# Jsewill/chiaSWARM

Hardware: AMD Instinct MI355X
Metric: images/sec (whole node) SD2.1 512×512 50-step txt2img at 1/2/4/8 MI355X; p50 job latency (higher is better)
Workload: dtype bf16; 1 GPU; bench_config=sd21, global_batch=4, seq_len=4096, parallelism=dp1, resolution=512x512, denoise_steps=50, scheduler=DPMSolverMultistepScheduler (karras), impl=hip, hip_graphs=True

## Files before the change

chiaswarm_amd/models/layers.py:

```python
from __future__ import annotations

import math

import torch
import torch.nn as nn
import torch.nn.functional as F

from .. import ops


class Prepared(nn.Module):

    def prepare(self):
        pass


def prepare_model(model: nn.Module) -> nn.Module:
    for m in model.modules():
        if isinstance(m, Prepared):
            m.prepare()
    if hasattr(model, "prepare_self"):
        model.prepare_self()
    return model


class Linear(nn.Linear, Prepared):

    def forward(self, x, residual=None, act=None, row_stats=False):
        return ops.gemm(x, self.weight, self.bias, residual=residual, act=act, row_stats=row_stats)


class Conv2d(nn.Conv2d, Prepared):

    def prepare(self):
        self.wp = ops.pack_conv_weight(self.weight.detach())

    def _wp(self):
        wp = getattr(self, "wp", None)
        if wp is None or wp.device != self.weight.device or wp.dtype != self.weight.dtype:
            self.prepare()
        return self.wp

    def forward(self, x, residual=None, up2x=False, bias2d=None, padding=None, act=None, out_scale=1.0,
                out=None, gn_stats=False, row_stats=False, residual2=None, res_scale=1.0,
                norm=None, norm_optional=False):
        kh, kw = self.kernel_size
        if (kh == 1 and kw == 1 and self.stride == (1, 1) and not up2x and act is None and out_scale == 1.0
                and out is None and x.is_contiguous() and residual2 is None and res_scale == 1.0 and norm is None):
            w2 = self.weight.view(self.out_channels, self.in_channels)
            gr = x.shape[1] * x.shape[2] if (gn_stats and bias2d is None and x.dim() == 4) else 0
            y = ops.gemm(x, w2, self.bias, residual=residual, gn_rows=gr, row_stats=row_stats and bias2d is None)
            if bias2d is not None:
                y = y + bias2d[:, None, None, :].to(y.dtype)
            return y
        if padding is None:
            ph, pw = self.padding
            pad = ph if ph == pw else (ph, pw, ph, pw)
        else:
            pad = padding
        return ops.conv2d(x, self._wp(), self.bias, self.stride[0], pad, residual=residual,
                          up2x=up2x, bias2d=bias2d, act=act, out_scale=out_scale, out=out,
                          dilation=max(self.dilation), gn_stats=gn_stats, residual2=residual2, res_scale=res_scale,
                          norm=norm, norm_optional=norm_optional)


class Conv1d(nn.Conv1d, Prepared):

    def prepare(self):
        self.wp = self.weight.detach().permute(0, 2, 1).unsqueeze(1).contiguous()

    def _wp(self):
        wp = getattr(self, "wp", None)
        if wp is None or wp.device != self.weight.device or wp.dtype != self.weight.dtype:
            self.prepare()
        return self.wp

    def forward(self, x, act=None, residual=None, out_scale=1.0, out=None, padding=None):
        assert self.stride == (1,), "Conv1d: stride 1 only"
        p = self.padding[0] if padding is None else padding
        return ops.conv1d(x, self._wp(), self.bias, padding=p, dilation=self.dilation[0], act=act,
                          residual=residual, out_scale=out_scale, out=out)


class ConvTranspose1d(nn.ConvTranspose1d, Prepared):

    def prepare(self):
        self.phases = ops.pack_conv_transpose1d(self.weight.detach(), self.stride[0], self.padding[0])

    def forward(self, x, act=None):
        ph = getattr(self, "phases", None)
        if ph is None or (ph[0][0] is not None and (ph[0][0].device != self.weight.device
                                                    or ph[0][0].dtype != self.weight.dtype)):
            self.prepare()
        return ops.conv_transpose1d(x, self.weight, self.bias, self.stride[0], self.padding[0], self.phases, act)


class GroupNorm(nn.GroupNorm):
    def forward(self, x, silu=False):
        pre = getattr(x, "_csk_prenorm", None)
        if pre is not None and pre[0] == self._key(silu):
            return pre[1]
        return ops.group_norm(x, self.weight, self.bias, self.num_groups, self.eps, silu=silu)

    def _key(self, silu):
        w, b = self.weight, self.bias
        return (w.data_ptr(), w._version, b.data_ptr(), b._version, self.num_groups, self.eps, bool(silu))

    def attach(self, raw, normed, silu=False):
        if normed is not None:
            raw._csk_prenorm = (self._key(silu), normed)
        return raw

    def after_conv(self, silu=False, keep_raw=False):
        return (self.weight, self.bias, self.num_groups, self.eps, silu, keep_raw)


class LayerNorm(nn.LayerNorm):
    def forward(self, x):
        return ops.layer_norm(x, self.weight, self.bias, self.eps)


class Attention(Prepared):
    def __init__(self, query_dim, heads, dim_head, cross_dim=None, bias=False, out_bias=True,
                 norm_groups=None, norm_eps=1e-6, residual=False):
        super().__init__()
        inner = heads * dim_head
        self.heads, self.dim_head = heads, dim_head
        self.is_cross = cross_dim is not None
        kv_dim = cross_dim if cross_dim is not None else query_dim
        self.to_q = Linear(query_dim, inner, bias=bias)
        self.to_k = Linear(kv_dim, inner, bias=bias)
        self.to_v = Linear(kv_dim, inner, bias=bias)
        self.to_out = nn.ModuleList([Linear(inner, query_dim, bias=out_bias)])
        self.group_norm = GroupNorm(norm_groups, query_dim, eps=norm_eps) if norm_groups else None
        self.residual = residual
        self.scale = 1.0 / math.sqrt(dim_head)

    def prepare(self):
        q, k, v = self.to_q, self.to_k, self.to_v
        if self.is_cross:
            self.w_kv = torch.cat([k.weight, v.weight], 0).detach()
            self.b_kv = torch.cat([k.bias, v.bias], 0).detach() if k.bias is not None else None
        else:
            self.w_qkv = torch.cat([q.weight, k.weight, v.weight], 0).detach()
            self.b_qkv = (torch.cat([q.bias, k.bias, v.bias], 0).detach()
                          if q.bias is not None else None)

    def _ensure(self):
        attr = "w_kv" if self.is_cross else "w_qkv"
        w = getattr(self, attr, None)
        if w is None or w.device != self.to_q.weight.device or w.dtype != self.to_q.weight.dtype:
            self.prepare()

    def context_kv(self, ctx):
        self._ensure()
        b, s, _ = ctx.shape
        kv = ops.gemm(ctx, self.w_kv, self.b_kv)
        return kv.view(b, s, 2, self.heads, self.dim_head)

    def forward(self, x, ctx=None, kv=None, residual=None, causal=False):
        self._ensure()
        if self.is_cross:
            return self.attend_q(self.to_q(x), kv, ctx if ctx is not None else x, residual)
        return self.attend_qkv(ops.gemm(x, self.w_qkv, self.b_qkv), residual, causal=causal)

    def attend_qkv(self, qkv, residual=None, causal=False, row_stats=False):
        b, s, _ = qkv.shape
        h, d = self.heads, self.dim_head
        qkv = qkv.view(b, s, 3, h, d)
        store = self.__dict__.get("_store_probs")
        if store is not None:
            q, k = qkv[:, :, 0].float().transpose(1, 2), qkv[:, :, 1].float().transpose(1, 2)
            store.append(torch.softmax(q @ k.transpose(-1, -2) * self.scale, dim=-1))
        o = ops.attention(qkv[:, :, 0], qkv[:, :, 1], qkv[:, :, 2], self.scale, causal=causal)
        return self.to_out[0](o.reshape(b, s, h * d), residual=residual, row_stats=row_stats)

    def attend_q(self, q, kv, ctx, residual=None, row_stats=False):
        b, s, _ = q.shape
        h, d = self.heads, self.dim_head
        if kv is None:
            kv = self.context_kv(ctx)
        store = self.__dict__.get("_store_probs")
        if store is not None:
            qf, kf = q.view(b, s, h, d).float().transpose(1, 2), kv[:, :, 0].float().transpose(1, 2)
            store.append(torch.softmax(qf @ kf.transpose(-1, -2) * self.scale, dim=-1))
        o = ops.attention(q.view(b, s, h, d), kv[:, :, 0], kv[:, :, 1], self.scale)
        return self.to_out[0](o.reshape(b, s, h * d), residual=residual, row_stats=row_stats)


class SpatialSelfAttention(Attention):

    def __init__(self, channels, norm_groups=32, eps=1e-6):
        super().__init__(channels, 1, channels, bias=True, norm_groups=norm_groups, norm_eps=eps)

    def forward(self, x):
        b, hh, ww, c = x.shape
        hN = self.group_norm(x).view(b, hh * ww, c)
        out = super().forward(hN, residual=x.view(b, hh * ww, c))
        return out.view(b, hh, ww, c)


class GEGLU(Prepared):
    def __init__(self, dim_in, dim_out):
        super().__init__()
        self.proj = Linear(dim_in, dim_out * 2)

    def prepare(self):
        self.wp, self.bp = ops.pack_geglu(self.proj.weight.detach(),
                                          self.proj.bias.detach() if self.proj.bias is not None else None)

    def ensure(self):
        wp = getattr(self, "wp", None)
        if wp is None or wp.device != self.proj.weight.device or wp.dtype != self.proj.weight.dtype:
            self.prepare()

    def forward(self, x):
        self.ensure()
        return ops.gemm(x, self.wp, self.bp, act="geglu")


class FeedForward(Prepared):

    def __init__(self, dim, mult=4):
        super().__init__()
        inner = dim * mult
        self.inner = inner
        self.net = nn.ModuleList([GEGLU(dim, inner), nn.Identity(), Linear(inner, dim)])

    def prepare(self):
        p, d = self.net[0].proj, self.net[2]
        if p.weight.shape[1] != 320:
            self.ff_w1p = self.ff_b1p = self.ff_w2p = None
            return
        self.ff_w1p, self.ff_b1p, self.ff_w2p = ops.pack_ff_fused(
            p.weight.detach(), None if p.bias is None else p.bias.detach(), d.weight.detach())

    def fused_weights(self):
        w = getattr(self, "ff_w1p", None)
        p = self.net[0].proj.weight
        if (w is None and p.shape[1] == 320) or (w is not None and (w.device != p.device or w.dtype != p.dtype)):
            self.prepare()
        return getattr(self, "ff_w1p", None), getattr(self, "ff_b1p", None), getattr(self, "ff_w2p", None)

    def forward(self, x, residual=None):
        return self.net[2](self.net[0](x), residual=residual)


class BasicTransformerBlock(nn.Module):
    def __init__(self, dim, heads, dim_head, cross_dim):
        super().__init__()
        self.norm1 = LayerNorm(dim)
        self.attn1 = Attention(dim, heads, dim_head)
        self.norm2 = LayerNorm(dim)
        self.attn2 = Attention(dim, heads, dim_head, cross_dim=cross_dim)
        self.norm3 = LayerNorm(dim)
        self.ff = FeedForward(dim)

    def _fold(self, name, w, b, norm):
        key = (w.data_ptr(), w._version, norm.weight.data_ptr(), norm.weight._version, w.dtype, w.device)
        folds = self.__dict__.setdefault("_ln_folds", {})
        f = folds.get(name)
        if f is None or f[0] != key:
            f = (key, ops.fold_layer_norm(w.detach(), None if b is None else b.detach(), norm.weight.detach(),
                                          None if norm.bias is None else norm.bias.detach()))
            folds[name] = f
        return f[1]

    def forward(self, x, ctx=None, kv=None, row_stats=None, dup=False, qkv=None):
        hip = ops.row_stats_wanted(x)
        if row_stats is None:
            row_stats = hip
        a1, a2, ff = self.attn1, self.attn2, self.ff
        a1._ensure()
        if qkv is None:
            fus = ops.ln_fusable(x)
            qkv = ops.layer_norm_gemm(x, self.norm1, a1.w_qkv, a1.b_qkv,
                                      self._fold("qkv", a1.w_qkv, a1.b_qkv, self.norm1) if fus else None)
        x = a1.attend_qkv(qkv, residual=x, row_stats=hip)
        if hip and not dup and kv is not None and x.dim() == 3 and ops.xattn_fusable(x, kv, x.shape[1]):
            w2, colsum, b2 = self._fold("q", a2.to_q.weight, a2.to_q.bias, self.norm2)
            x = ops.xattn_block(x, w2, colsum, b2, kv, a2.to_out[0].weight, a2.to_out[0].bias, self.norm2.eps,
                                a2.scale, x.shape[1], row_stats=hip)
        elif hip and not dup and kv is not None and x.dim() == 3 and ops.qattn_fusable(x, kv, x.shape[1]):
            fus = ops.ln_fusable(x)
            o = ops.layer_norm_gemm_attn(x, self.norm2, a2.to_q.weight, a2.to_q.bias,
                                         self._fold("q", a2.to_q.weight, a2.to_q.bias, self.norm2) if fus else None,
                                         kv, a2.scale, x.shape[1])
            x = a2.to_out[0](o, residual=x, row_stats=hip)
        else:
            fus = ops.ln_fusable(x)
            q = ops.layer_norm_gemm(x, self.norm2, a2.to_q.weight, a2.to_q.bias,
                                    self._fold("q", a2.to_q.weight, a2.to_q.bias, self.norm2) if fus else None)
            if dup:
                q, x = ops.dup2(q), ops.dup2(x)
            x = a2.attend_q(q, kv, ctx if ctx is not None else x, residual=x, row_stats=hip)
        if hip and not row_stats and ops.ff_fusable(x, ff.inner):
            w1p, b1p, w2p = ff.fused_weights()
            if w1p is not None:
                return ops.ff_fused(x, self.norm3.weight, self.norm3.bias, w1p, b1p, w2p, ff.net[2].bias,
                                    self.norm3.eps)
        g = ff.net[0]
        g.ensure()
        fus = ops.ln_fusable(x)
        hdn = ops.layer_norm_gemm(x, self.norm3, g.wp, g.bp, self._fold("ff", g.wp, g.bp, self.norm3) if fus else None,
                                  act="geglu")
        return ff.net[2](hdn, residual=x, row_stats=row_stats)


class Transformer2D(nn.Module):

    def __init__(self, channels, heads, cross_dim, layers=1, linear_proj=True, groups=32):
        super().__init__()
        dim_head = channels // heads
        self.norm = GroupNorm(groups, channels, eps=1e-6)
        self.linear_proj = linear_proj
        if linear_proj:
            self.proj_in = Linear(channels, channels)
            self.proj_out = Linear(channels, channels)
        else:
            self.proj_in = Conv2d(channels, channels, 1)
            self.proj_out = Conv2d(channels, channels, 1)
        self.transformer_blocks = nn.ModuleList(
            [BasicTransformerBlock(channels, heads, dim_head, cross_dim) for _ in range(layers)])

    def cross_modules(self):
        return [blk.attn2 for blk in self.transformer_blocks]

    def _xin_weights(self):
        blk = self.transformer_blocks[0]
        a1 = blk.attn1
        a1._ensure()
        wi = self.proj_in.weight
        key = (wi.data_ptr(), wi._version, a1.w_qkv.data_ptr(), a1.w_qkv._version, blk.norm1.weight._version,
               wi.device, wi.dtype)
        hit = self.__dict__.get("_xin")
        if hit is None or hit[0] != key:
            w2, colsum, b2 = blk._fold("qkv", a1.w_qkv, a1.b_qkv, blk.norm1)
            c = wi.shape[0]
            hit = (key, ops.pack_xin_qkv(wi.detach().reshape(c, c), None if self.proj_in.bias is None
                                         else self.proj_in.bias.detach(), w2, colsum, b2))
            self.__dict__["_xin"] = hit
        return hit[1]

    def _xin_ok(self, x) -> bool:
        if not ops.row_stats_wanted(x) or not self.transformer_blocks:
            return False
        c = x.shape[-1]
        a1 = self.transformer_blocks[0].attn1
        w = self.proj_in.weight
        return (w.shape[0] == c and w.numel() == c * c and a1.to_q.weight.shape[0] == c and not a1.is_cross
                and ops.xin_fusable(x, self.norm.num_groups))

    def forward(self, x, ctx=None, kvs=None, dup=False):
        b, hh, ww, c = x.shape
        hip = ops.row_stats_wanted(x)
        qkv0 = None
        got = None
        if self._xin_ok(x):
            got = ops.xin_qkv(x, self.norm.weight, self.norm.bias, self.norm.num_groups, self.norm.eps,
                              self._xin_weights(), self.transformer_blocks[0].norm1.eps)
        if got is not None:
            h, qkv0 = got[0].view(b, hh * ww, c), got[1].view(b, hh * ww, 3 * c)
        else:
            h = self.norm(x)
            h = self.proj_in(h, row_stats=hip)
            rows = getattr(h, "_csk_rows", None)
            h = h.view(b, hh * ww, c)
            if rows is not None:
                h._csk_rows = rows
        nb = len(self.transformer_blocks)
        for i, blk in enumerate(self.transformer_blocks):
            if dup and i == 0:
                h = blk(h, ctx=ctx, kv=None if kvs is None else kvs[i], row_stats=hip and i + 1 < nb, dup=True,
                        qkv=qkv0)
                x, b = ops.dup2(x), 2 * b
                continue
            h = blk(h, ctx=ctx, kv=None if kvs is None else kvs[i], row_stats=hip and i + 1 < nb,
                    qkv=qkv0 if i == 0 else None)
        if isinstance(self.proj_out, Linear):
            return ops.gemm(h.view(b, hh, ww, c), self.proj_out.weight, self.proj_out.bias, residual=x,
                            gn_rows=hh * ww)
        return self.proj_out(h.view(b, hh, ww, c), residual=x, gn_stats=True)


class ResnetBlock2D(Prepared):

    def __init__(self, cin, cout, temb_channels=None, groups=32, eps=1e-5, groups_out=None):
        super().__init__()
        self.norm1 = GroupNorm(groups, cin, eps=eps)
        self.conv1 = Conv2d(cin, cout, 3, padding=1)
        self.time_emb_proj = Linear(temb_channels, cout) if temb_channels else None
        self.norm2 = GroupNorm(groups_out or groups, cout, eps=eps)
        self.conv2 = Conv2d(cout, cout, 3, padding=1)
        self.conv_shortcut = Conv2d(cin, cout, 1, padding=0) if cin != cout else None
        self.out_channels = cout

    def prepare(self):
        self.__dict__["_scf"] = None

    def _sc_static(self) -> bool:
        sc, c2 = self.conv_shortcut, self.conv2
        return (sc is not None and sc.kernel_size == (1, 1) and sc.stride == (1, 1) and sc.padding == (0, 0)
                and c2.kernel_size == (3, 3) and c2.stride == (1, 1) and c2.padding == (1, 1)
                and c2.dilation == (1, 1) and sc.in_channels % 64 == 0 and c2.in_channels % 64 == 0
                and c2.out_channels % 64 == 0 and self.norm1.weight.dim() == 1 and self.norm2.weight.dim() == 1)

    def _sc_pack(self):
        sc, c2 = self.conv_shortcut, self.conv2
        w2, ws, b2, bs = c2.weight, sc.weight, c2.bias, sc.bias
        key = (w2.data_ptr(), w2._version, ws.data_ptr(), ws._version, None if b2 is None else b2._version,
               None if bs is None else bs._version, w2.device, w2.dtype)
        hit = self.__dict__.get("_scf")
        if hit is None or hit[0] != key:
            _, wv, (wsc,) = ops.pack_conv_extra(ops.pack_conv_weight(w2.detach()),
                                                [ws.detach().reshape(sc.out_channels, sc.in_channels)])
            bias = None
            if b2 is not None or bs is not None:
                bias = sum(b.detach().float() for b in (b2, bs) if b is not None).to(w2.dtype)
            hit = (key, (wv, wsc, bias))
            self.__dict__["_scf"] = hit
        if c2.__dict__.get("wp") is not None:
            c2.wp = None
        return hit[1]

    def _sc_fuse(self, srcs):
        if not ops.SC_FUSE or not self._sc_static():
            return None
        cs = [int(t.shape[-1]) for t in srcs]
        if sum(cs) != self.conv_shortcut.in_channels or any(c % 64 for c in cs) or any(t.dim() != 4 for t in srcs):
            return None
        wv, wsc, bias = self._sc_pack()
        extra, off = [], 0
        for t, c in zip(srcs, cs):
            extra.append((t, wsc[:, off:off + c]))
            off += c
        return wv, tuple(extra), bias

    def _shortcut(self, srcs):
        sc_conv = self.conv_shortcut
        if len(srcs) == 1:
            return sc_conv(srcs[0])
        a, b = srcs
        w = sc_conv.weight.view(sc_conv.out_channels, sc_conv.in_channels)
        ca = a.shape[-1]
        return ops.gemm(b, w[:, ca:], sc_conv.bias, residual=ops.gemm(a, w[:, :ca]))

    def _conv2(self, h, sc, next_norm, fuse=None):
        conv2 = lambda residual, **kw: self.conv2(h, residual=residual, **kw)
        if fuse is not None:
            wv, extra, bias = fuse
            if ops.conv_extra_fusable(h, wv, extra):
                conv2 = lambda residual, **kw: ops.conv2d(h, wv, bias, 1, 1, extra=extra, **kw)
                sc = None
            else:
                sc = self._shortcut(sc)
        if next_norm is None or next_norm.weight.dim() != 1:
            return conv2(sc, gn_stats=True)
        yn, out = conv2(sc, norm=next_norm.after_conv(keep_raw=True), norm_optional=True)
        return next_norm.attach(out, yn)

    def forward(self, x, temb_proj=None, next_norm=None):
        fuse = self._sc_fuse((x,))
        if fuse is not None:
            h = self.norm1(x, silu=True)
            h = self.conv1(h, bias2d=temb_proj, norm=self.norm2.after_conv(silu=True))
            return self._conv2(h, (x,), next_norm, fuse)
        sc = x
        with ops.side_branch(x) as br:
            if self.conv_shortcut is not None:
                sc = self.conv_shortcut(x)
        h = self.norm1(x, silu=True)
        h = self.conv1(h, bias2d=temb_proj, norm=self.norm2.after_conv(silu=True))
        br.join()
        return self._conv2(h, sc, next_norm)

    def forward_cat(self, a, b, temb_proj=None, next_norm=None):
        sc_conv = self.conv_shortcut
        hn = None
        if ops.use_hip(a) and sc_conv is not None and sc_conv.kernel_size == (1, 1) and self.norm1.weight.dim() == 1:
            hn = ops.group_norm_cat(a, b, self.norm1.weight, self.norm1.bias, self.norm1.num_groups,
                                    self.norm1.eps, silu=True)
        if hn is None:
            return self.forward(ops.cat_channels(a, b), temb_proj, next_norm)
        fuse = self._sc_fuse((a, b))
        if fuse is not None:
            h = self.conv1(hn, bias2d=temb_proj, norm=self.norm2.after_conv(silu=True))
            return self._conv2(h, (a, b), next_norm, fuse)
        w = sc_conv.weight.view(sc_conv.out_channels, sc_conv.in_channels)
        ca = a.shape[-1]
        with ops.side_branch(a) as br:
            sc = ops.gemm(a, w[:, :ca])
            sc = ops.gemm(b, w[:, ca:], sc_conv.bias, residual=sc)
        h = self.conv1(hn, bias2d=temb_proj, norm=self.norm2.after_conv(silu=True))
        br.join()
        return self._conv2(h, sc, next_norm)


class Downsample2D(nn.Module):
    def __init__(self, channels, padding=1):
        super().__init__()
        self.conv = Conv2d(channels, channels, 3, stride=2, padding=padding)
        self.pad_asym = padding == 0

    def forward(self, x):
        if self.pad_asym:
            return self.conv(x, padding=(0, 0, 1, 1), gn_stats=True)
        return self.conv(x, gn_stats=True)


class Upsample2D(nn.Module):
    def __init__(self, channels):
        super().__init__()
        self.conv = Conv2d(channels, channels, 3, padding=1)

    def forward(self, x, size=None):
        b, h, w, c = x.shape
        if size is None or (int(size[0]), int(size[1])) == (2 * h, 2 * w):
            return self.conv(x, up2x=True, gn_stats=True)
        xi = F.interpolate(x.permute(0, 3, 1, 2), size=(int(size[0]), int(size[1])), mode="nearest")
        return self.conv(xi.permute(0, 2, 3, 1).contiguous(), gn_stats=True)


def timestep_embedding(t: torch.Tensor, dim: int, flip_sin_to_cos=True, shift=0.0,
                       max_period=10000.0) -> torch.Tensor:
    half = dim // 2
    exponent = -math.log(max_period) * torch.arange(half, dtype=torch.float32, device=t.device)
    exponent = exponent / (half - shift)
    emb = t.float()[:, None] * torch.exp(exponent)[None, :]
    emb = torch.cat([torch.sin(emb), torch.cos(emb)], dim=-1)
    if flip_sin_to_cos:
        emb = torch.cat([emb[:, half:], emb[:, :half]], dim=-1)
    return emb


class TimestepEmbedding(nn.Module):
    def __init__(self, cin, dim):
        super().__init__()
        self.linear_1 = Linear(cin, dim)
        self.linear_2 = Linear(dim, dim)

    def forward(self, x):
        return self.linear_2(self.linear_1(x, act="silu"))


def init_random_(model: nn.Module, seed: int = 0, std_scale: float = 1.0):
    g = torch.Generator(device="cpu").manual_seed(seed)
    with torch.no_grad():
        for name, p in model.named_parameters():
            if p.dim() >= 2:
                fan_in = p[0].numel()
                std = std_scale / math.sqrt(fan_in)
                if name.endswith("embedding.weight") or "embedding" in name and p.dim() == 2 and "linear" not in name:
                    std = 0.02
                t = torch.randn(p.shape, generator=g, dtype=torch.float32) * std
                p.copy_(t.to(p.dtype))
            elif name.endswith("bias"):
                p.zero_()
            else:
                p.fill_(1.0)
    return model


def init_random_fast_(model: nn.Module, seed: int = 0, std_scale: float = 1.0):
    dev = next(model.parameters()).device
    g = torch.Generator(device=dev).manual_seed(seed)
    with torch.no_grad():
        for name, p in model.named_parameters():
            if p.dim() >= 2:
                fan_in = p[0].numel()
                std = std_scale / math.sqrt(fan_in)
                if "embedding" in name and "linear" not in name:
                    std = 0.02
                p.copy_((torch.randn(p.shape, generator=g, device=dev, dtype=torch.float32) * std).to(p.dtype))
            elif name.endswith("bias"):
                p.zero_()
            else:
                p.fill_(1.0)
    return model
```

chiaswarm_amd/ops/__init__.py:

```python
from __future__ import annotations

import math

import os

import torch
import torch.nn.functional as F

from . import _lib
from .mode import get_mode, ops_mode, set_mode, use_hip

GEGLU_BLOCK = 16


def pack_geglu(w: torch.Tensor, b: torch.Tensor | None):
    two_f, k = w.shape
    f = two_f // 2
    assert f % GEGLU_BLOCK == 0
    wp = w.view(2, f // GEGLU_BLOCK, GEGLU_BLOCK, k).transpose(0, 1).reshape(two_f, k)
    bp = None
    if b is not None:
        bp = b.view(2, f // GEGLU_BLOCK, GEGLU_BLOCK).transpose(0, 1).reshape(two_f)
    return wp.contiguous(), (bp.contiguous() if bp is not None else None)


def _gelu_f(x):
    return F.gelu(x)


_ACT_REF = {
    None: lambda y: y, "none": lambda y: y, "gelu": F.gelu, "silu": F.silu,
    "quick_gelu": lambda y: y * torch.sigmoid(1.702 * y), "lrelu": lambda y: F.leaky_relu(y, 0.2),
    "lrelu0.1": lambda y: F.leaky_relu(y, 0.1), "lrelu0.01": lambda y: F.leaky_relu(y, 0.01),
    "tanh": torch.tanh, "relu": F.relu, "elu": F.elu, "gelu_tanh": lambda y: F.gelu(y, approximate="tanh"),
}


def apply_act(y, act):
    return _ACT_REF[act](y)


def _cdt(t):
    return torch.float32 if not t.is_cuda else t.dtype


def _ref_gemm(a2, w, bias, residual, act):
    dt = _cdt(a2)
    if bias is not None:
        y = torch.addmm(bias.to(dt), a2.to(dt), w.to(dt).t())
    else:
        y = a2.to(dt) @ w.to(dt).t()
    if act == "geglu":
        m, n = y.shape
        y = y.view(m, n // (2 * GEGLU_BLOCK), 2, GEGLU_BLOCK)
        y = (y[:, :, 0, :] * _gelu_f(y[:, :, 1, :])).reshape(m, n // 2)
    else:
        y = apply_act(y, act)
    if residual is not None:
        y = y + residual.reshape(y.shape).to(dt)
    return y.to(a2.dtype)


def gemm(a: torch.Tensor, w: torch.Tensor, bias=None, residual=None, act=None, gn_rows=0, row_stats=False):
    lead = a.shape[:-1]
    k = a.shape[-1]
    a2 = a.reshape(-1, k)
    if use_hip(a):
        from . import hip_ops

        y = hip_ops.gemm(a2, w, bias, residual, act, gn_rows=gn_rows, row_stats=row_stats)
    else:
        y = _ref_gemm(a2, w, bias, residual, act)
    out = y.view(*lead, y.shape[-1])
    for attr in ("_csk_gn", "_csk_rows"):
        st = getattr(y, attr, None)
        if st is not None:
            setattr(out, attr, st)
    return out


def fold_layer_norm(w: torch.Tensor, bias, gamma: torch.Tensor, beta):
    wf = w.float()
    w2 = (wf * gamma.float()[None, :]).to(w.dtype)
    colsum = w2.float().sum(1).contiguous()
    b2 = wf @ beta.float() if beta is not None else torch.zeros(w.shape[0], device=w.device)
    if bias is not None:
        b2 = b2 + bias.float()
    return w2.contiguous(), colsum, b2.to(w.dtype)


LN_FUSE = os.environ.get("CSK_LN_FUSE", "1") == "1"


SIDE_STREAM = os.environ.get("CSK_SIDE_STREAM", "0") == "1"
_SIDE: dict = {}


class side_branch:

    def __init__(self, x: torch.Tensor):
        self.on = SIDE_STREAM and use_hip(x)
        self.dev = x.device

    def __enter__(self):
        if self.on:
            self.main = torch.cuda.current_stream(self.dev)
            self.side = _SIDE.get(self.dev)
            if self.side is None:
                self.side = _SIDE[self.dev] = torch.cuda.Stream(self.dev)
            self.side.wait_stream(self.main)
            self._ctx = torch.cuda.stream(self.side)
            self._ctx.__enter__()
        return self

    def __exit__(self, *exc):
        if self.on:
            self._ctx.__exit__(*exc)
        return False

    def join(self):
        if self.on:
            self.main.wait_stream(self.side)


def row_stats_wanted(x: torch.Tensor) -> bool:
    return LN_FUSE and use_hip(x)


def ln_fusable(x: torch.Tensor) -> bool:
    rows = getattr(x, "_csk_rows", None)
    return LN_FUSE and use_hip(x) and rows is not None and x.shape[-1] % 8 == 0


def layer_norm_gemm(x, norm, w, bias, folded, act=None, residual=None, row_stats=False):
    if ln_fusable(x):
        from . import hip_ops

        w2, colsum, b2 = folded
        lead = x.shape[:-1]
        y = hip_ops.gemm(x.reshape(-1, x.shape[-1]), w2, b2, residual, act,
                         ln=(x._csk_rows, colsum, float(norm.eps)), row_stats=row_stats)
        out = y.view(*lead, y.shape[-1])
        if getattr(y, "_csk_rows", None) is not None:
            out._csk_rows = y._csk_rows
        return out
    return gemm(layer_norm(x, norm.weight, norm.bias, norm.eps), w, bias, residual=residual, act=act,
                row_stats=row_stats)


def qattn_fusable(x: torch.Tensor, kv, rows_per_b: int) -> bool:
    if not use_hip(x):
        return False
    from . import hip_ops

    return hip_ops.qattn_ok(x, kv, rows_per_b)


def layer_norm_gemm_attn(x, norm, w, bias, folded, kv, scale, rows_per_b):
    lead = x.shape[:-1]
    if use_hip(x):
        from . import hip_ops

        if ln_fusable(x):
            w2, colsum, b2 = folded
            o = hip_ops.gemm_attn(x.reshape(-1, x.shape[-1]), w2, b2, kv, scale, rows_per_b,
                                  ln=(x._csk_rows, colsum, float(norm.eps)))
        else:
            xn = layer_norm(x, norm.weight, norm.bias, norm.eps)
            o = hip_ops.gemm_attn(xn.reshape(-1, x.shape[-1]), w, bias, kv, scale, rows_per_b)
        return o.view(*lead, o.shape[-1])
    return _ref_gemm_attn(layer_norm(x, norm.weight, norm.bias, norm.eps), w, bias, kv, scale)


def _ref_gemm_attn(xn, w, bias, kv, scale):
    b, s, c = xn.shape
    q = xn.float() @ w.float().t()
    if bias is not None:
        q = q + bias.float()
    heads, d = kv.shape[3], kv.shape[4]
    k, v = kv[:b, :, 0].float(), kv[:b, :, 1].float()
    qh = q.view(b, s, heads, d).transpose(1, 2)
    att = torch.softmax((qh @ k.permute(0, 2, 3, 1)) * scale, -1)
    return (att @ v.transpose(1, 2)).transpose(1, 2).reshape(b, s, c).to(xn.dtype)


_FF_PERM = (0, 1, 2, 3, 8, 9, 10, 11, 4, 5, 6, 7, 12, 13, 14, 15)


def _ff_keys(device):
    r = torch.arange(32, device=device)
    k1 = (r & 7) ^ ((r >> 3) & 1)
    k2 = (r >> 2) & 3
    p8, p4 = torch.arange(8, device=device), torch.arange(4, device=device)
    return p8[None, :] ^ k1[:, None], p4[None, :] ^ k2[:, None]


def pack_ff_fused(w1, b1, w2):
    two_i, c = w1.shape
    inner = two_i // 2
    t = inner // 16
    k8, k4 = _ff_keys(w1.device)
    w1t = torch.stack((w1[:inner].reshape(t, 16, c), w1[inner:].reshape(t, 16, c)), 1).reshape(t, 32, c // 64, 8, 8)
    w1p = torch.gather(w1t, 3, k8[None, :, None, :, None].expand(t, 32, c // 64, 8, 8))
    w1p = w1p.permute(0, 2, 1, 3, 4).reshape(t, c // 64, 32, 64)
    b1p = None
    if b1 is not None:
        b1p = torch.stack((b1[:inner].reshape(t, 16), b1[inner:].reshape(t, 16)), 1).reshape(t, 32).float()
    perm = torch.tensor(_FF_PERM, device=w2.device)
    w2q = w2.reshape(c, t, 16).index_select(2, perm).reshape(c // 32, 32, inner // 32, 4, 8)
    w2p = torch.gather(w2q, 3, k4[None, :, None, :, None].expand(c // 32, 32, inner // 32, 4, 8))
    w2p = w2p.permute(2, 0, 1, 3, 4).reshape(inner // 32, c // 32, 32, 32)
    return w1p.contiguous(), (None if b1p is None else b1p.contiguous()), w2p.contiguous()


def unpack_ff_fused(w1p, b1p, w2p):
    t, si = w1p.shape[0], w1p.shape[1]
    c, inner = 64 * si, 16 * t
    k8, k4 = _ff_keys(w1p.device)
    inv8, inv4 = torch.argsort(k8, 1), torch.argsort(k4, 1)
    x = w1p.reshape(t, si, 32, 8, 8).permute(0, 2, 1, 3, 4)
    x = torch.gather(x, 3, inv8[None, :, None, :, None].expand(t, 32, si, 8, 8)).reshape(t, 32, c)
    w1 = torch.cat((x[:, :16].reshape(inner, c), x[:, 16:].reshape(inner, c)), 0)
    b1 = None if b1p is None else torch.cat((b1p[:, :16].reshape(inner), b1p[:, 16:].reshape(inner)), 0)
    nc, no = w2p.shape[0], w2p.shape[1]
    y = w2p.reshape(nc, no, 32, 4, 8).permute(1, 2, 0, 3, 4)
    y = torch.gather(y, 3, inv4[None, :, None, :, None].expand(no, 32, nc, 4, 8)).reshape(c, inner // 16, 16)
    w2 = y[:, :, torch.argsort(torch.tensor(_FF_PERM, device=w2p.device))].reshape(c, inner)
    return w1, b1, w2


def ff_fusable(x: torch.Tensor, inner: int) -> bool:
    if not use_hip(x) or x.dim() != 3:
        return False
    from . import hip_ops

    return hip_ops.ff_fused_ok(x, inner)


def ff_fused(x, gamma, beta, w1p, b1p, w2p, b2, eps):
    if use_hip(x):
        from . import hip_ops

        return hip_ops.ff_geglu(x, gamma, beta, w1p, b1p, w2p, b2, eps)
    return _ref_ff_fused(x, gamma, beta, w1p, b1p, w2p, b2, eps)


def _ref_ff_fused(x, gamma, beta, w1p, b1p, w2p, b2, eps):
    w1, b1, w2 = unpack_ff_fused(w1p, b1p, w2p)
    c, inner = w2.shape
    xf = x.float()
    h = torch.nn.functional.layer_norm(xf, (c,), gamma.float(), None if beta is None else beta.float(), eps)
    vg = torch.nn.functional.linear(h, w1.float(), None if b1 is None else b1.float())
    hid = vg[..., :inner] * torch.nn.functional.gelu(vg[..., inner:])
    y = torch.nn.functional.linear(hid, w2.float(), None if b2 is None else b2.float())
    return (xf + y).to(x.dtype)


def _a_tiles(w):
    n, c = w.shape
    t = n // 32
    k8, _ = _ff_keys(w.device)
    x = w.reshape(t, 32, c // 64, 8, 8)
    x = torch.gather(x, 3, k8[None, :, None, :, None].expand(t, 32, c // 64, 8, 8))
    return x.permute(0, 2, 1, 3, 4).reshape(t, c // 64, 32, 64)


def _a_untiles(p):
    t, si = p.shape[0], p.shape[1]
    k8, _ = _ff_keys(p.device)
    inv8 = torch.argsort(k8, 1)
    x = p.reshape(t, si, 32, 8, 8).permute(0, 2, 1, 3, 4)
    return torch.gather(x, 3, inv8[None, :, None, :, None].expand(t, 32, si, 8, 8)).reshape(32 * t, 64 * si)


def pack_xin_qkv(wi, bi, wq, colsum, bq):
    c = wi.shape[0]
    perm = torch.tensor(_FF_PERM, device=wq.device)
    wqp = wq.reshape(wq.shape[0], c // 16, 16).index_select(2, perm).reshape(wq.shape[0], c)
    w = torch.cat([_a_tiles(wi.reshape(c, c)), _a_tiles(wqp)], 0).contiguous()
    f32 = lambda t, n: (torch.zeros(n, device=wi.device) if t is None else t.float()).contiguous()
    return w, f32(bi, c), f32(colsum, wq.shape[0]), f32(bq, wq.shape[0])


def unpack_xin_qkv(w):
    c = 64 * w.shape[1]
    full = _a_untiles(w)
    wi, wqp = full[:c], full[c:]
    inv = torch.argsort(torch.tensor(_FF_PERM, device=w.device))
    return wi, wqp.reshape(wqp.shape[0], c // 16, 16).index_select(2, inv).reshape(wqp.shape[0], c)


def xin_fusable(x: torch.Tensor, groups: int) -> bool:
    if not use_hip(x):
        return False
    from . import hip_ops

    return hip_ops.xin_ok(x, groups)


def xin_qkv(x, gn_gamma, gn_beta, groups, gn_eps, packed, ln_eps):
    w, bi, colsum, bq = packed
    if use_hip(x):
        from . import hip_ops

        stat = hip_ops.gn_stats(x, groups, gn_eps)
        if stat is None:
            return None
        return hip_ops.xin_qkv(x, stat, gn_gamma, gn_beta, w, bi, colsum, bq, ln_eps)
    return _ref_xin_qkv(x, gn_gamma, gn_beta, groups, gn_eps, packed, ln_eps)


def _ref_xin_qkv(x, gn_gamma, gn_beta, groups, gn_eps, packed, ln_eps):
    w, bi, colsum, bq = packed
    wi, wq = unpack_xin_qkv(w)
    B, C = x.shape[0], x.shape[-1]
    xf = x.float().reshape(B, -1, C)
    g = xf.reshape(B, -1, groups, C // groups)
    mean = g.mean(dim=(1, 3), keepdim=True)
    var = g.var(dim=(1, 3), keepdim=True, unbiased=False)
    xg = ((g - mean) * torch.rsqrt(var + gn_eps)).reshape(B, -1, C)
    xg = xg * gn_gamma.float() + (0 if gn_beta is None else gn_beta.float())
    h = xg @ wi.float().t() + bi
    n = torch.nn.functional.layer_norm(h, (C,), eps=ln_eps)
    qkv = n @ wq.float().t() + bq
    return h.reshape(-1, C).to(x.dtype), qkv.reshape(-1, 3 * C).to(x.dtype)


def xattn_fusable(x: torch.Tensor, kv, rows_per_b: int) -> bool:
    if not use_hip(x):
        return False
    from . import hip_ops

    return hip_ops.xattn_ok(x, kv, rows_per_b)


def xattn_block(x, wq, colsum, bq, kv, wo, bo, eps, scale, rows_per_b, row_stats=True):
    if use_hip(x):
        from . import hip_ops

        return hip_ops.xattn_block(x, wq, colsum, bq, kv, wo, bo, eps, scale, rows_per_b, row_stats=row_stats)
    return _ref_xattn_block(x, wq, colsum, bq, kv, wo, bo, eps, scale)


def _ref_xattn_block(x, wq, colsum, bq, kv, wo, bo, eps, scale):
    xf = x.float()
    mean = xf.mean(-1, keepdim=True)
    rstd = torch.rsqrt(xf.var(-1, unbiased=False, keepdim=True) + eps)
    q = rstd * (xf @ wq.float().t() - mean * colsum.float()) + bq.float()
    b, s, c = x.shape
    heads, d = kv.shape[3], kv.shape[4]
    k, v = kv[:b, :, 0].float(), kv[:b, :, 1].float()
    qh = q.view(b, s, heads, d).transpose(1, 2)
    att = torch.softmax((qh @ k.permute(0, 2, 3, 1)) * scale, -1)
    o = (att @ v.transpose(1, 2)).transpose(1, 2).reshape(b, s, c)
    y = o @ wo.float().t() + xf
    if bo is not None:
        y = y + bo.float()
    return y.to(x.dtype)


def cat_channels(a: torch.Tensor, b: torch.Tensor) -> torch.Tensor:
    y = torch.cat([a, b], dim=-1)
    sa, sb = getattr(a, "_csk_gn", None), getattr(b, "_csk_gn", None)
    if sa is not None and sb is not None and sa[1] == sb[1]:
        ca, cb = a.shape[-1], b.shape[-1]
        nseg = sa[0].numel() // (2 * ca)
        if nseg * 2 * cb == sb[0].numel():
            y._csk_gn = (torch.cat([sa[0].view(nseg, ca, 2), sb[0].view(nseg, cb, 2)], 1).view(-1), sa[1])
    return y


def pack_conv_weight(w: torch.Tensor) -> torch.Tensor:
    return w.permute(0, 2, 3, 1).contiguous()


def norm_padding(padding):
    if isinstance(padding, int):
        return (padding,) * 4
    assert len(padding) == 4
    return tuple(int(p) for p in padding)


def conv_out_size(h, w, kh, kw, stride, padding, up2x=False, dilation=1):
    pt, pl, pb, pr = norm_padding(padding)
    if up2x:
        h, w = 2 * h, 2 * w
    return ((h + pt + pb - dilation * (kh - 1) - 1) // stride + 1,
            (w + pl + pr - dilation * (kw - 1) - 1) // stride + 1)


def _ref_conv2d(x, wp, bias, stride, padding, residual, up2x, bias2d, act=None, out_scale=1.0, dilation=1,
                residual2=None, res_scale=1.0, extra=None):
    dt = _cdt(x)
    xn = x.to(dt).permute(0, 3, 1, 2)
    if up2x:
        xn = F.interpolate(xn, scale_factor=2.0, mode="nearest")
    pt, pl, pb, pr = norm_padding(padding)
    w = wp.to(dt).permute(0, 3, 1, 2)
    b = bias.to(dt) if bias is not None else None
    if pt == pb and pl == pr and min(pt, pl) >= 0:
        y = F.conv2d(xn, w, b, stride=stride, padding=(pt, pl), dilation=dilation)
    else:
        y = F.conv2d(F.pad(xn, (pl, pr, pt, pb)), w, b, stride=stride, dilation=dilation)
    y = y.permute(0, 2, 3, 1)
    for a, wa in extra or ():
        y = y + a.to(dt) @ wa.to(dt).t()
    if bias2d is not None:
        y = y + bias2d.to(dt)[:, None, None, :]
    y = apply_act(y, act)
    if out_scale != 1.0:
        y = y * out_scale
    if residual is not None:
        y = y + (residual.to(dt) if res_scale == 1.0 else res_scale * residual.to(dt))
    if residual2 is not None:
        y = y + residual2.to(dt)
    return y.to(x.dtype).contiguous()


SC_FUSE = os.environ.get("CSK_SC_FUSE", "1") == "1"


def pack_conv_extra(wp: torch.Tensor, ws) -> tuple:
    cout, kh, kw, cin = wp.shape
    wf = torch.cat([wp.reshape(cout, -1)] + [w.reshape(cout, -1).to(wp.dtype) for w in ws], dim=1).contiguous()
    k0, views = kh * kw * cin, []
    off = k0
    for w in ws:
        c = w.reshape(cout, -1).shape[1]
        views.append(wf[:, off:off + c])
        off += c
    return wf, wf[:, :k0].unflatten(1, (kh, kw, cin)), tuple(views)


def conv_extra_fusable(x, wp, extra, stride=1, padding=1, up2x=False, dilation=1) -> bool:
    if not use_hip(x):
        return True
    from . import hip_ops

    return hip_ops.conv_extra_ok(x, wp, extra, stride, padding, up2x, dilation)


def conv2d(x, wp, bias=None, stride=1, padding=1, residual=None, up2x=False, bias2d=None, act=None,
           out_scale=1.0, out=None, dilation=1, gn_stats=False, residual2=None, res_scale=1.0, out_u8=False,
           norm=None, norm_optional=False, extra=None):
    if use_hip(x):
        from . import hip_ops

        return hip_ops.conv2d(x, wp, bias, stride, padding, residual, up2x, bias2d, act, out_scale, out, dilation,
                              gn_stats, residual2=residual2, res_scale=res_scale, out_u8=out_u8, norm=norm,
                              norm_optional=norm_optional, extra=extra)
    if norm is not None and (out_u8 or residual2 is not None or res_scale != 1.0):
        raise ValueError("conv2d: norm with out_u8 / residual2 / res_scale")
    if norm is not None and out is not None and not norm[5]:
        raise ValueError("conv2d: out= with norm is the raw output: it needs keep_raw")
    y = _ref_conv2d(x, wp, bias, stride, padding, residual, up2x, bias2d, act, out_scale, dilation,
                    residual2, res_scale, extra)
    if out_u8:
        y = (y.float().clamp(0, 1) * 255).round().to(torch.uint8)
    if out is not None:
        out.copy_(y)
        y = out
    if norm is not None:
        gamma, beta, groups, eps, silu, keep_raw = norm
        if norm_optional and keep_raw:
            return None, y
        yn = _ref_group_norm(y, gamma, beta, groups, eps, silu)
        return (yn, y) if keep_raw else yn
    return y


DW_KMAX = 7
DW_PAD_MODES = ("zeros", "reflect")


def pack_depthwise_weight(w: torch.Tensor) -> torch.Tensor:
    if w.dim() == 4:
        if w.shape[1] != 1:
            raise ValueError(f"pack_depthwise_weight: expected [C, 1, kh, kw], got {tuple(w.shape)}")
        w = w[:, 0]
    if w.dim() != 3:
        raise ValueError(f"pack_depthwise_weight: expected [C, 1, kh, kw] or [C, kh, kw], got {tuple(w.shape)}")
    return w.detach().permute(1, 2, 0).float().contiguous()


def _dw_check(name, x, wp, bias, padding, pad_mode):
    if x.dim() != 4:
        raise ValueError(f"{name}: x must be NHWC [B, H, W, C], got {tuple(x.shape)}")
    B, H, W, C = x.shape
    if C % 8 != 0:
        raise ValueError(f"{name}: C = {C} is not a multiple of 8")
    if wp.dim() != 3 or wp.shape[2] != C or wp.dtype != torch.float32:
        raise ValueError(f"{name}: wp must be pack_depthwise_weight's fp32 [kh, kw, {C}], got "
                         f"{wp.dtype} {tuple(wp.shape)}")
    kh, kw = wp.shape[0], wp.shape[1]
    if not (1 <= kh <= DW_KMAX and 1 <= kw <= DW_KMAX):
        raise ValueError(f"{name}: kernel {kh}x{kw} outside 1..{DW_KMAX}")
    if pad_mode not in DW_PAD_MODES:
        raise ValueError(f"{name}: pad_mode {pad_mode!r} not in {DW_PAD_MODES}")
    pad = norm_padding(padding)
    if min(pad) < 0:
        raise ValueError(f"{name}: negative padding {pad}")
    pt, pl, pb, pr = pad
    if pad_mode == "reflect" and (max(pt, pb) >= H or max(pl, pr) >= W):
        raise ValueError(f"{name}: reflect padding {pad} must be smaller than the input {H}x{W}")
    if bias is not None and tuple(bias.shape) != (C,):
        raise ValueError(f"{name}: bias shape {tuple(bias.shape)} != ({C},)")
    return pad


def _dw_view_check(name, t, shape, what):
    if t is not None and tuple(t.shape) != tuple(shape):
        raise ValueError(f"{name}: {what} shape {tuple(t.shape)} != {tuple(shape)}")


def _dw_padded(x, pad, pad_mode):
    pt, pl, pb, pr = pad
    xn = x.to(_cdt(x)).permute(0, 3, 1, 2)
    if max(pad) == 0:
        return xn
    return F.pad(xn, (pl, pr, pt, pb), mode="reflect" if pad_mode == "reflect" else "constant")


def _ref_depthwise_conv2d(x, wp, bias, stride, pad, pad_mode, residual):
    dt = _cdt(x)
    c = x.shape[-1]
    w = wp.permute(2, 0, 1).unsqueeze(1).to(dt).contiguous()
    y = F.conv2d(_dw_padded(x, pad, pad_mode), w, bias.to(dt) if bias is not None else None, stride=stride, groups=c)
    y = y.permute(0, 2, 3, 1)
    if residual is not None:
        y = y + residual.to(dt)
    return y.to(x.dtype).contiguous()


def depthwise_conv2d(x, wp, bias=None, stride=1, padding=0, pad_mode="zeros", residual=None, out=None):
    name = "depthwise_conv2d"
    pad = _dw_check(name, x, wp, bias, padding, pad_mode)
    if stride not in (1, 2):
        raise ValueError(f"{name}: stride {stride} not in (1, 2)")
    B, H, W, C = x.shape
    ho, wo = conv_out_size(H, W, wp.shape[0], wp.shape[1], stride, pad)
    if ho < 1 or wo < 1:
        raise ValueError(f"{name}: kernel {wp.shape[0]}x{wp.shape[1]} larger than the padded input")
    _dw_view_check(name, residual, (B, ho, wo, C), "residual")
    _dw_view_check(name, out, (B, ho, wo, C), "out")
    if use_hip(x):
        from . import hip_ops

        return hip_ops.depthwise_conv2d(x, wp, bias, stride, pad, pad_mode, residual, out, (ho, wo))
    y = _ref_depthwise_conv2d(x, wp, bias, stride, pad, pad_mode, residual)
    if out is not None:
        out.copy_(y)
        y = out
    return y


def _ref_depthwise_conv_transpose2d(x, wp, bias, pad, pad_mode, crop):
    dt = _cdt(x)
    c = x.shape[-1]
    w = wp.permute(2, 0, 1).unsqueeze(1).to(dt).contiguous()
    y = F.conv_transpose2d(_dw_padded(x, pad, pad_mode), w, bias.to(dt) if bias is not None else None, stride=2,
                           padding=crop, groups=c)
    return y.permute(0, 2, 3, 1).to(x.dtype).contiguous()


def depthwise_conv_transpose2d(x, wp, bias=None, in_padding=0, pad_mode="zeros", crop=0, out=None):
    name = "depthwise_conv_transpose2d"
    pad = _dw_check(name, x, wp, bias, in_padding, pad_mode)
    if not isinstance(crop, int) or crop < 0:
        raise ValueError(f"{name}: crop {crop!r} must be a non-negative int")
    B, H, W, C = x.shape
    pt, pl, pb, pr = pad
    ho = (H + pt + pb - 1) * 2 - 2 * crop + wp.shape[0]
    wo = (W + pl + pr - 1) * 2 - 2 * crop + wp.shape[1]
    if ho < 1 or wo < 1:
        raise ValueError(f"{name}: crop {crop} leaves no output")
    _dw_view_check(name, out, (B, ho, wo, C), "out")
    if use_hip(x):
        from . import hip_ops

        return hip_ops.depthwise_conv_transpose2d(x, wp, bias, pad, pad_mode, crop, out, (ho, wo))
    y = _ref_depthwise_conv_transpose2d(x, wp, bias, pad, pad_mode, crop)
    if out is not None:
        out.copy_(y)
        y = out
    return y


def conv1d(x, wp, bias=None, padding=0, dilation=1, act=None, residual=None, out_scale=1.0, out=None):
    pl, pr = (padding, padding) if isinstance(padding, int) else padding
    x4 = x.unsqueeze(1)
    r4 = residual.unsqueeze(1) if residual is not None else None
    o4 = out.unsqueeze(1) if out is not None else None
    y = conv2d(x4, wp, bias, 1, (0, pl, 0, pr), residual=r4, act=act, out_scale=out_scale, out=o4,
               dilation=dilation)
    return y.squeeze(1)


def pack_conv_transpose1d(w: torch.Tensor, stride: int, padding: int):
    cin, cout, k = w.shape
    s, p = int(stride), int(padding)
    phases = []
    for r in range(s):
        j0, q = (r + p) % s, (r + p) // s
        nt = max(0, -(-(k - j0) // s))
        if nt == 0:
            phases.append((None, 0))
            continue
        taps = [j0 + (nt - 1 - u) * s for u in range(nt)]
        wr = w[:, :, taps]
        phases.append((wr.permute(1, 2, 0).unsqueeze(1).contiguous(), nt - 1 - q))
    return phases


def conv_transpose1d(x, w, bias, stride, padding, phases=None, act=None):
    b, L, _ = x.shape
    cout, k = w.shape[1], w.shape[2]
    s = int(stride)
    lout = (L - 1) * s - 2 * padding + k
    if not use_hip(x):
        dt = _cdt(x)
        y = F.conv_transpose1d(x.to(dt).transpose(1, 2), w.to(dt), bias.to(dt) if bias is not None else None,
                               stride=s, padding=padding)
        return apply_act(y.transpose(1, 2), act).to(x.dtype).contiguous()
    if phases is None:
        phases = pack_conv_transpose1d(w, s, padding)
    return _conv_transpose1d_polyphase(x, phases, bias, s, lout, cout, act)


def _conv_transpose1d_polyphase(x, phases, bias, s, lout, cout, act=None):
    b, L, _ = x.shape
    tmax = -(-lout // s)
    buf = torch.empty(b, tmax * s, cout, dtype=x.dtype, device=x.device)
    view = buf.view(b, tmax, s, cout)
    for r, (wp, pl) in enumerate(phases):
        tr = -(-(lout - r) // s)
        if tr <= 0:
            continue
        o = view[:, :tr, r, :]
        if wp is None:
            o.copy_((bias if bias is not None else torch.zeros(cout, device=x.device)).to(x.dtype).expand_as(o))
            if act is not None:
                o.copy_(apply_act(o.float(), act).to(o.dtype))
            continue
        nt = wp.shape[2]
        pr = tr - L - pl + nt - 1
        if b > 1 and tr != tmax:
            for i in range(b):
                conv1d(x[i:i + 1], wp, bias, padding=(pl, pr), act=act, out=o[i:i + 1])
        else:
            conv1d(x, wp, bias, padding=(pl, pr), act=act, out=o)
    return buf[:, :lout] if tmax * s != lout else buf


def axpby_nhwc(x, z, a, b, out=None, act=None):
    if out is None:
        out = torch.empty(x.shape, dtype=x.dtype, device=x.device)
    if use_hip(x):
        from . import hip_ops

        if x.dim() == 3:
            hip_ops.axpby_nhwc(x.unsqueeze(1), z.unsqueeze(1) if z is not None else None, a, b, out.unsqueeze(1), act)
            return out
        return hip_ops.axpby_nhwc(x, z, a, b, out, act)
    y = a * x.to(_cdt(x))
    if z is not None:
        y = y + b * z.to(_cdt(x))
    out.copy_(apply_act(y, act).to(out.dtype))
    return out


def act(x, kind, out=None):
    return axpby_nhwc(x, None, 1.0, 0.0, out, kind)


def axpby(x, y, a, b):
    if use_hip(x):
        from . import hip_ops

        return hip_ops.axpby(x, y, a, b)
    return (a * x.to(_cdt(x)) + b * y.to(_cdt(x))).to(x.dtype)


def _ref_group_norm(x, gamma, beta, groups, eps, silu):
    dt = _cdt(x)
    c = x.shape[-1]
    xn = x.to(dt).movedim(-1, 1)
    if gamma.dim() == 2:
        y = F.group_norm(xn, groups, None, None, eps)
        shp = (gamma.shape[0], c) + (1,) * (xn.dim() - 2)
        y = y * gamma.to(dt).view(shp) + beta.to(dt).view(shp)
    else:
        y = F.group_norm(xn, groups, gamma.to(dt), beta.to(dt), eps)
    if silu == "gelu":
        y = F.gelu(y)
    elif silu:
        y = F.silu(y)
    return y.movedim(1, -1).to(x.dtype).contiguous()


def group_norm(x, gamma, beta, groups=32, eps=1e-5, silu=False):
    if use_hip(x):
        from . import hip_ops

        return hip_ops.group_norm(x, gamma, beta, groups, eps, silu)
    return _ref_group_norm(x, gamma, beta, groups, eps, silu)


def group_norm_cat(a, b, gamma, beta, groups=32, eps=1e-5, silu=False):
    if use_hip(a):
        from . import hip_ops

        return hip_ops.group_norm_cat(a, b, gamma, beta, groups, eps, silu)
    return None


def _ref_layer_norm(x, gamma, beta, eps):
    dt = _cdt(x)
    return F.layer_norm(x.to(dt), (x.shape[-1],), gamma.to(dt), beta.to(dt) if beta is not None else None,
                        eps).to(x.dtype)


def layer_norm(x, gamma, beta, eps=1e-5):
    if use_hip(x):
        from . import hip_ops

        return hip_ops.layer_norm(x, gamma, beta, eps)
    return _ref_layer_norm(x, gamma, beta, eps)


def _ref_attention(q, k, v, scale, causal):
    if q.is_cuda:
        o = F.scaled_dot_product_attention(q.transpose(1, 2), k.transpose(1, 2), v.transpose(1, 2),
                                           is_causal=causal, scale=scale)
        return o.transpose(1, 2).contiguous()
    qt, kt, vt = (t.permute(0, 2, 1, 3).float() for t in (q, k, v))
    s = (qt @ kt.transpose(-1, -2)) * scale
    if causal:
        sq, sk = s.shape[-2], s.shape[-1]
        mask = torch.ones(sq, sk, dtype=torch.bool, device=s.device).triu(1 + sk - sq)
        s = s.masked_fill(mask, float("-inf"))
    p = torch.softmax(s, dim=-1)
    o = p @ vt
    return o.permute(0, 2, 1, 3).to(q.dtype).contiguous()


def _ref_attention_bias(q, k, v, scale, causal=False, bias=None, kv_lens=None):
    B, Sq, H, _ = q.shape
    Skv = k.shape[1]
    qt, kt, vt = (t.permute(0, 2, 1, 3).float() for t in (q, k, v))
    s = (qt @ kt.transpose(-1, -2)) * scale
    if bias is not None:
        s = s + bias.float().expand(B, H, Sq, Skv)
    if kv_lens is not None:
        hidden = torch.arange(Skv, device=s.device)[None, :] >= kv_lens.reshape(B, 1).to(torch.long)
        s = s.masked_fill(hidden[:, None, None, :], float("-inf"))
    if causal:
        mask = torch.ones(Sq, Skv, dtype=torch.bool, device=s.device).triu(1 + Skv - Sq)
        s = s.masked_fill(mask, float("-inf"))
    m = s.amax(-1, keepdim=True)
    p = torch.exp(s - torch.where(torch.isinf(m), torch.zeros_like(m), m))
    l = p.sum(-1, keepdim=True)
    o = (p @ vt) / torch.where(l > 0, l, torch.ones_like(l))
    return o.permute(0, 2, 1, 3).to(q.dtype).contiguous()


def attention(q, k, v, scale=None, causal=False, kv_len=None, *, bias=None, kv_lens=None):
    if scale is None:
        scale = 1.0 / math.sqrt(q.shape[-1])
    if bias is not None or kv_lens is not None:
        if kv_len is not None:
            raise ValueError("attention: kv_len (KV-cache fill level) and kv_lens (per-sample key padding) "
                             "cannot be combined")
        if use_hip(q):
            from . import hip_ops

            return hip_ops.attention_bias(q, k, v, scale, causal, bias, kv_lens)
        return _ref_attention_bias(q, k, v, scale, causal, bias, kv_lens)
    if use_hip(q):
        from . import hip_ops

        return hip_ops.attention(q, k, v, scale, causal, kv_len)
    if kv_len is not None:
        n = int(kv_len.reshape(-1)[0].item())
        k, v = k[:, :n], v[:, :n]
    return _ref_attention(q, k, v, scale, causal)


def _ref_rms_norm(x, gamma, eps):
    xf = x.float()
    return xf * torch.rsqrt(xf.pow(2).mean(-1, keepdim=True) + eps) * gamma.float()


def _ref_decode_norm(x2, ln, rms, what):
    if ln is not None and rms is not None:
        raise ValueError(f"{what}: ln= and rms= exclude each other")
    if ln is not None:
        return _ref_layer_norm(x2, ln[0], ln[1], ln[2])
    if rms is not None:
        return _ref_rms_norm(x2, rms[0], rms[1]).to(_cdt(x2))
    return x2


def gemv(x, w, bias=None, *, act=None, residual=None, ln=None, rms=None, out=None):
    if ln is not None and rms is not None:
        raise ValueError("gemv: ln= and rms= exclude each other")
    lead = x.shape[:-1]
    k = x.shape[-1]
    x2 = x.reshape(-1, k)
    if use_hip(x):
        from . import hip_ops

        y = hip_ops.gemv(x2, w, bias, act, residual, ln, out, rms)
    else:
        y = _ref_gemm(_ref_decode_norm(x2, ln, rms, "gemv"), w, bias, residual, act).to(x.dtype)
        if out is not None:
            out.copy_(y)
            y = out
    return y.view(*lead, y.shape[-1]) if out is None else y


def gemv_glu(x, w_gate, w_up, *, act="silu", rms=None, ln=None, out=None):
    if ln is not None and rms is not None:
        raise ValueError("gemv_glu: ln= and rms= exclude each other")
    if act == "geglu":
        raise ValueError("gemv_glu: act is the gate's pointwise activation, not 'geglu'")
    lead = x.shape[:-1]
    x2 = x.reshape(-1, x.shape[-1])
    if use_hip(x):
        from . import hip_ops

        y = hip_ops.gemv_glu(x2, w_gate, w_up, act, rms, ln, out)
    else:
        xn = _ref_decode_norm(x2, ln, rms, "gemv_glu")
        y = (_ref_gemm(xn, w_gate, None, None, act) * _ref_gemm(xn, w_up, None, None, None)).to(x.dtype)
        if out is not None:
            out.copy_(y)
            y = out
    return y.view(*lead, y.shape[-1]) if out is None else y


def _ref_rope(x, cos, sin):
    h = x.shape[-1] // 2
    xf = x.float()
    a, b = xf[..., :h], xf[..., h:]
    return torch.cat((a * cos - b * sin, b * cos + a * sin), -1)


def decode_attention(q, k_cache, v_cache, scale, kv_len, *, k_new=None, v_new=None, pos=None, rope=None):
    if scale is None:
        scale = 1.0 / math.sqrt(q.shape[-1])
    if not isinstance(kv_len, torch.Tensor) or kv_len.dtype != torch.int32 or kv_len.device != q.device:
        raise TypeError("decode_attention: kv_len must be an int32 tensor on the device of q")
    if q.dim() != 4 or q.shape[1] != 1:
        raise ValueError(f"decode_attention: q must be [B, 1, H, D], got {tuple(q.shape)}")
    B, _, H, D = q.shape
    if (k_cache.dim() != 4 or k_cache.shape != v_cache.shape or k_cache.shape[0] != B or k_cache.shape[3] != D
            or k_cache.shape[2] < 1 or H % k_cache.shape[2] != 0):
        raise ValueError(f"decode_attention: caches {tuple(k_cache.shape)} / {tuple(v_cache.shape)} do not match "
                         f"q {tuple(q.shape)}")
    Hkv = k_cache.shape[2]
    if (k_new is None) != (v_new is None):
        raise ValueError("decode_attention: k_new and v_new come together")
    if k_new is not None and (k_new.shape != (B, 1, Hkv, D) or v_new.shape != (B, 1, Hkv, D)):
        raise ValueError(f"decode_attention: k_new / v_new {tuple(k_new.shape)} / {tuple(v_new.shape)} must be "
                         f"{(B, 1, Hkv, D)}")
    if rope is not None and (D % 2 or len(rope) != 2):
        raise ValueError("decode_attention: rope = (cos, sin) needs an even head dim")
    if use_hip(q):
        from . import hip_ops

        return hip_ops.decode_attention(q, k_cache, v_cache, scale, kv_len, k_new, v_new, pos, rope)
    n = min(max(int(kv_len.reshape(-1)[0].item()), 0), k_cache.shape[1])
    if n == 0:
        return torch.zeros_like(q)
    if rope is not None:
        cos, sin = rope[0][n - 1].float(), rope[1][n - 1].float()
        q = _ref_rope(q, cos, sin).to(q.dtype)
        if k_new is not None:
            k_new = _ref_rope(k_new, cos, sin)
    if k_new is not None:
        k_cache[:, n - 1] = k_new[:, 0].to(k_cache.dtype)
        v_cache[:, n - 1] = v_new[:, 0].to(v_cache.dtype)
    k, v = k_cache[:, :n], v_cache[:, :n]
    if Hkv != H:
        k, v = (t[:, :, :, None].expand(B, n, Hkv, H // Hkv, D).reshape(B, n, H, D) for t in (k, v))
    return _ref_attention(q, k, v, scale, False)


def canny(gray: torch.Tensor, low: float = 100.0, high: float = 200.0) -> torch.Tensor:
    if use_hip(gray):
        from . import hip_ops

        return hip_ops.canny(gray, low, high)
    from ..controlnet.preprocess import canny_np

    return torch.from_numpy(canny_np(gray.cpu().numpy(), float(low), float(high))).to(gray.device)


def dup2(x):
    if use_hip(x):
        from . import hip_ops

        y = hip_ops.dup2(x)
        st = getattr(x, "_csk_gn", None)
        if st is not None:
            y._csk_gn = (torch.cat([st[0], st[0]]), st[1])
        return y
    return torch.cat([x, x], 0)


def silu(x):
    if use_hip(x):
        from . import hip_ops

        return hip_ops.silu(x)
    return F.silu(x.to(_cdt(x))).to(x.dtype)


def add(x, y):
    if use_hip(x):
        from . import hip_ops

        return hip_ops.add(x, y)
    return (x.to(_cdt(x)) + y.to(_cdt(x))).to(x.dtype)


def _ref_sched_step(e, x, prev_x0, c, guidance, noise):
    ef = e.float()
    if guidance is not None:
        e_u, e_c = ef.chunk(2)
        ef = e_u + guidance * (e_c - e_u)
    x0 = c.p * x + c.q * ef
    out = c.A * x + c.B * x0
    if c.C != 0.0 and prev_x0 is not None:
        out = out + c.C * prev_x0
    if c.D != 0.0 and noise is not None:
        out = out + c.D * noise
    return out, x0


def sched_step(e, x, sched, coeffs, guidance=None, noise=None):
    prev = sched.prev_x0
    if use_hip(x):
        from . import hip_ops

        out, x0 = hip_ops.sched_step(e, x, prev, coeffs, guidance, noise)
    else:
        out, x0 = _ref_sched_step(e, x, prev, coeffs, guidance, noise)
    sched.prev_x0 = x0
    sched.step_index += 1
    return out


def vae_postprocess(img):
    if use_hip(img):
        from . import hip_ops

        return hip_ops.vae_postprocess(img)
    return ((img.float() / 2 + 0.5).clamp(0, 1) * 255).round().to(torch.uint8)
```

chiaswarm_amd/ops/hip_ops.py:

```python
from __future__ import annotations

import ctypes
import os

import torch

from . import _lib, tuning
from ._lib import c_float, c_int, c_int64, c_void_p, sig

ACT = {None: 0, "none": 0, "gelu": 1, "silu": 2, "geglu": 3, "quick_gelu": 4}

sig("csk_gemm", c_void_p, c_void_p, c_void_p, c_void_p, c_void_p, c_void_p,
    c_int, c_int, c_int, c_int, c_int, c_int, c_int, c_int, c_int, c_float, c_void_p, c_int, c_int, c_void_p, c_void_p)
sig("csk_conv2d", c_void_p, c_void_p, c_void_p, c_void_p, c_void_p, c_void_p,
    c_int, c_int, c_int, c_int, c_int, c_int, c_int, c_int, c_int, c_int, c_int, c_int, c_int,
    c_int, c_int, c_int, c_int, c_float, c_int, c_void_p, c_int, c_int, c_void_p, c_void_p)
sig("csk_gemm_ln", c_void_p, c_void_p, c_void_p, c_void_p, c_void_p, c_void_p,
    c_int, c_int, c_int, c_int, c_int, c_int, c_int, c_int, c_int, c_float, c_void_p,
    c_void_p, c_void_p, c_int, c_int, c_float, c_void_p, c_void_p, c_int, c_int, c_void_p, c_void_p)
sig("csk_conv2d_ex", c_void_p, c_void_p, c_void_p, c_void_p, c_void_p, c_int, c_void_p,
    c_int, c_int, c_int, c_int, c_int, c_int, c_int, c_int, c_int, c_int, c_int, c_int, c_int,
    c_int, c_int, c_int, c_int, c_float, c_int, c_void_p, c_int, c_int, c_void_p, c_void_p)
sig("csk_group_norm_part", c_void_p, c_void_p, c_void_p, c_int, c_void_p, c_int, c_void_p, c_void_p, c_void_p,
    c_int, c_int, c_int, c_int, c_int, c_int, c_float, c_int, c_int, c_void_p)
sig("csk_group_norm_part2", c_void_p, c_void_p, c_void_p, c_int, c_void_p, c_void_p, c_int, c_void_p, c_void_p,
    c_void_p, c_int, c_int, c_int, c_int, c_int, c_int, c_float, c_int, c_int, c_void_p)


GN_FINE = 0


def set_gn_fine(v: int):
    global GN_FINE
    GN_FINE = int(v)
    _lib.call("csk_set_gn_fine", GN_FINE)


GN_TARGET_WG = 512
SPLITK_GN_SEG = 64
SPLITK_GN = True


def _gn_seg(tile, split, rows_per_b, M, code, N=8):
    bm, bn = tuning.TILES.get(tile, (0, 0))
    if code == 3 or bm == 0 or rows_per_b <= 0:
        return 0
    if split > 1:
        if not SPLITK_GN:
            return 0
        s = SPLITK_GN_SEG
        return s if rows_per_b % s == 0 and M % s == 0 and N % 8 == 0 else 0
    if rows_per_b % bm or M % bm:
        return 0
    seg = bm * bn // 256 if GN_FINE else bm
    band = bm // tuning.EPI_WM.get(tile, 2) if (bm > 128 or bn == 160) else bm
    return min(seg, band)


def _ws(split, M, N, device):
    if split > 1:
        return torch.empty(split * M * N, dtype=torch.float32, device=device)
    if split < 0:
        return torch.empty(-split * (M + 255) * (N + 255), dtype=torch.float32, device=device)
    return None


def _gn_part(M, N, seg, device):
    return torch.empty((M // seg) * N * 2, dtype=torch.float32, device=device)
sig("csk_axpby", c_void_p, c_void_p, c_void_p, c_int64, c_float, c_float, c_void_p)
ACT.update({"lrelu": 5, "lrelu0.1": 6, "tanh": 7, "relu": 8, "lrelu0.01": 9, "elu": 10, "gelu_tanh": 11})
sig("csk_group_norm", c_void_p, c_void_p, c_void_p, c_int, c_void_p, c_void_p, c_void_p, c_int, c_int, c_int, c_int,
    c_int, c_int, c_float, c_int, c_int, c_void_p)
sig("csk_layer_norm", c_void_p, c_void_p, c_void_p, c_void_p, c_int, c_int, c_float, c_void_p)
ATTN_VARIANT = int(os.environ.get("CSK_ATTN", "0"))
sig("csk_attention", c_void_p, c_void_p, c_void_p, c_void_p, ctypes.POINTER(c_int64), c_int, c_int, c_int, c_int,
    c_int, c_float, c_int, c_int, c_void_p, c_void_p)
sig("csk_silu", c_void_p, c_void_p, c_int64, c_void_p)
sig("csk_canny", c_void_p, c_void_p, c_int, c_int, c_int, c_float, c_float, c_void_p, c_void_p)
sig("csk_add", c_void_p, c_void_p, c_void_p, c_int64, c_void_p)
sig("csk_sched_step", c_void_p, c_void_p, c_void_p, c_void_p, c_void_p, c_void_p, c_int64,
    c_float, c_float, c_float, c_float, c_float, c_float, c_float, c_int, c_void_p)
sig("csk_vae_post", c_void_p, c_void_p, c_int64, c_void_p)
sig("csk_loop_prologue", c_void_p, c_void_p, c_void_p, c_void_p, c_int, c_void_p)
sig("csk_sched_loop", c_void_p, c_void_p, c_void_p, c_void_p, c_void_p, c_void_p, c_void_p, c_int, c_int, c_int64,
    c_int, c_void_p)
LOOP_COEF_STRIDE = 12
sig("csk_pad_channels", c_void_p, c_void_p, c_int64, c_int, c_int, c_void_p)
sig("csk_set_gn_prologue_max", c_int)
sig("csk_debug_selftest", c_int, c_void_p)
sig("csk_set_gn_lds", c_int)
sig("csk_set_sw_odd", c_int)
sig("csk_set_epi_band", c_int)
sig("csk_set_epi_nt", c_int)
sig("csk_set_skr_unroll", c_int)
sig("csk_set_short_kv_variant", c_int)
sig("csk_set_short_kv_rows", c_int)
sig("csk_set_attn32", c_int)
sig("csk_xattn_block", c_void_p, c_void_p, c_void_p, c_void_p, c_void_p, c_void_p, c_void_p, c_void_p, c_void_p,
    c_int, c_int, c_int, c_int, c_int, c_float, c_float, c_void_p)
sig("csk_attention_fa", c_void_p, c_void_p, c_void_p, c_void_p, ctypes.POINTER(c_int64), c_int, c_int, c_int, c_int,
    c_int, c_float, c_int, c_void_p)
sig("csk_set_attn_fa", c_int)
sig("csk_attn_fa_ok", c_int, c_int, c_int, c_int, c_int, c_int, c_int)
sig("csk_attention_split", c_void_p, c_void_p, c_void_p, c_void_p, ctypes.POINTER(c_int64), c_int, c_int, c_int, c_int,
    c_int, c_float, c_int, c_void_p, c_void_p, c_void_p)
sig("csk_dup2", c_void_p, c_void_p, c_int64, c_void_p)
sig("csk_row_bcast", c_void_p, c_void_p, c_void_p, c_int, c_int, c_int, c_void_p)
sig("csk_set_ln_in_kernel", c_int)
sig("csk_set_gn_finalize_wg", c_int)
sig("csk_set_gn_cb", c_int)
sig("csk_set_gn_cb_mult", c_int)
sig("csk_set_gn_cb_small", c_int)
sig("csk_set_gn_fine", c_int)
sig("csk_timestep_embedding", c_void_p, c_void_p, c_int, c_int, c_int, c_int, c_float, c_float, c_void_p)


def timestep_embedding(t, batch, dim, flip_sin_to_cos=True, shift=0.0, max_period=10000.0):
    t = t.reshape(-1)
    if t.dtype != torch.float32 or not t.is_contiguous():
        t = t.float().contiguous()
    if t.numel() not in (1, batch):
        raise ValueError(f"timestep_embedding: {t.numel()} timesteps for batch {batch}")
    y = torch.empty((batch, dim), dtype=torch.bfloat16, device=t.device)
    _lib.call("csk_timestep_embedding", _p(y), _p(t), 0 if t.numel() == 1 else 1, batch, dim,
              int(bool(flip_sin_to_cos)), float(shift), float(max_period), _s())
    return y


def _bf16(t, name):
    if t.dtype != torch.bfloat16:
        raise TypeError(f"{name}: HIP kernels take bfloat16, got {t.dtype}")


def _p(t):
    return None if t is None else t.data_ptr()


def _s():
    return _lib.stream_ptr()


def _round8(n):
    return (n + 7) // 8 * 8


def pad_last(x: torch.Tensor, n: int) -> torch.Tensor:
    c = x.shape[-1]
    if c == n:
        return x
    x = x.contiguous()
    y = torch.empty(x.shape[:-1] + (n,), dtype=x.dtype, device=x.device)
    rows = x.numel() // c
    _lib.call("csk_pad_channels", _p(y), _p(x), rows, c, n, _s())
    return y


def gemm(a2, w, bias=None, residual=None, act=None, out=None, gn_rows=0, ln=None, row_stats=False):
    _bf16(a2, "gemm.a")
    _bf16(w, "gemm.w")
    M, K = a2.shape
    N = w.shape[0]
    if w.shape[1] != K:
        raise ValueError(f"gemm: K mismatch {a2.shape} x {w.shape}")
    if a2.stride(1) != 1 or a2.stride(0) % 8 != 0 or (a2.data_ptr() % 16):
        a2 = a2.contiguous()
    if w.stride(1) != 1 or w.stride(0) % 8 != 0:
        w = w.contiguous()
    if K % 8 != 0:
        kp = _round8(K)
        a2 = pad_last(a2, kp)
        w = pad_last(w, kp)
        K = kp
    code = ACT[act]
    n_out = N // 2 if code == 3 else N
    if out is None:
        out = torch.empty((M, n_out), dtype=torch.bfloat16, device=a2.device)
    if residual is not None:
        residual = residual.reshape(M, n_out)
        _bf16(residual, "gemm.residual")
        if not residual.is_contiguous():
            residual = residual.contiguous()
    if bias is not None:
        _bf16(bias, "gemm.bias")
    lda, ldb = a2.stride(0), w.stride(0)

    def run(tile, split, part=None):
        ws = _ws(split, M, N, a2.device)
        _lib.call("csk_gemm", _p(out), _p(a2), _p(w), _p(bias), None, _p(residual),
                  M, N, K, lda, ldb, n_out, n_out, 1, code, 1.0, _p(part), tile, split, _p(ws), _s())

    tile, split = tuning.choose(f"g:{M}:{N}:{K}:{code}", M, N, K, run)
    if split < 0 and tile not in tuning.GLDS:
        split = 1
    if ln is not None or row_stats:
        if split > 1:
            tile, split = (19 if N <= 1280 else 20), 1
        if tile in (25, 26, 31, 32, 33, 34):
            tile = 11
        elif tile == 36:
            tile = 13
        if ln is None and code == 3:
            row_stats = False
    seg = _gn_seg(tile, split, gn_rows, M, code, N) if gn_rows and out.is_contiguous() else 0
    part = _gn_part(M, N, seg, a2.device) if seg else None
    if ln is None and not row_stats:
        run(tile, split, part)
    else:
        bn = tuning.TILES[tile][1]
        rp = torch.empty(-(-N // bn) * M * 2, dtype=torch.float32, device=a2.device) if row_stats else None
        lp = lc = rowbuf = None
        nparts = pcols = 0
        eps = 0.0
        if ln is not None:
            (lp, nparts, pcols), lc, eps = ln
            if K % 8 or nparts * pcols < K or lp.numel() < nparts * M * 2:
                raise ValueError("gemm: fused LayerNorm statistics do not match the input")
            rowbuf = torch.empty(M * 2, dtype=torch.float32, device=a2.device)
        _lib.call("csk_gemm_ln", _p(out), _p(a2), _p(w), _p(bias), None, _p(residual),
                  M, N, K, lda, ldb, n_out, n_out, 1, code, 1.0, _p(part), _p(lp), _p(lc), nparts, pcols,
                  float(eps), _p(rowbuf), _p(rp), tile, 1, None, _s())
        if rp is not None:
            out._csk_rows = (rp, -(-N // bn), bn)
    if part is not None:
        out._csk_gn = (part, seg)
    return out


sig("csk_gemm_ln_attn", c_void_p, c_void_p, c_void_p, c_void_p, c_int, c_int, c_int, c_int, c_int, c_int, c_int,
    c_void_p, c_void_p, c_int, c_int, c_float, c_void_p, c_void_p, c_int, c_int, c_float, c_int, c_void_p)
QATTN = os.environ.get("CSK_QATTN", "1") == "1"
QATTN_MIN_TILES = int(os.environ.get("CSK_QATTN_MIN_TILES", "256"))
QATTN_STATS = [0]


def qattn_ok(x, kv, rows_per_b) -> bool:
    C = x.shape[-1]
    M = x.numel() // C
    return (QATTN and kv is not None and kv.dim() == 5 and kv.shape[2] == 2 and kv.shape[4] == 64
            and kv.shape[3] * 64 == C and 1 <= kv.shape[1] <= 80 and C % 64 == 0 and rows_per_b % 128 == 0
            and M % rows_per_b == 0 and kv.shape[0] >= M // rows_per_b
            and (M // 128) * (C // 64) >= QATTN_MIN_TILES)


def gemm_attn(a2, w, bias, kv, scale, rows_per_b, ln=None, tile=None):
    _bf16(a2, "gemm_attn.a")
    _bf16(w, "gemm_attn.w")
    _bf16(kv, "gemm_attn.kv")
    M, K = a2.shape
    N = w.shape[0]
    if w.shape[1] != K or K % 8:
        raise ValueError(f"gemm_attn: K mismatch {a2.shape} x {w.shape}")
    if a2.stride(1) != 1 or a2.stride(0) % 8 != 0 or (a2.data_ptr() % 16):
        a2 = a2.contiguous()
    w = w.contiguous()
    kv = kv.contiguous()
    if bias is not None:
        _bf16(bias, "gemm_attn.bias")
        bias = bias.contiguous()
    if tile is None:
        tile = 12 if K >= 1280 else 19
    elif tile not in (12, 19):
        raise ValueError("gemm_attn: tile 12 or 19")
    out = torch.empty((M, N), dtype=torch.bfloat16, device=a2.device)
    lp = lc = rowbuf = None
    nparts = pcols = 0
    eps = 0.0
    if ln is not None:
        (lp, nparts, pcols), lc, eps = ln
        if nparts * pcols < K or lp.numel() < nparts * M * 2:
            raise ValueError("gemm_attn: fused LayerNorm statistics do not match the input")
        rowbuf = torch.empty(M * 2, dtype=torch.float32, device=a2.device)
    QATTN_STATS[0] += 1
    _lib.call("csk_gemm_ln_attn", _p(out), _p(a2), _p(w), _p(bias), M, N, K, a2.stride(0), w.stride(0), N,
              int(rows_per_b), _p(lp), _p(lc), nparts, pcols, float(eps), _p(rowbuf), _p(kv), int(kv.shape[0]),
              int(kv.shape[1]), float(scale), tile, _s())
    return out


def _pix_stride(t):
    B, H, W, C = t.shape
    s = t.stride()
    if s[3] != 1:
        return None
    ps = s[2]
    if (W > 1 and s[2] != ps) or (H > 1 and s[1] != W * ps) or (B > 1 and s[0] != H * W * ps):
        return None
    return ps


sig("csk_conv_tile_ok2", c_int, c_int, c_int, c_int, c_int, c_int, c_int, c_int)
sig("csk_conv_tile2", c_void_p, c_void_p, c_void_p, c_void_p, c_void_p, c_void_p, c_int, c_int, c_int, c_int, c_int,
    c_int, c_int, c_int, c_int, c_int, c_float, c_float, c_int, c_int, c_void_p)
CONV_TILE = os.environ.get("CSK_CONV_TILE", "1") == "1"
CONV_TILE64 = os.environ.get("CSK_CONV_TILE64", "1") == "1"
CONV_TILE_NARROW_MIN_PX = int(os.environ.get("CSK_CONV_TILE_NARROW_MIN_PX", str(1 << 18)))
CONV_TILE_STATS = [0]

sig("csk_set_skgn_fused", c_int)
sig("csk_set_skgn_min_wg", c_int)
sig("csk_get_skgn_min_wg")
sig("csk_get_skr_unroll")
sig("csk_splitk_gn_fused_ok", c_int, c_int, c_int, c_int)
sig("csk_conv2d_gn", c_void_p, c_void_p, c_void_p, c_void_p, c_void_p, c_int, c_void_p, c_int, c_int, c_int, c_int,
    c_int, c_int, c_int, c_int, c_int, c_int, c_int, c_int, c_int, c_int, c_int, c_int, c_float, c_int, c_int, c_int,
    c_void_p, c_void_p, c_void_p, c_void_p, c_int, c_float, c_int, c_int, c_void_p)
sig("csk_conv2d_ex2", c_void_p, c_void_p, c_void_p, c_void_p, c_void_p, c_int, c_void_p, c_int, c_int, c_int, c_int,
    c_int, c_int, c_int, c_int, c_int, c_int, c_int, c_int, c_int, c_int, c_int, c_int, c_int, c_float, c_int,
    c_void_p, c_int, c_int, c_void_p, c_void_p, c_int, c_int, c_void_p, c_int, c_int, c_void_p)
sig("csk_conv2d_gn2", c_void_p, c_void_p, c_void_p, c_void_p, c_void_p, c_int, c_void_p, c_int, c_int, c_int, c_int,
    c_int, c_int, c_int, c_int, c_int, c_int, c_int, c_int, c_int, c_int, c_int, c_int, c_float, c_int, c_int, c_int,
    c_void_p, c_void_p, c_void_p, c_void_p, c_int, c_float, c_int, c_int, c_void_p, c_int, c_int, c_void_p, c_int,
    c_int, c_void_p)
SC_FUSE_STATS = [0]
XS_TILES = tuning.GLDS | {33, 34}
SC_FUSE_OFF = set()


def conv_extra_ok(x, wp, extra, stride=1, padding=1, up2x=False, dilation=1) -> bool:
    from . import conv_out_size

    if not extra or len(extra) > 2 or x.dim() != 4 or x.dtype != torch.bfloat16:
        return False
    B, H, W, Cin = x.shape
    Cout, kh, kw, _ = wp.shape
    if stride != 1 or up2x or dilation != 1 or Cin % 64 or conv_out_size(H, W, kh, kw, 1, padding) != (H, W):
        return False
    xs = _pix_stride(x)
    if xs is None or xs % 8 or x.data_ptr() % 16:
        return False
    for a, wa in extra:
        if a.dtype != torch.bfloat16 or a.dim() != 4 or tuple(a.shape[:3]) != (B, H, W) or a.shape[3] % 64:
            return False
        ps = _pix_stride(a)
        if ps is None or ps % 8 or a.data_ptr() % 16 or tuple(wa.shape) != (Cout, a.shape[3]):
            return False
    if (B, H, W, Cin, Cout, tuple(a.shape[3] for a, _ in extra)) in SC_FUSE_OFF:
        return False
    return fused_weight(wp, extra) is not None


def fused_weight(wp, extra):
    Cout, kh, kw, Cin = wp.shape
    k0 = kh * kw * Cin
    K = k0 + sum(w.shape[1] for _, w in extra)
    if wp.dtype != torch.bfloat16 or wp.stride() != (K, kw * Cin, Cin, 1) or wp.data_ptr() % 16:
        return None
    off = k0
    for _, w in extra:
        if w.dtype != wp.dtype or w.stride() != (K, 1) or w.data_ptr() != wp.data_ptr() + 2 * off:
            return None
        off += w.shape[1]
    return torch.as_strided(wp, (Cout, K), (K, 1))


SKGN_FUSED = os.environ.get("CSK_SKGN_FUSED", "1") == "1"
SKGN_STATS = [0, 0, 0]
SKGN_SITES = None


def set_skgn_fused(on: bool):
    global SKGN_FUSED
    SKGN_FUSED = bool(on)
    _lib.call("csk_set_skgn_fused", int(SKGN_FUSED))


def set_skgn_min_wg(n: int) -> int:
    old = _lib.call_int("csk_get_skgn_min_wg")
    _lib.call("csk_set_skgn_min_wg", int(n))
    return old


def _eff_split(split, K):
    if split <= 1:
        return split
    kchunk = -(-(-(-K // 64)) // split) * 64
    return -(-K // kchunk)


def _skgn_ok(split, K, M, Cout, rows_per_b, ys, code, gamma, beta, groups, silu, bias, bias2d, b2s, residual, rs,
             out, keep_raw):
    if not SKGN_FUSED or _eff_split(split, K) <= 1 or code != 0 or gamma.dim() != 1 or silu not in (True, False):
        return False
    if gamma.dtype != torch.bfloat16 or beta.dtype != torch.bfloat16 or gamma.numel() != Cout or beta.numel() != Cout:
        return False
    if not (gamma.is_contiguous() and beta.is_contiguous()):
        return False
    for t in (gamma, beta, bias, bias2d, residual, out if keep_raw else None):
        if t is not None and t.data_ptr() % 8:
            return False
    if (keep_raw and ys % 4) or (residual is not None and rs % 4) or (bias2d is not None and b2s % 4):
        return False
    return _lib.call_int("csk_splitk_gn_fused_ok", M, Cout, rows_per_b, int(groups)) > 0


def conv2d(x, wp, bias, stride, padding, residual, up2x, bias2d, act=None, out_scale=1.0, out=None, dilation=1,
           gn_stats=False, residual2=None, res_scale=1.0, out_u8=False, norm=None, norm_optional=False, extra=None):
    from . import conv_out_size, norm_padding

    if extra is not None:
        if out_u8 or residual2 is not None or res_scale != 1.0:
            raise ValueError("conv2d: extra with out_u8 / residual2 / res_scale")
        if not conv_extra_ok(x, wp, extra, stride, padding, up2x, dilation):
            raise ValueError("conv2d: extra K segments need conv_extra_ok() (64-channel multiples, same-size "
                             "stride-1 conv, aligned NHWC sources, one packed weight)")
    if norm is not None:
        if out_u8 or residual2 is not None or res_scale != 1.0:
            raise ValueError("conv2d: norm with out_u8 / residual2 / res_scale")
        if out is not None and not norm[5]:
            raise ValueError("conv2d: out= with norm is the raw output: it needs keep_raw")
        gn_stats = True

    _bf16(x, "conv.x")
    _bf16(wp, "conv.w")
    B, H, W, Cin = x.shape
    xs = _pix_stride(x)
    if xs is None or xs % 8 != 0 or Cin % 8 != 0 or x.data_ptr() % 16:
        x = x.contiguous()
        xs = Cin
    Cout, kh, kw, Cw = wp.shape
    if Cw != Cin:
        raise ValueError(f"conv2d: Cin mismatch {tuple(x.shape)} vs {tuple(wp.shape)}")
    if Cin % 8 != 0:
        cp = _round8(Cin)
        x = pad_last(x, cp)
        wp = pad_last(wp.contiguous(), cp)
        Cin = xs = cp
    wf, xseg = None, ()
    if extra is not None:
        wf = fused_weight(wp, extra)
        xseg = tuple((a, _pix_stride(a), a.shape[3]) for a, _ in extra)
    else:
        wp = wp.contiguous()
    pt, pl, pb, pr = norm_padding(padding)
    Ho, Wo = conv_out_size(H, W, kh, kw, stride, padding, up2x, dilation)
    if out_u8:
        return _conv2d_u8(x, wp, bias, stride, padding, residual, up2x, bias2d, act, out_scale, out, dilation,
                          residual2, res_scale, Ho, Wo)
    oshape = (B, Ho, Wo, Cout)
    if out is None and (norm is None or norm[5]):
        out = torch.empty(oshape, dtype=torch.bfloat16, device=x.device)
    ys = Cout if out is None else _pix_stride(out)
    if out is not None and (out.shape != oshape or ys is None):
        raise ValueError(f"conv2d out {tuple(out.shape)} / strides unsupported")
    rs = 0
    if residual is not None:
        if tuple(residual.shape) != oshape:
            raise ValueError(f"conv2d residual {tuple(residual.shape)} != {oshape}")
        rs = _pix_stride(residual)
        if rs is None:
            residual = residual.contiguous()
            rs = Cout
    b2s = 0
    if bias2d is not None:
        if bias2d.shape != (B, Cout):
            raise ValueError("conv2d bias2d shape")
        _bf16(bias2d, "conv.bias2d")
        if bias2d.stride(1) != 1 or bias2d.data_ptr() % 16 or bias2d.stride(0) % 8:
            bias2d = bias2d.contiguous()
        b2s = bias2d.stride(0) if B > 1 else Cout
    M, K = B * Ho * Wo, kh * kw * Cin + sum(s[2] for s in xseg)
    code = ACT[act]
    sargs = ()
    if xseg:
        sb = xseg[1] if len(xseg) > 1 else (None, 0, 0)
        sargs = (_p(xseg[0][0]), xseg[0][1], xseg[0][2], _p(sb[0]), sb[1], sb[2])

    def run(tile, split, part=None):
        nonlocal out
        if out is None:
            out = torch.empty(oshape, dtype=torch.bfloat16, device=x.device)
        ws = _ws(split, M, Cout, x.device)
        if xseg:
            _lib.call("csk_conv2d_ex2", _p(out), _p(x), _p(wf), _p(bias), _p(bias2d), b2s, _p(residual),
                      B, H, W, Cin, Cout, kh, kw, stride, pt, pl, Ho, Wo, 0, xs, ys, rs, code,
                      float(out_scale), int(dilation), _p(part), tile, split, _p(ws), *sargs, _s())
            return
        _lib.call("csk_conv2d_ex", _p(out), _p(x), _p(wp), _p(bias), _p(bias2d), b2s, _p(residual),
                  B, H, W, Cin, Cout, kh, kw, stride, pt, pl, Ho, Wo, int(bool(up2x)), xs, ys, rs, code,
                  float(out_scale), int(dilation), _p(part), tile, split, _p(ws), _s())

    rs2 = 0
    if residual2 is not None:
        if tuple(residual2.shape) != oshape:
            raise ValueError(f"conv2d residual2 {tuple(residual2.shape)} != {oshape}")
        rs2 = _pix_stride(residual2)
        if rs2 is None:
            residual2 = residual2.contiguous()
            rs2 = Cout
    key = f"c:{B}:{H}:{W}:{Cin}:{Cout}:{kh}:{stride}:{int(bool(up2x))}"
    if kh != kw or dilation != 1:
        key += f":{kw}:{dilation}"
    narrow = Cout < 16
    if xseg:
        fkey = key + ":x" + ":".join(str(s[2]) for s in xseg)
        tile, split = tuning.choose_extra(fkey, key, M, Cout, K, run, XS_TILES)
        SC_FUSE_STATS[0] += 1
    elif (CONV_TILE and kh == 3 and kw == 3 and stride == 1 and (pt, pl, pb, pr) == (1, 1, 1, 1) and dilation == 1
            and bias2d is None and not gn_stats
            and code in (0, 2, 5, 6, 8, 9)
            and (Cout == 32 or (Cout == 64 and CONV_TILE64) or (Cout <= 16 and M >= CONV_TILE_NARROW_MIN_PX))
            and (residual is None or (not narrow and rs % 4 == 0 and residual.data_ptr() % 8 == 0))
            and (residual2 is None or (not narrow and rs2 % 4 == 0 and residual2.data_ptr() % 8 == 0))
            and _lib.call_int("csk_conv_tile_ok2", B, Ho, Wo, Cin, Cout, xs, ys, int(bool(up2x))) > 0
            and x.data_ptr() % 16 == 0 and (narrow or out.data_ptr() % 8 == 0) and wp.data_ptr() % 16 == 0):
        _lib.call("csk_conv_tile2", _p(out), _p(x), _p(wp), _p(bias), _p(residual), _p(residual2), B, Ho, Wo, Cin,
                  Cout, xs, ys, rs, rs2, code, float(out_scale), float(res_scale), int(bool(up2x)), 0, _s())
        CONV_TILE_STATS[0] += 1
        return out
    elif residual2 is not None or res_scale != 1.0:
        y = conv2d(x, wp, bias, stride, padding, None, up2x, bias2d, act, out_scale, None, dilation)
        if residual is not None:
            y = torch.add(y, residual, alpha=res_scale) if res_scale != 1.0 else y + residual
        if residual2 is not None:
            y = y + residual2
        out.copy_(y)
        return out
    else:
        tile, split = tuning.choose(key, M, Cout, K, run)
    if norm is not None:
        gamma, beta, groups, eps, silu, keep_raw = norm
        if ys == Cout and _skgn_ok(split, K, M, Cout, Ho * Wo, ys, code, gamma, beta, groups, silu, bias, bias2d, b2s,
                                   residual, rs, out, keep_raw):
            yn = torch.empty((B, Ho, Wo, Cout), dtype=torch.bfloat16, device=x.device)
            ws = _ws(split, M, Cout, x.device)
            _lib.call("csk_conv2d_gn2" if xseg else "csk_conv2d_gn", _p(out) if keep_raw else None, _p(x),
                      _p(wf if xseg else wp), _p(bias), _p(bias2d), b2s,
                      _p(residual), B, H, W, Cin, Cout, kh, kw, stride, pt, pl, Ho, Wo, int(bool(up2x)), xs, ys, rs,
                      float(out_scale), int(dilation), tile, split, _p(ws), _p(yn), _p(gamma), _p(beta), int(groups),
                      float(eps), int(bool(silu)), int(bool(keep_raw)), *sargs, _s())
            SKGN_STATS[0] += 1
            if SKGN_SITES is not None:
                SKGN_SITES.append((B, Ho, Wo, Cin, Cout, split, bool(keep_raw)))
            return (yn, out) if keep_raw else yn
    seg = _gn_seg(tile, split, Ho * Wo, M, code, Cout) if gn_stats and ys == Cout else 0
    part = _gn_part(M, Cout, seg, x.device) if seg else None
    run(tile, split, part)
    if part is not None:
        out._csk_gn = (part, seg)
    return _norm_after(out, norm, norm_optional)


def _norm_after(out, norm, optional=False):
    if norm is None:
        return out
    gamma, beta, groups, eps, silu, keep_raw = norm
    if optional and keep_raw:
        SKGN_STATS[2] += 1
        return None, out
    SKGN_STATS[1] += 1
    yn = group_norm(out, gamma, beta, groups, eps, silu)
    return (yn, out) if keep_raw else yn


def _conv2d_u8(x, wp, bias, stride, padding, residual, up2x, bias2d, act, out_scale, out, dilation, residual2,
               res_scale, Ho, Wo):
    from . import norm_padding

    B, H, W, Cin = x.shape
    Cout = wp.shape[0]
    if out is None:
        out = torch.empty((B, Ho, Wo, Cout), dtype=torch.uint8, device=x.device)
    if out.dtype != torch.uint8 or out.shape != (B, Ho, Wo, Cout) or not out.is_contiguous():
        raise ValueError("conv2d out_u8: out must be a contiguous uint8 [B, Ho, Wo, Cout]")
    xs = _pix_stride(x)
    if (CONV_TILE and Cout < 16 and residual is None and residual2 is None and bias2d is None and stride == 1
            and wp.shape[1:3] == (3, 3) and norm_padding(padding) == (1, 1, 1, 1) and dilation == 1
            and code_ok(act) and B * Ho * Wo >= CONV_TILE_NARROW_MIN_PX and xs is not None
            and x.data_ptr() % 16 == 0 and wp.is_contiguous() and wp.data_ptr() % 16 == 0
            and _lib.call_int("csk_conv_tile_ok2", B, Ho, Wo, Cin, Cout, xs, Cout, int(bool(up2x))) > 0):
        _lib.call("csk_conv_tile2", _p(out), _p(x), _p(wp), _p(bias), None, None, B, Ho, Wo, Cin, Cout, xs, Cout,
                  0, 0, ACT[act], float(out_scale), 1.0, int(bool(up2x)), 1, _s())
        CONV_TILE_STATS[0] += 1
        return out
    y = conv2d(x, wp, bias, stride, padding, residual, up2x, bias2d, act, out_scale, None, dilation,
               residual2=residual2, res_scale=res_scale)
    out.copy_((y.float().clamp(0, 1) * 255).round().to(torch.uint8))
    return out


def code_ok(act):
    return ACT[act] in (0, 2, 5, 6, 8, 9)


sig("csk_dwconv_tile", c_int)
sig("csk_dwconv", c_void_p, c_void_p, c_void_p, c_int, c_void_p, c_void_p, c_int, c_int, c_int, c_int, c_int, c_int,
    c_int, c_int, c_int, c_int, c_int, c_int, c_int, c_int, c_int, c_int, c_void_p)
sig("csk_dwconv_t", c_void_p, c_void_p, c_void_p, c_int, c_void_p, c_int, c_int, c_int, c_int, c_int, c_int, c_int,
    c_int, c_int, c_int, c_int, c_int, c_int, c_int, c_int, c_int, c_void_p)
DWCONV_TH, DWCONV_TW, DWCONV_CB = 8, 16, 64
DWCONV_VARIANTS = ("direct", "halo")
DWCONV_STATS = [0]


def _dw_variant(kh, kw, stride):
    return "halo" if stride == 1 and kh * kw > 1 else "direct"


def _dw_operand(name, what, t, C):
    if t.dtype != torch.bfloat16:
        raise ValueError(f"{name}: {what} must be bfloat16 on the HIP path, got {t.dtype}")
    ps = _pix_stride(t)
    if ps is None or ps % 8 or ps < C or t.data_ptr() % 16:
        raise ValueError(f"{name}: {what} must be an NHWC tensor or channel slice (last dim contiguous, pixel "
                         f"stride and channel offset multiples of 8), got strides {t.stride()}")
    return ps


def _dw_common(name, x, wp, bias, out, ho, wo):
    B, H, W, C = x.shape
    xs = _dw_operand(name, "x", x, C)
    if not wp.is_cuda or wp.device != x.device or not wp.is_contiguous():
        raise ValueError(f"{name}: wp must be a contiguous tensor on {x.device}")
    if B > 65535:
        raise ValueError(f"{name}: batch {B} > 65535")
    bias_f32 = 0
    if bias is not None:
        if bias.dtype not in (torch.bfloat16, torch.float32) or not bias.is_contiguous() or bias.device != x.device:
            raise ValueError(f"{name}: bias must be contiguous bf16 or fp32 on {x.device}")
        if bias.data_ptr() % 16:
            raise ValueError(f"{name}: bias must be 16-byte aligned")
        bias_f32 = int(bias.dtype == torch.float32)
    if out is None:
        out = torch.empty((B, ho, wo, C), dtype=torch.bfloat16, device=x.device)
    os_ = _dw_operand(name, "out", out, C)
    return xs, os_, bias_f32, out


def depthwise_conv2d(x, wp, bias, stride, pad, pad_mode, residual, out, out_hw, variant=None):
    name = "depthwise_conv2d"
    B, H, W, C = x.shape
    ho, wo = out_hw
    kh, kw = wp.shape[0], wp.shape[1]
    xs, os_, bias_f32, out = _dw_common(name, x, wp, bias, out, ho, wo)
    rs = 0
    if residual is not None:
        rs = _dw_operand(name, "residual", residual, C)
    variant = variant or _dw_variant(kh, kw, stride)
    if variant not in DWCONV_VARIANTS:
        raise ValueError(f"{name}: variant {variant!r} not in {DWCONV_VARIANTS}")
    _lib.call("csk_dwconv", _p(x), _p(wp), _p(bias), bias_f32, _p(residual), _p(out), B, H, W, C, xs, rs, os_, ho, wo,
              kh, kw, int(stride), pad[0], pad[1], int(pad_mode == "reflect"), DWCONV_VARIANTS.index(variant), _s())
    DWCONV_STATS[0] += 1
    return out


def depthwise_conv_transpose2d(x, wp, bias, pad, pad_mode, crop, out, out_hw):
    name = "depthwise_conv_transpose2d"
    B, H, W, C = x.shape
    ho, wo = out_hw
    xs, os_, bias_f32, out = _dw_common(name, x, wp, bias, out, ho, wo)
    pt, pl, pb, pr = pad
    _lib.call("csk_dwconv_t", _p(x), _p(wp), _p(bias), bias_f32, _p(out), B, H, W, C, xs, os_, ho, wo, wp.shape[0],
              wp.shape[1], pt, pl, H + pt + pb, W + pl + pr, int(crop), int(pad_mode == "reflect"), _s())
    DWCONV_STATS[0] += 1
    return out


sig("csk_axpby_nhwc", c_void_p, c_int, c_void_p, c_int, c_void_p, c_int, c_int64, c_int, c_float, c_float, c_int,
    c_void_p)


def axpby_nhwc(x, z, a, b, out, act=None):
    xs, ys = _pix_stride(x), _pix_stride(out)
    zs = _pix_stride(z) if z is not None else 0
    if None in (xs, zs, ys) or (z is not None and x.shape != z.shape) or x.shape != out.shape:
        raise ValueError("axpby_nhwc: operands must be same-shape NHWC views")
    C = x.shape[-1]
    P = x.numel() // C
    if C % 8 or xs % 8 or ys % 8 or zs % 8:
        raise ValueError("axpby_nhwc: channels / pixel strides must be multiples of 8")
    _lib.call("csk_axpby_nhwc", _p(out), ys, _p(x), xs, _p(z), zs, P, C, float(a), float(b), ACT[act], _s())
    return out


def axpby(x, y, a, b, out=None):
    x, y = x.contiguous(), y.contiguous()
    out = torch.empty_like(x) if out is None else out
    _lib.call("csk_axpby", _p(out), _p(x), _p(y), x.numel(), float(a), float(b), _s())
    return out


def group_norm(x, gamma, beta, groups, eps, silu):
    _bf16(x, "group_norm.x")
    x = x.contiguous()
    B, C = x.shape[0], x.shape[-1]
    P = x.numel() // (B * C)
    rows = max(1, 256 // max(1, -(-(C // 8) // (2 if C > 2048 else 1))))
    chunk = max(4 * rows, -(-P * B // GN_TARGET_WG))
    nchunk = -(-P // chunk)
    chunk = -(-P // nchunk)
    bstride = 0
    if gamma.dim() == 2:
        if gamma.shape != (B, C) or beta.shape != (B, C):
            raise ValueError("group_norm: per-sample affine must be [B, C]")
        if gamma.stride(1) != 1 or beta.stride(1) != 1 or gamma.stride(0) != beta.stride(0):
            gamma, beta = gamma.contiguous(), beta.contiguous()
        bstride = gamma.stride(0)
    act = 2 if silu == "gelu" else int(bool(silu))
    y = torch.empty_like(x)
    fused = getattr(x, "_csk_gn", None)
    if fused is not None:
        fpart, seg = fused
        if P % seg == 0 and fpart.numel() == (B * P // seg) * C * 2:
            stat = torch.empty(B * groups * 2, dtype=torch.float32, device=x.device)
            _lib.call("csk_group_norm_part", _p(y), _p(x), None, 0, _p(fpart), seg, _p(stat), _p(gamma), _p(beta),
                      B, P, C, groups, chunk, nchunk, float(eps), act, bstride, _s())
            return y
    part = torch.empty(B * nchunk * groups * 3 + B * groups * 2, dtype=torch.float32, device=x.device)
    _lib.call("csk_group_norm", _p(y), _p(x), None, 0, _p(part), _p(gamma), _p(beta), B, P, C, groups, chunk, nchunk,
              float(eps), act, bstride, _s())
    return y


def group_norm_cat(a, b, gamma, beta, groups, eps, silu):
    sa, sb = getattr(a, "_csk_gn", None), getattr(b, "_csk_gn", None)
    GN_CAT_STATS[1] += 1
    if a.shape[:-1] != b.shape[:-1] or not (a.is_contiguous() and b.is_contiguous()):
        return None
    B, Ca, Cb = a.shape[0], a.shape[-1], b.shape[-1]
    C = Ca + Cb
    P = a.numel() // (B * Ca)
    if Ca % 8 or Cb % 8 or gamma.dim() != 1 or C % groups or C > 4096:
        return None
    rows = max(1, 256 // max(1, -(-(C // 8) // (2 if C > 2048 else 1))))
    chunk = max(4 * rows, -(-P * B // GN_TARGET_WG))
    nchunk = -(-P // chunk)
    chunk = -(-P // nchunk)
    y = torch.empty(a.shape[:-1] + (C,), dtype=torch.bfloat16, device=a.device)
    fused = sa is not None and sb is not None and sa[1] == sb[1] and P % sa[1] == 0
    if fused:
        seg = sa[1]
        nseg = sa[0].numel() // (2 * Ca)
        fused = nseg * 2 * Cb == sb[0].numel()
    if fused:
        stat = torch.empty(B * groups * 2, dtype=torch.float32, device=a.device)
        _lib.call("csk_group_norm_part2", _p(y), _p(a), _p(b), Ca, _p(sa[0]), _p(sb[0]), seg, _p(stat), _p(gamma),
                  _p(beta), B, P, C, groups, chunk, nchunk, float(eps), int(bool(silu)), 0, _s())
    else:
        part = torch.empty(B * nchunk * groups * 3 + B * groups * 2, dtype=torch.float32, device=a.device)
        _lib.call("csk_group_norm", _p(y), _p(a), _p(b), Ca, _p(part), _p(gamma), _p(beta), B, P, C, groups, chunk,
                  nchunk, float(eps), int(bool(silu)), 0, _s())
    GN_CAT_STATS[0] += 1
    return y


GN_CAT_STATS = [0, 0]


def layer_norm(x, gamma, beta, eps):
    _bf16(x, "layer_norm.x")
    x = x.contiguous()
    C = x.shape[-1]
    y = torch.empty_like(x)
    _lib.call("csk_layer_norm", _p(y), _p(x), _p(gamma), _p(beta), x.numel() // C, C, float(eps), _s())
    return y


def attention(q, k, v, scale, causal=False, kv_len=None):
    for t, n in ((q, "q"), (k, "k"), (v, "v")):
        _bf16(t, "attention." + n)
        if t.stride(-1) != 1:
            raise ValueError("attention: last dim must be contiguous")
    B, Sq, H, D = q.shape
    Skv = k.shape[1]
    if D > 512 or (D > 256 and (causal or kv_len is not None or D % 16)):
        raise ValueError(f"attention: head dim {D} unsupported (<= 256, or <= 512 non-causal, multiple of 16)")
    o = torch.empty((B, Sq, H, D), dtype=torch.bfloat16, device=q.device)
    st = (c_int64 * 12)(*q.stride()[:3], *k.stride()[:3], *v.stride()[:3], *o.stride()[:3])
    if kv_len is not None and (kv_len.dtype != torch.int32 or not kv_len.is_cuda):
        raise TypeError("attention: kv_len must be an int32 device tensor")
    plain = not causal and kv_len is None and ATTN_VARIANT == 0
    if plain and attn_fa_ok(B, H, Sq, Skv, D):
        _lib.call("csk_attention_fa", _p(o), _p(q), _p(k), _p(v), st, B, H, Sq, Skv, D, float(scale), ATTN_FA_WORKERS,
                  _s())
        return o
    split = attn_kv_split(B, H, Sq, Skv, D) if plain else 1
    if split > 1:
        return attention_split(q, k, v, scale, split, o)
    _lib.call("csk_attention", _p(o), _p(q), _p(k), _p(v), st, B, H, Sq, Skv, D, float(scale), int(bool(causal)),
              ATTN_VARIANT, _p(kv_len), _s())
    return o


sig("csk_attention_bias", c_void_p, c_void_p, c_void_p, c_void_p, ctypes.POINTER(c_int64), c_int, c_int, c_int, c_int,
    c_int, c_float, c_int, c_void_p, ctypes.POINTER(c_int64), c_void_p, c_void_p)
sig("csk_set_attn_bias_waves", c_int)


def set_attn_bias_waves(n: int):
    _lib.call("csk_set_attn_bias_waves", int(n))


def attention_bias(q, k, v, scale, causal=False, bias=None, kv_lens=None):
    for t, n in ((q, "q"), (k, "k"), (v, "v")):
        _bf16(t, "attention_bias." + n)
        if t.dim() != 4:
            raise ValueError(f"attention_bias.{n}: expected [B, S, H, D], got {tuple(t.shape)}")
        if not t.is_cuda:
            raise TypeError(f"attention_bias.{n}: must be a device tensor")
        if t.stride(-1) != 1:
            raise ValueError("attention_bias: last dim must be contiguous")
    B, Sq, H, D = q.shape
    Skv = k.shape[1]
    if k.shape != (B, Skv, H, D) or v.shape != (B, Skv, H, D):
        raise ValueError(f"attention_bias: k / v {tuple(k.shape)} / {tuple(v.shape)} do not match q {tuple(q.shape)}")
    if bias is not None:
        if bias.dtype != torch.float32 or not bias.is_cuda:
            raise TypeError("attention_bias: bias must be a float32 device tensor")
        if bias.dim() == 0:
            bias = bias.reshape(1)
        full = (B, H, Sq, Skv)
        if bias.dim() > 4 or any(n not in (1, m) for n, m in zip(bias.shape[::-1], full[::-1])):
            raise ValueError(f"attention_bias: bias {tuple(bias.shape)} does not broadcast to {full}")
        if Skv > 1 and (bias.shape[-1] != Skv or bias.stride(-1) != 1):
            bias = bias.expand(*bias.shape[:-1], Skv).contiguous()
        bias = bias.expand(B, H, Sq, Skv)
    if kv_lens is not None:
        if kv_lens.dtype != torch.int32 or not kv_lens.is_cuda:
            raise TypeError("attention_bias: kv_lens must be an int32 device tensor")
        if tuple(kv_lens.shape) != (B,) or kv_lens.stride(0) != 1:
            raise ValueError(f"attention_bias: kv_lens must be a contiguous [B = {B}] tensor, got {tuple(kv_lens.shape)}")
    if D > 128 or D % 8 or D < 8:
        from . import _ref_attention_bias

        return _ref_attention_bias(q, k, v, scale, causal, bias, kv_lens)
    o = torch.empty((B, Sq, H, D), dtype=torch.bfloat16, device=q.device)
    if o.numel() == 0:
        return o
    if Skv == 0:
        return o.zero_()
    st = (c_int64 * 12)(*q.stride()[:3], *k.stride()[:3], *v.stride()[:3], *o.stride()[:3])
    bst = (c_int64 * 3)(*bias.stride()[:3]) if bias is not None else None
    _lib.call("csk_attention_bias", _p(o), _p(q), _p(k), _p(v), st, B, H, Sq, Skv, D, float(scale),
              int(bool(causal)), _p(bias), bst, _p(kv_lens), _s())
    return o


def attention_split(q, k, v, scale, split, o=None):
    B, Sq, H, D = q.shape
    Skv = k.shape[1]
    if D != 64 or not 2 <= split <= 16:
        raise ValueError("attention_split: head dim 64, 2..16 splits")
    if o is None:
        o = torch.empty((B, Sq, H, D), dtype=torch.bfloat16, device=q.device)
    st = (c_int64 * 12)(*q.stride()[:3], *k.stride()[:3], *v.stride()[:3], *o.stride()[:3])
    rows = B * H * Sq
    part_o = torch.empty((split, rows, 64), dtype=torch.float32, device=q.device)
    part_ml = torch.empty((split, rows, 2), dtype=torch.float32, device=q.device)
    _lib.call("csk_attention_split", _p(o), _p(q), _p(k), _p(v), st, B, H, Sq, Skv, D, float(scale), split,
              _p(part_o), _p(part_ml), _s())
    return o


ATTN_FA = os.environ.get("CSK_ATTN_FA", "1") == "1"
ATTN_FA_WORKERS = 0


def attn_fa_ok(B, H, Sq, Skv, D) -> bool:
    return ATTN_FA and _lib.call_int("csk_attn_fa_ok", B, H, Sq, Skv, D, 0, 0) == 1


def set_attn_fa(on: bool):
    global ATTN_FA
    ATTN_FA = bool(on)
    _lib.call("csk_set_attn_fa", int(ATTN_FA))


def attn_fa_errors() -> int:
    out = ctypes.c_uint(0)
    fn = _lib.load().csk_attn_fa_errors
    fn.restype = ctypes.c_int
    err = fn(ctypes.byref(out))
    if err:
        raise RuntimeError(f"csk_attn_fa_errors: hipError {err}")
    return int(out.value)


sig("csk_attn_fa_reset")


def attn_fa_health() -> bool:
    if attn_fa_errors() == 0:
        return True
    set_attn_fa(False)
    _lib.call("csk_attn_fa_reset")
    return False


ATTN32 = True


def set_attn32(on: bool):
    global ATTN32
    ATTN32 = bool(on)
    _lib.call("csk_set_attn32", int(ATTN32))


ATTN_SPLIT_WG = int(os.environ.get("CSK_ATTN_SPLIT_WG", "1024"))


def attn_kv_split(B, H, Sq, Skv, D) -> int:
    if D != 64 or Skv <= 128 or ATTN_SPLIT_WG <= 0 or not ATTN32:
        return 1
    wg = B * H * -(-Sq // 128)
    split = 1
    while wg * split < ATTN_SPLIT_WG and split < 4 and -(-Skv // 64) >= 32 * split:
        split *= 2
    return split


def silu(x):
    _bf16(x, "silu")
    x = x.contiguous()
    y = torch.empty_like(x)
    _lib.call("csk_silu", _p(y), _p(x), x.numel(), _s())
    return y


def row_bcast(dst, tab, cur):
    _bf16(dst, "row_bcast.dst")
    _bf16(tab, "row_bcast.tab")
    if dst.dim() != 2 or tab.dim() != 2 or dst.shape[1] != tab.shape[1] or not dst.is_contiguous() \
            or not tab.is_contiguous() or cur.dtype != torch.int32:
        raise ValueError("row_bcast: contiguous bf16 [rows, W] / [n, W], int32 cur")
    _lib.call("csk_row_bcast", _p(dst), _p(tab), _p(cur), dst.shape[0], dst.shape[1], tab.shape[0], _s())


def dup2(x):
    x = x.contiguous()
    y = torch.empty((2 * x.shape[0],) + tuple(x.shape[1:]), dtype=x.dtype, device=x.device)
    if x.dtype != torch.bfloat16 or x.numel() % 8 or x.data_ptr() % 16:
        y[: x.shape[0]].copy_(x)
        y[x.shape[0]:].copy_(x)
        return y
    _lib.call("csk_dup2", _p(y), _p(x), x.numel(), _s())
    return y


def add(x, y):
    _bf16(x, "add")
    if x.shape != y.shape:
        raise ValueError(f"hip add: shapes {tuple(x.shape)} and {tuple(y.shape)} differ (no broadcasting)")
    x, y = x.contiguous(), y.contiguous().to(x.dtype)
    out = torch.empty_like(x)
    _lib.call("csk_add", _p(out), _p(x), _p(y), x.numel(), _s())
    return out


def sched_step(e, x, prev_x0, c, guidance, noise):
    _bf16(e, "sched_step.e")
    x = x.contiguous()
    n = x.numel()
    cfg = guidance is not None
    if e.numel() != n * (2 if cfg else 1):
        raise ValueError("sched_step: model output / latent size mismatch")
    xn = torch.empty_like(x)
    x0 = torch.empty_like(x)
    _lib.call("csk_sched_step", _p(xn), _p(x0), _p(e.contiguous()), _p(x),
              _p(prev_x0) if (prev_x0 is not None and c.C != 0.0) else None,
              _p(noise) if (noise is not None and c.D != 0.0) else None, n,
              float(c.p), float(c.q), float(c.A), float(c.B), float(c.C), float(c.D),
              float(guidance or 0.0), int(cfg), _s())
    return xn, x0


def loop_prologue(counter, cur, t_tab, t_out):
    if counter.dtype != torch.int32 or cur.dtype != torch.int32 or t_tab.dtype != torch.float32 \
            or t_out.dtype != torch.float32 or t_tab.numel() < 1:
        raise TypeError("loop_prologue: int32 counter/cur, fp32 t_tab/t_out")
    _lib.call("csk_loop_prologue", _p(counter), _p(cur), _p(t_tab), _p(t_out), t_tab.numel(), _s())


def sched_loop(e, x, x0prev, noise_tab, cur, coef, x_in, mode, reps=None):
    _bf16(e, "sched_loop.e")
    _bf16(x_in, "sched_loop.x_in")
    nrep = mode + 1
    reps = nrep if reps is None else int(reps)
    B, H, W, C = x.shape
    if C != 4 or x.dtype != torch.float32 or not x.is_contiguous() or not x0prev.is_contiguous() \
            or x0prev.shape != x.shape or x0prev.dtype != torch.float32:
        raise ValueError("sched_loop: x / x0prev must be contiguous fp32 [B, H, W, 4]")
    if e.numel() != nrep * x.numel() or not e.is_contiguous():
        raise ValueError(f"sched_loop: model output {tuple(e.shape)} vs {nrep} x {tuple(x.shape)}")
    if x_in.dim() != 4 or x_in.shape[0] != reps * B or x_in.shape[1:3] != (H, W) or x_in.shape[3] < 4 \
            or not x_in.is_contiguous():
        raise ValueError(f"sched_loop: x_in {tuple(x_in.shape)} for {reps} x {tuple(x.shape)}")
    if coef.dtype != torch.float32 or coef.dim() != 2 or coef.shape[1] != LOOP_COEF_STRIDE \
            or cur.dtype != torch.int32:
        raise ValueError("sched_loop: coef must be fp32 [n, LOOP_COEF_STRIDE], cur int32")
    if noise_tab is not None and (noise_tab.dtype != torch.float32 or
                                  noise_tab.numel() != coef.shape[0] * x.numel()):
        raise ValueError("sched_loop: noise table must be fp32 [n, B, H, W, 4]")
    _lib.call("csk_sched_loop", _p(e), _p(x), _p(x0prev), _p(noise_tab), _p(cur), _p(coef), _p(x_in),
              x_in.shape[3], reps, B * H * W, mode, _s())


def vae_postprocess(img):
    _bf16(img, "vae_post")
    img = img.contiguous()
    y = torch.empty(img.shape, dtype=torch.uint8, device=img.device)
    _lib.call("csk_vae_post", _p(y), _p(img), img.numel(), _s())
    return y


def canny(img, low, high):
    if img.dtype != torch.uint8 or img.dim() not in (2, 3):
        raise TypeError("canny: uint8 [H, W] or [H, W, C] expected")
    img = img.contiguous()
    H, W = img.shape[:2]
    C = 1 if img.dim() == 2 else img.shape[2]
    out = torch.empty((H, W), dtype=torch.uint8, device=img.device)
    a4, a1 = -(-(H * W * 4) // 256) * 256, -(-(H * W) // 256) * 256
    ws = torch.empty(256 + a4 + 2 * a1, dtype=torch.uint8, device=img.device)
    _lib.call("csk_canny", _p(out), _p(img), H, W, C, float(low), float(high), _p(ws), _s())
    return out


XATTN_FUSED = os.environ.get("CSK_XATTN", "1") == "1"
XATTN_CHANNELS = (320,)
XATTN_WAVES = int(os.environ.get("CSK_XATTN_WAVES", "8"))
_xattn_waves_applied = [None]


XATTN_MIN_WG = int(os.environ.get("CSK_XATTN_MIN_WG", "256"))


def xattn_ok(x, kv, rows_per_b) -> bool:
    C = x.shape[-1]
    if x.numel() // max(C, 1) // 128 < XATTN_MIN_WG:
        return False
    return (XATTN_FUSED and C in XATTN_CHANNELS and kv is not None and kv.dim() == 5 and kv.shape[2] == 2
            and kv.shape[3] * kv.shape[4] == C and kv.shape[4] == 64 and 1 <= kv.shape[1] <= 80
            and rows_per_b % 128 == 0 and x.numel() // C % rows_per_b == 0
            and kv.shape[0] >= x.numel() // C // rows_per_b)


def xattn_block(x, wq, colsum, bq, kv, wo, bo, eps, scale, rows_per_b, row_stats=True):
    for t, n in ((x, "x"), (wq, "wq"), (bq, "bq"), (kv, "kv"), (wo, "wo")):
        _bf16(t, "xattn_block." + n)
    if bo is not None:
        _bf16(bo, "xattn_block.bo")
    C = x.shape[-1]
    M = x.numel() // C
    x2 = x.reshape(M, C)
    if not x2.is_contiguous():
        x2 = x2.contiguous()
    kv = kv.contiguous()
    if colsum.dtype != torch.float32 or colsum.numel() != C:
        raise ValueError("xattn_block: colsum must be fp32 [C]")
    y = torch.empty((M, C), dtype=torch.bfloat16, device=x.device)
    rp = torch.empty(M * 2, dtype=torch.float32, device=x.device) if row_stats else None
    if _xattn_waves_applied[0] != XATTN_WAVES:
        _lib.call("csk_set_xattn_waves", int(XATTN_WAVES))
        _xattn_waves_applied[0] = XATTN_WAVES
    _lib.call("csk_xattn_block", _p(y), _p(x2), _p(wq.contiguous()), _p(colsum.contiguous()), _p(bq.contiguous()),
              _p(kv), _p(wo.contiguous()), _p(None if bo is None else bo.contiguous()), _p(rp), M, C, int(rows_per_b),
              int(kv.shape[0]), int(kv.shape[1]), float(eps), float(scale), _s())
    out = y.view(x.shape)
    if rp is not None:
        out._csk_rows = (rp, 1, C)
    return out


sig("csk_ff_geglu_ok", c_int, c_int, c_int)
sig("csk_ff_geglu", c_void_p, c_void_p, c_void_p, c_void_p, c_void_p, c_void_p, c_void_p, c_void_p, c_int, c_int,
    c_int, c_float, c_void_p)
sig("csk_set_ff_probe", c_int)
FF_MIN_ROWS = int(os.environ.get("CSK_FF_MIN_ROWS", "16384"))
FF_FUSED = os.environ.get("CSK_FF_FUSED", "1") == "1"


def ff_fused_ok(x, inner: int) -> bool:
    C = x.shape[-1]
    M = x.numel() // C
    return (FF_FUSED and x.dtype == torch.bfloat16 and M >= FF_MIN_ROWS
            and _lib.call_int("csk_ff_geglu_ok", M, C, inner) == 1)


def ff_geglu(x, gamma, beta, w1p, b1p, w2p, b2, eps):
    for t, n in ((x, "x"), (gamma, "gamma"), (w1p, "w1p"), (w2p, "w2p")):
        _bf16(t, "ff_geglu." + n)
    C = x.shape[-1]
    M = x.numel() // C
    inner = 32 * w2p.shape[0]
    x2 = x.reshape(M, C)
    if not x2.is_contiguous():
        x2 = x2.contiguous()
    y = torch.empty((M, C), dtype=torch.bfloat16, device=x.device)
    if beta is not None:
        _bf16(beta, "ff_geglu.beta")
    if b2 is not None:
        _bf16(b2, "ff_geglu.b2")
    if b1p is not None and b1p.dtype != torch.float32:
        raise ValueError("ff_geglu: b1p must be fp32")
    _lib.call("csk_ff_geglu", _p(y), _p(x2), _p(gamma.contiguous()), _p(None if beta is None else beta.contiguous()),
              _p(w1p.contiguous()), _p(None if b1p is None else b1p.contiguous()), _p(w2p.contiguous()),
              _p(None if b2 is None else b2.contiguous()), M, C, inner, float(eps), _s())
    return y.view(x.shape)


sig("csk_set_xattn_probe", c_int)
sig("csk_set_xattn_waves", c_int)


sig("csk_xin_qkv_ok", c_int, c_int, c_int, c_int)
sig("csk_xin_qkv", c_void_p, c_void_p, c_void_p, c_void_p, c_void_p, c_void_p, c_int, c_void_p, c_void_p, c_void_p,
    c_void_p, c_int, c_int, c_float, c_void_p)
sig("csk_set_xin_probe", c_int)
sig("csk_set_conv_tile_no_rw", c_int)
sig("csk_gn_finalize", c_void_p, c_void_p, c_void_p, c_int, c_int, c_int, c_int, c_int, c_int, c_float, c_void_p)
XIN_FUSED = os.environ.get("CSK_XIN_FUSED", "1") == "1"
XIN_MIN_ROWS = int(os.environ.get("CSK_XIN_MIN_ROWS", "16384"))


def gn_stats(x, groups, eps):
    fused = getattr(x, "_csk_gn", None)
    if fused is None:
        return None
    B, C = x.shape[0], x.shape[-1]
    P = x.numel() // (B * C)
    part, seg = fused
    if P % seg or part.numel() != (B * P // seg) * C * 2 or C % groups:
        return None
    stat = torch.empty((B, groups, 2), dtype=torch.float32, device=x.device)
    _lib.call("csk_gn_finalize", _p(stat), _p(part), None, 0, seg, B, P, C, groups, float(eps), _s())
    return stat


def xin_ok(x, groups) -> bool:
    if not XIN_FUSED or x.dtype != torch.bfloat16 or getattr(x, "_csk_gn", None) is None:
        return False
    B, C = x.shape[0], x.shape[-1]
    M = x.numel() // C
    return M >= XIN_MIN_ROWS and _lib.call_int("csk_xin_qkv_ok", M, C, M // B, groups) == 1


def xin_qkv(x, stat, gamma, beta, w, bi, colsum, bq, eps):
    _bf16(x, "xin.x")
    _bf16(w, "xin.w")
    _bf16(gamma, "xin.gamma")
    B, C = x.shape[0], x.shape[-1]
    M = x.numel() // C
    x2 = x.reshape(M, C)
    if not x2.is_contiguous():
        x2 = x2.contiguous()
    for t, n in ((bi, "bi"), (colsum, "colsum"), (bq, "bq"), (stat, "stat")):
        if t is not None and (t.dtype != torch.float32 or not t.is_contiguous()):
            raise ValueError(f"xin_qkv: {n} must be contiguous fp32")
    if beta is not None:
        _bf16(beta, "xin.beta")
    h = torch.empty((M, C), dtype=torch.bfloat16, device=x.device)
    qkv = torch.empty((M, 3 * C), dtype=torch.bfloat16, device=x.device)
    _lib.call("csk_xin_qkv", _p(h), _p(qkv), _p(x2), _p(stat), _p(gamma.contiguous()),
              _p(None if beta is None else beta.contiguous()), stat.shape[1], _p(w.contiguous()), _p(bi), _p(colsum),
              _p(bq), M, M // B, float(eps), _s())
    return h, qkv


sig("csk_gemv", c_void_p, c_void_p, c_void_p, c_void_p, c_void_p, c_void_p, c_void_p, c_int, c_int, c_int, c_int,
    c_int, c_int, c_int, c_int, c_float, c_void_p)
sig("csk_gemv_ex", c_void_p, c_void_p, c_void_p, c_void_p, c_void_p, c_void_p, c_void_p, c_void_p, c_int, c_int,
    c_int, c_int, c_int, c_int, c_int, c_int, c_int, c_int, c_float, c_void_p)
sig("csk_gemv_plan", c_int)
sig("csk_set_gemv_nt", c_int)
sig("csk_attention_decode", c_void_p, c_void_p, c_void_p, c_void_p, c_void_p, c_void_p, ctypes.POINTER(c_int64),
    c_int, c_int, c_int, c_int, c_float, c_void_p, c_void_p, c_void_p, c_void_p)
sig("csk_attention_decode_ex", c_void_p, c_void_p, c_void_p, c_void_p, c_void_p, c_void_p, ctypes.POINTER(c_int64),
    c_int, c_int, c_int, c_int, c_int, c_float, c_void_p, c_void_p, c_void_p, c_void_p, c_void_p, c_int, c_void_p)
sig("csk_attn_decode_split")
DECODE = os.environ.get("CSK_DECODE", "1") == "1"
DECODE_STATS = {"gemv": 0, "decode_attention": 0, "gemv_glu": 0}
GEMV_NORM_NONE, GEMV_NORM_LN, GEMV_NORM_RMS = 0, 1, 2
GEMV_MAX_M = 8
GEMV_LDS_FLOATS = 32768
DECODE_SPLIT = 64
DECODE_HEAD_DIMS = (32, 64, 128)
_DECODE_WS: dict = {}


def set_decode(on: bool):
    global DECODE
    DECODE = bool(on)


def set_gemv_nt(on: bool):
    _lib.call("csk_set_gemv_nt", int(bool(on)))


def _aligned_rows(t, single_row_ok=False):
    return (t.stride(1) == 1 and t.data_ptr() % 16 == 0
            and (t.stride(0) % 8 == 0 or (single_row_ok and t.shape[0] == 1)))


def rms_norm(x, gamma, eps):
    from . import _ref_rms_norm

    return _ref_rms_norm(x, gamma, eps).to(x.dtype)


def _gemv_kernel_takes(M, K):
    mt = 1 if M <= 1 else 2 if M <= 2 else 4 if M <= 4 else 8
    return DECODE and 1 <= M <= GEMV_MAX_M and K % 8 == 0 and K >= 8 and mt * K <= GEMV_LDS_FLOATS


def _gemv_norm(ln, rms, K):
    if ln is None and rms is None:
        return GEMV_NORM_NONE, None, None, 0.0
    if ln is not None:
        mode, (gamma, beta, eps), what = GEMV_NORM_LN, ln, "LayerNorm"
    else:
        mode, (gamma, eps), beta, what = GEMV_NORM_RMS, rms, None, "RMSNorm"
    _bf16(gamma, "gemv.gamma")
    if gamma.numel() != K or (beta is not None and beta.numel() != K):
        raise ValueError(f"gemv: {what} affine of {gamma.numel()} elements for K = {K}")
    gamma = gamma.contiguous()
    if gamma.data_ptr() % 16:
        gamma = gamma.clone()
    if beta is not None:
        _bf16(beta, "gemv.beta")
        beta = beta.contiguous()
        if beta.data_ptr() % 16:
            beta = beta.clone()
    return mode, gamma, beta, float(eps)


def gemv(x2, w, bias=None, act=None, residual=None, ln=None, out=None, rms=None):
    _bf16(x2, "gemv.x")
    _bf16(w, "gemv.w")
    M, K = x2.shape
    N = w.shape[0]
    if w.shape[1] != K:
        raise ValueError(f"gemv: K mismatch {tuple(x2.shape)} x {tuple(w.shape)}")
    code = ACT[act]
    if not _gemv_kernel_takes(M, K) or code == 3:
        if ln is not None:
            x2 = layer_norm(x2, ln[0], ln[1], ln[2])
        elif rms is not None:
            x2 = rms_norm(x2, rms[0], rms[1])
        y = gemm(x2, w, bias, residual, act, out=out if out is not None and out.is_contiguous() else None)
        if out is not None and y is not out:
            out.copy_(y)
            return out
        return y
    if not _aligned_rows(x2, single_row_ok=True):
        x2 = x2.contiguous()
    if not _aligned_rows(w):
        w = w.contiguous()
    if out is None:
        out = torch.empty((M, N), dtype=torch.bfloat16, device=x2.device)
    elif out.shape != (M, N) or out.dtype != torch.bfloat16 or out.stride(1) != 1 or out.device != x2.device:
        raise ValueError(f"gemv: out must be a bf16 [{M}, {N}] view with a contiguous last dim")
    ldr = 0
    if residual is not None:
        _bf16(residual, "gemv.residual")
        residual = residual.reshape(M, N)
        if residual.stride(1) != 1:
            residual = residual.contiguous()
        ldr = residual.stride(0)
    if bias is not None:
        _bf16(bias, "gemv.bias")
        bias = bias.contiguous()
    mode, gamma, beta, eps = _gemv_norm(ln, rms, K)
    _lib.call("csk_gemv_ex", _p(out), _p(x2), _p(w), None, _p(bias), _p(residual), _p(gamma), _p(beta), mode, M, N, K,
              x2.stride(0), w.stride(0), 0, ldr, out.stride(0), code, eps, _s())
    DECODE_STATS["gemv"] += 1
    return out


def gemv_glu(x2, wg, wu, act="silu", rms=None, ln=None, out=None):
    _bf16(x2, "gemv_glu.x")
    _bf16(wg, "gemv_glu.w_gate")
    _bf16(wu, "gemv_glu.w_up")
    M, K = x2.shape
    N = wg.shape[0]
    if wg.shape != wu.shape or wg.shape[1] != K:
        raise ValueError(f"gemv_glu: shapes {tuple(x2.shape)} x {tuple(wg.shape)} / {tuple(wu.shape)}")
    code = ACT[act]
    if code == 3:
        raise ValueError("gemv_glu: act is the gate's pointwise activation, not 'geglu'")
    if out is not None and (out.shape != (M, N) or out.dtype != torch.bfloat16 or out.stride(1) != 1
                            or out.device != x2.device):
        raise ValueError(f"gemv_glu: out must be a bf16 [{M}, {N}] view with a contiguous last dim")
    if not _gemv_kernel_takes(M, K):
        if ln is not None:
            x2 = layer_norm(x2, ln[0], ln[1], ln[2])
        elif rms is not None:
            x2 = rms_norm(x2, rms[0], rms[1])
        y = gemm(x2, wg, None, None, act) * gemm(x2, wu, None, None, None)
        if out is not None:
            out.copy_(y)
            return out
        return y
    if not _aligned_rows(x2, single_row_ok=True):
        x2 = x2.contiguous()
    if not _aligned_rows(wg):
        wg = wg.contiguous()
    if not _aligned_rows(wu):
        wu = wu.contiguous()
    if out is None:
        out = torch.empty((M, N), dtype=torch.bfloat16, device=x2.device)
    mode, gamma, beta, eps = _gemv_norm(ln, rms, K)
    _lib.call("csk_gemv_ex", _p(out), _p(x2), _p(wg), _p(wu), None, None, _p(gamma), _p(beta), mode, M, N, K,
              x2.stride(0), wg.stride(0), wu.stride(0), 0, out.stride(0), code, eps, _s())
    DECODE_STATS["gemv_glu"] += 1
    return out


def gemv_plan(N):
    v = _lib.call_int("csk_gemv_plan", int(N))
    return v // 16, v % 16


def _decode_ws(device, B, H, S, D):
    key = (device, B, H, S, D)
    ws = _DECODE_WS.get(key)
    if ws is None:
        nsplit = -(-S // DECODE_SPLIT)
        ws = (torch.zeros(B * H * nsplit * (D + 2), dtype=torch.float32, device=device),
              torch.zeros(B * H, dtype=torch.int32, device=device))
        _DECODE_WS[key] = ws
    return ws


def decode_attention(q, kc, vc, scale, kv_len, k_new=None, v_new=None, pos=None, rope=None):
    for t, n in ((q, "q"), (kc, "k_cache"), (vc, "v_cache"), (k_new, "k_new"), (v_new, "v_new")):
        if t is not None:
            _bf16(t, "decode_attention." + n)
            if t.stride(-1) != 1:
                raise ValueError("decode_attention: last dim must be contiguous")
    B, _, H, D = q.shape
    S, Hkv = kc.shape[1], kc.shape[2]
    cos = sin = None
    if rope is not None:
        cos, sin = rope
        for t in (cos, sin):
            if t.dtype != torch.float32 or t.device != q.device or t.dim() != 2 or t.shape[1] != D // 2 \
                    or t.shape[0] < S or not t.is_contiguous():
                raise ValueError(f"decode_attention: rope tables must be contiguous fp32 [P >= {S}, {D // 2}] on "
                                 f"the device of q, got {tuple(t.shape)} {t.dtype}")

    def vec_ok(t):
        return t is None or (t.data_ptr() % 16 == 0 and all(s % 8 == 0 for s in t.stride()[:3]))

    if (not DECODE or D not in DECODE_HEAD_DIMS or B * H > 65535 or not (vec_ok(kc) and vec_ok(vc))
            or (cos is not None and (cos.data_ptr() % 16 or sin.data_ptr() % 16))):
        if (k_new is not None or rope is not None) and pos is None:
            pos = (kv_len.to(torch.long) - 1).clamp_(0, S - 1)
        if rope is not None:
            from . import _ref_rope

            c, s = cos.index_select(0, pos), sin.index_select(0, pos)
            q = _ref_rope(q, c, s).to(q.dtype)
            if k_new is not None:
                k_new = _ref_rope(k_new, c, s).to(k_new.dtype)
        if k_new is not None:
            kc.index_copy_(1, pos, k_new)
            vc.index_copy_(1, pos, v_new)
        if Hkv != H:
            kc, vc = (t[:, :, :, None].expand(B, S, Hkv, H // Hkv, D).reshape(B, S, H, D) for t in (kc, vc))
        return attention(q, kc, vc, scale, kv_len=kv_len)
    if not vec_ok(q):
        q = q.contiguous()
    if not vec_ok(k_new):
        k_new = k_new.contiguous()
    if not vec_ok(v_new):
        v_new = v_new.contiguous()
    o = torch.empty((B, 1, H, D), dtype=torch.bfloat16, device=q.device)
    ws, cnt = _decode_ws(q.device, B, H, S, D)

    def bh(t):
        return (t.stride(0), t.stride(2)) if t is not None else (0, 0)

    st = (c_int64 * 14)(*bh(q), *kc.stride()[:3], *vc.stride()[:3], *bh(k_new), *bh(v_new), *bh(o))
    _lib.call("csk_attention_decode_ex", _p(o), _p(q), _p(kc), _p(vc), _p(k_new), _p(v_new), st, B, H, Hkv, S, D,
              float(scale), _p(kv_len), _p(ws), _p(cnt), _p(cos), _p(sin), 0 if cos is None else cos.shape[0], _s())
    DECODE_STATS["decode_attention"] += 1
    return o
```

csrc/kernels/ff.hip:

```cpp
#include "common.h"

#include "attn_tile.h"

typedef __attribute__((address_space(1))) const void* ff_gptr_t;
typedef __attribute__((address_space(3))) void* ff_lptr_t;

struct FfArgs {
  const bf16_t* x;
  const bf16_t* gamma;
  const bf16_t* beta;
  const bf16_t* w1;
  const float* b1;
  const bf16_t* w2;
  const bf16_t* b2;
  bf16_t* y;
  const bf16_t* x_end;
  const bf16_t* w1_end;
  const bf16_t* w2_end;
  int M, I;
  float eps;
};

#define FF_WAVES 4
#define FF_ROWS (32 * FF_WAVES)
#define FF_SLOT 10240
#define FF_NSLOT 7
#define FF_PIECES (FF_SLOT / 512)
#define FF_PPW (FF_PIECES / FF_WAVES)
#define FF_IMAX 1280

template <int N>
__device__ __forceinline__ void ff_vmcnt() {
  asm volatile("s_waitcnt vmcnt(%0)" ::"n"(N) : "memory");
}

__device__ __forceinline__ void ff_ld(v8s& d, unsigned addr) {
  asm volatile("ds_read_b128 %0, %1" : "=v"(d) : "v"(addr));
}
__device__ __forceinline__ void ff_ldf(v4f& d, unsigned addr) {
  asm volatile("ds_read_b128 %0, %1" : "=v"(d) : "v"(addr));
}
__device__ __forceinline__ void ff_wait(int n, v8s& d) {
  switch (n) {
    case 0: asm volatile("s_waitcnt lgkmcnt(0)" : "+v"(d)); break;
    case 1: asm volatile("s_waitcnt lgkmcnt(1)" : "+v"(d)); break;
    case 2: asm volatile("s_waitcnt lgkmcnt(2)" : "+v"(d)); break;
    case 3: asm volatile("s_waitcnt lgkmcnt(3)" : "+v"(d)); break;
    case 4: asm volatile("s_waitcnt lgkmcnt(4)" : "+v"(d)); break;
    case 5: asm volatile("s_waitcnt lgkmcnt(5)" : "+v"(d)); break;
    case 6: asm volatile("s_waitcnt lgkmcnt(6)" : "+v"(d)); break;
    default: asm volatile("s_waitcnt lgkmcnt(7)" : "+v"(d)); break;
  }
}
template <int N>
__device__ __forceinline__ void ff_waitf(v4f (&b)[4]) {
  asm volatile("s_waitcnt lgkmcnt(%4)" : "+v"(b[0]), "+v"(b[1]), "+v"(b[2]), "+v"(b[3]) : "n"(N));
}

template <int C, int PROBE = 0>
__global__ __launch_bounds__(FF_WAVES * 64, 1) void ff_geglu_kernel(const FfArgs a) {
  constexpr int KS = C / 16;
  constexpr int NOT = C / 32;
  constexpr int SI = C / 64;
  static_assert(32 * C == FF_SLOT && 32 * C == NOT * 1024, "one W1 tile / one W2 slice per slot");
  static_assert(FF_PIECES % FF_WAVES == 0, "pieces per wave");
  __shared__ __attribute__((aligned(16))) bf16_t ring[FF_NSLOT * FF_SLOT];
  __shared__ __attribute__((aligned(16))) float s_b1[2 * FF_IMAX];

  const int tid = threadIdx.x, lane = tid & 63;
  const int wid = __builtin_amdgcn_readfirstlane(tid >> 6);
  const int r32 = lane & 31, h = lane >> 5;
  const int m0 = blockIdx.x * FF_ROWS;
  const int row = m0 + wid * 32 + r32;
  const bool row_ok = row < a.M;
  const int I = a.I;
  const int nchunk = I / 32;
  const int nslots = 3 * nchunk;

  auto dma_piece = [&](int t, int i) {
    bf16_t* base = ring + (t % FF_NSLOT) * FF_SLOT;
    const int c = t / 3, kind = t - 3 * c;
    const int p = wid + FF_WAVES * i;
    const bf16_t* src = (kind < 2 ? a.w1 + (size_t)(2 * c + kind) * FF_SLOT : a.w2 + (size_t)c * FF_SLOT) +
                        512 * p + 8 * lane;
    CSK_DCHECK(src + 8 <= (kind < 2 ? a.w1_end : a.w2_end), 91, t, I);
    __builtin_amdgcn_global_load_lds((ff_gptr_t)src, (ff_lptr_t)(base + 512 * p), 16, 0, 0);
  };
  auto dma_slot = [&](int t) {
#pragma unroll
    for (int i = 0; i < FF_PPW; ++i) dma_piece(t, i);
  };

  constexpr int LEAD = FF_NSLOT - 2;
  uint4 xu[KS];
#pragma unroll
  for (int ks = 0; ks < KS; ++ks) {
    xu[ks] = make_uint4(0, 0, 0, 0);
    if (row_ok) {
      CSK_DCHECK(a.x + (size_t)row * C + 16 * ks + 8 * h + 8 <= a.x_end, 93, row, a.M);
      xu[ks] = *reinterpret_cast<const uint4*>(a.x + (size_t)row * C + 16 * ks + 8 * h);
    }
  }
  uint4 gmu[KS], btu[KS];
#pragma unroll
  for (int ks = 0; ks < KS; ++ks) {
    gmu[ks] = *reinterpret_cast<const uint4*>(a.gamma + 16 * ks + 8 * h);
    btu[ks] = a.beta ? *reinterpret_cast<const uint4*>(a.beta + 16 * ks + 8 * h) : make_uint4(0, 0, 0, 0);
  }
  for (int i = tid; i < 2 * I; i += FF_WAVES * 64) s_b1[i] = a.b1 ? a.b1[i] : 0.f;
  for (int t = 0; t < LEAD && t < nslots; ++t) dma_slot(t);

  v8s xf[KS];
  float mean = 0.f, rstd = 0.f;
  {
    float f[KS][8];
#pragma unroll
    for (int ks = 0; ks < KS; ++ks) unpack8(xu[ks], f[ks]);
    float s = 0.f;
#pragma unroll
    for (int ks = 0; ks < KS; ++ks)
#pragma unroll
      for (int j = 0; j < 8; ++j) s += f[ks][j];
    s += __shfl_xor(s, 32, 64);
    mean = s * (1.0f / C);
    float q = 0.f;
#pragma unroll
    for (int ks = 0; ks < KS; ++ks)
#pragma unroll
      for (int j = 0; j < 8; ++j) {
        const float d = f[ks][j] - mean;
        q = __builtin_fmaf(d, d, q);
      }
    q += __shfl_xor(q, 32, 64);
    rstd = rsqrtf(q * (1.0f / C) + a.eps);
#pragma unroll
    for (int ks = 0; ks < KS; ++ks) {
      float gm[8], bt[8];
      unpack8(gmu[ks], gm);
      unpack8(btu[ks], bt);
      float v[8];
#pragma unroll
      for (int j = 0; j < 8; ++j) v[j] = __builtin_fmaf((f[ks][j] - mean) * rstd, gm[j], bt[j]);
      xf[ks] = __builtin_bit_cast(v8s, pack8(v));
    }
  }

  v16f out[NOT];
#pragma unroll
  for (int o = 0; o < NOT; ++o)
#pragma unroll
    for (int i = 0; i < 16; ++i) out[o][i] = 0.f;

  auto enter_pair = [&](int t) {
    if constexpr ((PROBE & 4) == 0) {
      if (t + 4 < nslots) ff_vmcnt<FF_PPW * 3>();
      else ff_vmcnt<0>();
    } else {
      ff_vmcnt<0>();
    }
    asm volatile("s_waitcnt lgkmcnt(0)" ::: "memory");
    __builtin_amdgcn_s_barrier();
    asm volatile("" ::: "memory");
  };
  auto dma_hook = [&](int t, int k) {
    if constexpr ((PROBE & 4) == 0) {
      if ((k & 3) == 3 && t + 5 < nslots) dma_piece(t + 5, k >> 2);
    }
  };

  const unsigned ring0 = (unsigned)(size_t)(ff_lptr_t)(void*)ring;
  const unsigned b1base = (unsigned)(size_t)(ff_lptr_t)(void*)s_b1 + (unsigned)(16 * h);
  unsigned w1o[4];
#pragma unroll
  for (int j = 0; j < 4; ++j) w1o[j] = 2u * (unsigned)at_off64(r32, 2 * j + h);
  unsigned w2o[2];
#pragma unroll
  for (int s2 = 0; s2 < 2; ++s2) w2o[s2] = 2u * (unsigned)(r32 * 32 + (((2 * s2 + h) ^ ((r32 >> 2) & 3)) << 3));
  auto slot_base = [&](int t) -> unsigned {
    return ring0 + (unsigned)(((PROBE & 4) ? (t % 3) : (t % FF_NSLOT)) * FF_SLOT * 2);
  };
  constexpr int D = 6;
  constexpr int GAT = 2;

  auto geglu = [&](v16f& acc, v4f (&bq)[4]) -> v8s {
    asm volatile("" : "+v"(bq[0]), "+v"(bq[1]), "+v"(bq[2]), "+v"(bq[3]));
    mfma_fence16(acc, acc);
    float hv[8];
#pragma unroll
    for (int j = 0; j < 8; ++j) {
      const float v = acc[j] + bq[j >> 2][j & 3];
      const float g = acc[j + 8] + bq[2 + (j >> 2)][j & 3];
      if constexpr ((PROBE & 2) != 0) hv[j] = v + g;
      else hv[j] = v * gelu_geglu(g);
    }
    return __builtin_bit_cast(v8s, pack8(hv));
  };

  auto w1_tile = [&](int t, int tt, v16f& acc, v4f (&bq)[4], v16f* pacc, v4f (*pbq)[4], v8s* pout) {
    const unsigned sb = slot_base(t);
#pragma unroll
    for (int q = 0; q < 4; ++q) ff_ldf(bq[q], b1base + (unsigned)((tt * 32 + 8 * q) * 4));
    v8s wf[KS];
#pragma unroll
    for (int ks = 0; ks < D; ++ks) ff_ld(wf[ks], sb + w1o[ks & 3] + (unsigned)((ks >> 2) * 4096));
#pragma unroll
    for (int i = 0; i < 16; ++i) acc[i] = 0.f;
#pragma unroll
    for (int ks = 0; ks < KS; ++ks) {
      ff_wait(ks + D - 1 < KS ? D - 1 : KS - 1 - ks, wf[ks]);
      if constexpr ((PROBE & 1) != 0) asm volatile("" ::"v"(wf[ks]), "v"(xf[ks]));
      else acc = __builtin_amdgcn_mfma_f32_32x32x16_bf16(wf[ks], xf[ks], acc, 0, 0, 0);
      if (ks + D < KS) {
        const int k1 = ks + D;
        ff_ld(wf[k1], sb + w1o[k1 & 3] + (unsigned)((k1 >> 2) * 4096));
      }
      dma_hook(t, ks);
      if (ks == GAT && pacc) *pout = geglu(*pacc, *pbq);
    }
  };

  auto w2_slice = [&](int t, const v8s& ha, v16f& acc_b, v4f (&bqb)[4]) {
    const unsigned sb = slot_base(t);
    constexpr int NR = 2 * NOT;
    v8s wf[NR];
    v8s hb;
#pragma unroll
    for (int i = 0; i < D; ++i) ff_ld(wf[i], sb + w2o[i / NOT] + (unsigned)((i % NOT) * 2048));
#pragma unroll
    for (int i = 0; i < NR; ++i) {
      ff_wait(i + D - 1 < NR ? D - 1 : NR - 1 - i, wf[i]);
      const int o = i % NOT;
      if constexpr ((PROBE & 1) != 0) asm volatile("" ::"v"(wf[i]), "v"(ha), "v"(hb));
      else out[o] = __builtin_amdgcn_mfma_f32_32x32x16_bf16(wf[i], i < NOT ? ha : hb, out[o], 0, 0, 0);
      if (i + D < NR) {
        const int i1 = i + D;
        ff_ld(wf[i1], sb + w2o[i1 / NOT] + (unsigned)((i1 % NOT) * 2048));
      }
      dma_hook(t, i);
      if (i == GAT) hb = geglu(acc_b, bqb);
    }
  };

  for (int c = 0; c < nchunk; c += 2) {
    const int t = 3 * c;
    v16f acc_a, acc_b;
    v4f bqa[4], bqb[4];
    v8s ha;
    enter_pair(t);
    w1_tile(t, 2 * c, acc_a, bqa, nullptr, nullptr, nullptr);
    w1_tile(t + 1, 2 * c + 1, acc_b, bqb, &acc_a, &bqa, &ha);
    enter_pair(t + 2);
    w2_slice(t + 2, ha, acc_b, bqb);
    w1_tile(t + 3, 2 * c + 2, acc_a, bqa, nullptr, nullptr, nullptr);
    enter_pair(t + 4);
    w1_tile(t + 4, 2 * c + 3, acc_b, bqb, &acc_a, &bqa, &ha);
    w2_slice(t + 5, ha, acc_b, bqb);
  }

  if (!row_ok) return;
  uint2 xr[NOT][4], br[NOT][4];
#pragma unroll
  for (int o = 0; o < NOT; ++o)
#pragma unroll
    for (int q = 0; q < 4; ++q) {
      const int n = 32 * o + 8 * q + 4 * h;
      xr[o][q] = *reinterpret_cast<const uint2*>(a.x + (size_t)row * C + n);
      br[o][q] = a.b2 ? *reinterpret_cast<const uint2*>(a.b2 + n) : make_uint2(0, 0);
    }
#pragma unroll
  for (int o = 0; o < NOT; ++o)
#pragma unroll
    for (int q = 0; q < 4; ++q) {
      const int n = 32 * o + 8 * q + 4 * h;
      const uint2 u = xr[o][q], ub = br[o][q];
      const float rv[4] = {bf2f((bf16_t)(u.x & 0xffff)), bf2f((bf16_t)(u.x >> 16)), bf2f((bf16_t)(u.y & 0xffff)),
                           bf2f((bf16_t)(u.y >> 16))};
      const float bb[4] = {bf2f((bf16_t)(ub.x & 0xffff)), bf2f((bf16_t)(ub.x >> 16)), bf2f((bf16_t)(ub.y & 0xffff)),
                           bf2f((bf16_t)(ub.y >> 16))};
      uint2 w;
      w.x = pack2(out[o][4 * q] + bb[0] + rv[0], out[o][4 * q + 1] + bb[1] + rv[1]);
      w.y = pack2(out[o][4 * q + 2] + bb[2] + rv[2], out[o][4 * q + 3] + bb[3] + rv[3]);
      *reinterpret_cast<uint2*>(a.y + (size_t)row * C + n) = w;
    }
}

CSK_DEBUG_EXPORT(ff)

static int g_ff_probe = 0;
CSK_API int csk_set_ff_probe(int p) {
  g_ff_probe = p;
  return 0;
}

CSK_API int csk_ff_geglu_ok(int M, int C, int I) {
  return (C == 320 && I > 0 && I % 64 == 0 && I <= FF_IMAX && M > 0) ? 1 : 0;
}

CSK_API int csk_ff_geglu(void* y, const void* x, const void* gamma, const void* beta, const void* w1, const void* b1,
                         const void* w2, const void* b2, int M, int C, int I, float eps, hipStream_t stream) {
  if (!csk_ff_geglu_ok(M, C, I) || !x || !y || !gamma || !w1 || !w2 || x == y) return (int)hipErrorInvalidValue;
  FfArgs a;
  a.x = (const bf16_t*)x;
  a.gamma = (const bf16_t*)gamma;
  a.beta = (const bf16_t*)beta;
  a.w1 = (const bf16_t*)w1;
  a.b1 = (const float*)b1;
  a.w2 = (const bf16_t*)w2;
  a.b2 = (const bf16_t*)b2;
  a.y = (bf16_t*)y;
  a.x_end = a.x + (size_t)M * C;
  a.w1_end = a.w1 + (size_t)2 * I * C;
  a.w2_end = a.w2 + (size_t)C * I;
  a.M = M;
  a.I = I;
  a.eps = eps;
  const dim3 grid((M + FF_ROWS - 1) / FF_ROWS);
  switch (g_ff_probe) {
    case 1: ff_geglu_kernel<320, 1><<<grid, FF_WAVES * 64, 0, stream>>>(a); break;
    case 2: ff_geglu_kernel<320, 2><<<grid, FF_WAVES * 64, 0, stream>>>(a); break;
    case 4: ff_geglu_kernel<320, 4><<<grid, FF_WAVES * 64, 0, stream>>>(a); break;
    default: ff_geglu_kernel<320><<<grid, FF_WAVES * 64, 0, stream>>>(a); break;
  }
  return (int)hipGetLastError();
}
```

csrc/kernels/xattn.hip:

```cpp
#include "attn_tile.h"

typedef __attribute__((address_space(1))) const void* xa_gptr_t;
typedef __attribute__((address_space(3))) void* xa_lptr_t;

struct XattnArgs {
  const bf16_t* x;
  const bf16_t* wq;
  const float* colsum;
  const bf16_t* bq;
  const bf16_t* kv;
  const bf16_t* wo;
  const bf16_t* bo;
  bf16_t* y;
  float* row_part;
  const bf16_t* zero;
  const bf16_t* x_end;
  const bf16_t* kv_end;
  int M, rows_per_b, Skv;
  float eps, scale_log2;
};

#define XA_BM 128
#define XA_KVR 96

template <int N>
__device__ __forceinline__ void xa_vmcnt() {
  asm volatile("s_waitcnt vmcnt(%0)" ::"n"(N) : "memory");
}

__device__ __forceinline__ void xa_dma(const bf16_t* src, bf16_t* dst) {
  __builtin_amdgcn_global_load_lds((xa_gptr_t)src, (xa_lptr_t)dst, 16, 0, 0);
}
__device__ __forceinline__ void xa_dma_off(const bf16_t* base, unsigned off, bf16_t* dst) {
  xa_dma(base + off, dst);
}

__device__ __forceinline__ int xa_off64(int r, int c) { return at_off64(r, c); }
__device__ __forceinline__ v8s xa_pack8(const v4f& lo, const v4f& hi, float s) { return at_pack8(lo, hi, s); }

template <int C, int NW, int RT, int PROBE = 0>
__global__ __launch_bounds__(NW * 64, 1) void xattn_block_kernel(const XattnArgs a) {
  constexpr int H = C / 64, NCS = C / 32, NNT = C / 16, CPR = C / 8;
  constexpr int WQ = 64 * C, WO = C * 64, KVI = XA_KVR * 64;
  constexpr int WQ_PIECES = WQ / 512, WO_PIECES = WO / 512, KV_PIECES = 2 * KVI / 512;
  static_assert(WQ_PIECES % NW == 0 && WO_PIECES % NW == 0 && KV_PIECES % NW == 0, "pieces per wave");
  static_assert(NW * RT * 16 == XA_BM, "workgroup rows");
  constexpr int NWQ = WQ_PIECES / NW, NWO = WO_PIECES / NW, NKV = KV_PIECES / NW;
  __shared__ __attribute__((aligned(16))) bf16_t s_wq[WQ];
  __shared__ __attribute__((aligned(16))) bf16_t s_wo[WO];
  __shared__ __attribute__((aligned(16))) bf16_t s_kv0[2 * KVI];
  __shared__ __attribute__((aligned(16))) bf16_t s_kv1[2 * KVI];
  __shared__ __attribute__((aligned(16))) float s_cb[2 * C];

  const int tid = threadIdx.x, lane = tid & 63;
  const int wid = __builtin_amdgcn_readfirstlane(tid >> 6);
  const int fr = lane & 15, g = lane >> 4;
  const int m0 = xcd_remap(blockIdx.x, gridDim.x) * XA_BM;
  const int b = m0 / a.rows_per_b;
  const int Skv = a.Skv;
  const int row_w = m0 + wid * (RT * 16);

  auto dma_wq = [&](int h) {
#pragma unroll
    for (int i = 0; i < NWQ; ++i) {
      const int p = wid + NW * i;
      const int f = 64 * p + lane, row = f / CPR, slot = f % CPR;
      CSK_DCHECK(h * 64 + row < C, 71, row, C);
      xa_dma_off(a.wq, (unsigned)((h * 64 + row) * C + 8 * (slot ^ (row & 7))), s_wq + 512 * p);
    }
  };
  auto dma_wo = [&](int h) {
#pragma unroll
    for (int i = 0; i < NWO; ++i) {
      const int p = wid + NW * i;
      const int row = 8 * p + (lane >> 3), slot = lane & 7;
      CSK_DCHECK(row < C, 72, row, C);
      xa_dma_off(a.wo, (unsigned)(row * C + h * 64 + 8 * (slot ^ at_key(row))), s_wo + 512 * p);
    }
  };
  auto dma_kv = [&](int h, bf16_t* dst) {
#pragma unroll
    for (int i = 0; i < NKV; ++i) {
      const int p = wid + NW * i;
      const int which = p >= KV_PIECES / 2;
      const int row = 8 * (p - which * (KV_PIECES / 2)) + (lane >> 3), slot = lane & 7;
      const int rr = min(row, Skv - 1);
      const unsigned off = (unsigned)(((b * Skv + rr) * 2 + which) * (H * 64) + h * 64 + 8 * (slot ^ at_key(row)));
      CSK_DCHECK(a.kv + off + 8 <= a.kv_end, 73, row, Skv);
      xa_dma_off(a.kv, off, dst + 512 * p);
    }
  };

  for (int i = tid; i < C; i += NW * 64) {
    s_cb[i] = a.colsum[i];
    s_cb[C + i] = bf2f(a.bq[i]);
  }
  dma_wq(0);
  dma_wo(0);
  dma_kv(0, s_kv0);
  v8s xf[RT][NCS];
#pragma unroll
  for (int rt = 0; rt < RT; ++rt) {
    const int m = row_w + rt * 16 + fr;
#pragma unroll
    for (int cs = 0; cs < NCS; ++cs) {
      uint4 u = make_uint4(0, 0, 0, 0);
      if (m < a.M) {
        CSK_DCHECK(a.x + (size_t)m * C + 32 * cs + 8 * g + 8 <= a.x_end, 74, m, a.M);
        u = *reinterpret_cast<const uint4*>(a.x + (size_t)m * C + 32 * cs + 8 * g);
      }
      xf[rt][cs] = __builtin_bit_cast(v8s, u);
    }
  }
  float mean[RT], rstd[RT];
#pragma unroll
  for (int rt = 0; rt < RT; ++rt) {
    float s = 0.f;
#pragma unroll
    for (int cs = 0; cs < NCS; ++cs) {
      float f[8];
      unpack8(__builtin_bit_cast(uint4, xf[rt][cs]), f);
#pragma unroll
      for (int j = 0; j < 8; ++j) s += f[j];
    }
    s += __shfl_xor(s, 16, 64);
    s += __shfl_xor(s, 32, 64);
    mean[rt] = s * (1.0f / C);
    float q = 0.f;
#pragma unroll
    for (int cs = 0; cs < NCS; ++cs) {
      float f[8];
      unpack8(__builtin_bit_cast(uint4, xf[rt][cs]), f);
#pragma unroll
      for (int j = 0; j < 8; ++j) {
        const float d = f[j] - mean[rt];
        q = __builtin_fmaf(d, d, q);
      }
    }
    q += __shfl_xor(q, 16, 64);
    q += __shfl_xor(q, 32, 64);
    rstd[rt] = rsqrtf(q * (1.0f / C) + a.eps);
  }

  v4f out[RT][NNT];
#pragma unroll
  for (int rt = 0; rt < RT; ++rt)
#pragma unroll
    for (int nt = 0; nt < NNT; ++nt) out[rt][nt] = v4f{0.f, 0.f, 0.f, 0.f};

  xa_vmcnt<0>();
  __syncthreads();

  const float sl2 = a.scale_log2;
  for (int h = 0; h < H; ++h) {
    const int cur = h & 1;
    const bool more = h + 1 < H;
    if (more && (PROBE & 8) == 0) {
      if (cur) dma_kv(h + 1, s_kv0);
      else dma_kv(h + 1, s_kv1);
    }

    v4f qa[RT][4];
#pragma unroll
    for (int rt = 0; rt < RT; ++rt)
#pragma unroll
      for (int dt = 0; dt < 4; ++dt) qa[rt][dt] = v4f{0.f, 0.f, 0.f, 0.f};
    auto ld_wq = [&](int cs, v8s (&wf)[4]) {
#pragma unroll
      for (int dt = 0; dt < 4; ++dt) {
        const int r = 16 * dt + fr;
        wf[dt] = *reinterpret_cast<const v8s*>(s_wq + r * C + 8 * ((4 * cs + g) ^ (r & 7)));
      }
    };
    v8s wf[2][4];
    ld_wq(0, wf[0]);
#pragma unroll
    for (int cs = 0; cs < NCS; ++cs) {
      if (cs + 1 < NCS) ld_wq(cs + 1, wf[(cs + 1) & 1]);
#pragma unroll
      for (int rt = 0; rt < RT; ++rt)
#pragma unroll
        for (int dt = 0; dt < 4; ++dt) {
          if constexpr ((PROBE & 1) != 0) asm volatile("" ::"v"(wf[cs & 1][dt]), "v"(xf[rt][cs]));
          else qa[rt][dt] = __builtin_amdgcn_mfma_f32_16x16x32_bf16(wf[cs & 1][dt], xf[rt][cs], qa[rt][dt], 0, 0, 0);
        }
      asm volatile("" ::: "memory");
    }
    asm volatile("s_waitcnt lgkmcnt(0)" ::: "memory");
    __builtin_amdgcn_s_barrier();
    if (more && (PROBE & 8) == 0) dma_wq(h + 1);

    v8s qf[RT][2];
    {
      v4f cw[4], bw[4];
#pragma unroll
      for (int dt = 0; dt < 4; ++dt) {
        const int d = h * 64 + 16 * dt + 4 * g;
        cw[dt] = *reinterpret_cast<const v4f*>(s_cb + d);
        bw[dt] = *reinterpret_cast<const v4f*>(s_cb + C + d);
      }
#pragma unroll
      for (int rt = 0; rt < RT; ++rt) {
        v4f qv[4];
#pragma unroll
        for (int dt = 0; dt < 4; ++dt)
#pragma unroll
          for (int r = 0; r < 4; ++r)
            qv[dt][r] = __builtin_fmaf(rstd[rt], qa[rt][dt][r] - mean[rt] * cw[dt][r], bw[dt][r]);
        qf[rt][0] = xa_pack8(qv[0], qv[1], sl2);
        qf[rt][1] = xa_pack8(qv[2], qv[3], sl2);
      }
    }

    v8s of[RT][2];
    auto attend = [&](const bf16_t* ks) {
#pragma unroll
      for (int rt = 0; rt < RT; ++rt) {
        v4f o[4];
        float inv;
        at_attend_rowtile(ks, ks + KVI, qf[rt], Skv, o, inv);
        of[rt][0] = xa_pack8(o[0], o[1], inv);
        of[rt][1] = xa_pack8(o[2], o[3], inv);
      }
    };
    if constexpr ((PROBE & 2) != 0) {
      for (int rt = 0; rt < RT; ++rt) {
        of[rt][0] = qf[rt][0];
        of[rt][1] = qf[rt][1];
      }
    } else {
      if (cur) attend(s_kv1);
      else attend(s_kv0);
    }
    if (more && (PROBE & 8) == 0) xa_vmcnt<NKV + NWQ>();
    else xa_vmcnt<0>();
    __builtin_amdgcn_s_barrier();

    v8s wof[2][2];
    wof[0][0] = at_perm_frag(s_wo, fr, 4 * g);
    wof[0][1] = at_perm_frag(s_wo, fr, 32 + 4 * g);
#pragma unroll
    for (int nt = 0; nt < NNT; ++nt) {
      if (nt + 1 < NNT) {
        wof[(nt + 1) & 1][0] = at_perm_frag(s_wo, 16 * (nt + 1) + fr, 4 * g);
        wof[(nt + 1) & 1][1] = at_perm_frag(s_wo, 16 * (nt + 1) + fr, 32 + 4 * g);
      }
#pragma unroll
      for (int ds = 0; ds < 2; ++ds)
#pragma unroll
        for (int rt = 0; rt < RT; ++rt) {
          if constexpr ((PROBE & 4) != 0) asm volatile("" ::"v"(wof[nt & 1][ds]), "v"(of[rt][ds]));
          else out[rt][nt] = __builtin_amdgcn_mfma_f32_16x16x32_bf16(wof[nt & 1][ds], of[rt][ds], out[rt][nt], 0, 0, 0);
        }
      asm volatile("" ::: "memory");
    }
    xa_vmcnt<0>();
    asm volatile("s_waitcnt lgkmcnt(0)" ::: "memory");
    __builtin_amdgcn_s_barrier();
    if (more && (PROBE & 8) == 0) dma_wo(h + 1);
  }

  uint2 xres[RT][NNT], bres[NNT];
#pragma unroll
  for (int nt = 0; nt < NNT; ++nt) {
    bres[nt] = make_uint2(0, 0);
    if (a.bo) bres[nt] = *reinterpret_cast<const uint2*>(a.bo + 16 * nt + 4 * g);
  }
#pragma unroll
  for (int rt = 0; rt < RT; ++rt) {
    const int m = row_w + rt * 16 + fr;
#pragma unroll
    for (int nt = 0; nt < NNT; ++nt) {
      xres[rt][nt] = make_uint2(0, 0);
      if (m < a.M) xres[rt][nt] = *reinterpret_cast<const uint2*>(a.x + (size_t)m * C + 16 * nt + 4 * g);
    }
  }
#pragma unroll
  for (int rt = 0; rt < RT; ++rt) {
    const int m = row_w + rt * 16 + fr;
    const bool ok = m < a.M;
    float s = 0.f;
#pragma unroll
    for (int nt = 0; nt < NNT; ++nt) {
      const int n = 16 * nt + 4 * g;
      const uint2 u = xres[rt][nt];
      const uint2 ub = bres[nt];
      float rv[4] = {bf2f((bf16_t)(u.x & 0xffff)), bf2f((bf16_t)(u.x >> 16)), bf2f((bf16_t)(u.y & 0xffff)),
                     bf2f((bf16_t)(u.y >> 16))};
      const float bov[4] = {bf2f((bf16_t)(ub.x & 0xffff)), bf2f((bf16_t)(ub.x >> 16)), bf2f((bf16_t)(ub.y & 0xffff)),
                            bf2f((bf16_t)(ub.y >> 16))};
#pragma unroll
      for (int r = 0; r < 4; ++r) {
        const float v = bf2f(f2bf(out[rt][nt][r] + bov[r] + rv[r]));
        out[rt][nt][r] = v;
        s += v;
      }
      if (ok) {
        uint2 w;
        w.x = pack2(out[rt][nt][0], out[rt][nt][1]);
        w.y = pack2(out[rt][nt][2], out[rt][nt][3]);
        *reinterpret_cast<uint2*>(a.y + (size_t)m * C + n) = w;
      }
    }
    if (a.row_part) {
      s += __shfl_xor(s, 16, 64);
      s += __shfl_xor(s, 32, 64);
      const float mu = s * (1.0f / C);
      float q = 0.f;
#pragma unroll
      for (int nt = 0; nt < NNT; ++nt)
#pragma unroll
        for (int r = 0; r < 4; ++r) {
          const float d = out[rt][nt][r] - mu;
          q = __builtin_fmaf(d, d, q);
        }
      q += __shfl_xor(q, 16, 64);
      q += __shfl_xor(q, 32, 64);
      if (ok && g == 0) *reinterpret_cast<float2*>(a.row_part + (size_t)m * 2) = make_float2(mu, q);
    }
  }
}

CSK_DEBUG_EXPORT(xattn)

static int g_xattn_probe = 0;
static int g_xattn_waves = 8;
CSK_API int csk_set_xattn_probe(int p) {
  g_xattn_probe = p;
  return 0;
}
CSK_API int csk_set_xattn_waves(int w) {
  if (w != 4 && w != 8) return (int)hipErrorInvalidValue;
  g_xattn_waves = w;
  return 0;
}

template <int C, int NW, int RT>
static void xattn_launch(const XattnArgs& a, dim3 grid, hipStream_t stream) {
  switch (g_xattn_probe) {
    case 1: xattn_block_kernel<C, NW, RT, 1><<<grid, NW * 64, 0, stream>>>(a); break;
    case 2: xattn_block_kernel<C, NW, RT, 2><<<grid, NW * 64, 0, stream>>>(a); break;
    case 4: xattn_block_kernel<C, NW, RT, 4><<<grid, NW * 64, 0, stream>>>(a); break;
    case 8: xattn_block_kernel<C, NW, RT, 8><<<grid, NW * 64, 0, stream>>>(a); break;
    case 15: xattn_block_kernel<C, NW, RT, 15><<<grid, NW * 64, 0, stream>>>(a); break;
    default: xattn_block_kernel<C, NW, RT><<<grid, NW * 64, 0, stream>>>(a); break;
  }
}

const bf16_t* csk_zero_ptr();

CSK_API int csk_xattn_block(void* y, const void* x, const void* wq, const void* colsum, const void* bq,
                            const void* kv, const void* wo, const void* bo, void* row_part, int M, int C,
                            int rows_per_b, int Bc, int Skv, float eps, float scale, hipStream_t stream) {
  if (!csk_zero_ptr()) return (int)hipErrorNotInitialized;
  if (Skv < 1 || Skv > 80 || rows_per_b % XA_BM != 0 || M % rows_per_b != 0 || M / rows_per_b > Bc)
    return (int)hipErrorInvalidValue;
  XattnArgs a;
  a.x = (const bf16_t*)x;
  a.wq = (const bf16_t*)wq;
  a.colsum = (const float*)colsum;
  a.bq = (const bf16_t*)bq;
  a.kv = (const bf16_t*)kv;
  a.wo = (const bf16_t*)wo;
  a.bo = (const bf16_t*)bo;
  a.y = (bf16_t*)y;
  a.row_part = (float*)row_part;
  a.zero = csk_zero_ptr();
  a.x_end = a.x + (size_t)M * C;
  a.kv_end = a.kv + (size_t)Bc * Skv * 2 * C;
  a.M = M;
  a.rows_per_b = rows_per_b;
  a.Skv = Skv;
  a.eps = eps;
  a.scale_log2 = scale * 1.4426950408889634f;
  const dim3 grid((M + XA_BM - 1) / XA_BM);
  switch (C) {
    case 320:
      if (g_xattn_waves == 8) xattn_launch<320, 8, 1>(a, grid, stream);
      else xattn_launch<320, 4, 2>(a, grid, stream);
      break;
    default: return (int)hipErrorInvalidValue;
  }
  return (int)hipGetLastError();
}
```

Before: 7.596 images/s.

## Fuse self-attn out-projection into cross-attn block and proj_out into FF kernel

In 320-channel transformer blocks, the self-attention output projection plus residual is computed as a prologue inside the fused cross-attention kernel, and can broadcast rows for the CFG duplicate batch. This removes a separate GEMM launch and the write and re-read of the intermediate hidden state. The last block's feed-forward kernel also folds in the Transformer2D proj_out linear and its residual, which drops another GEMM launch and round trip. In exchange the kernels hold more registers and do more staging through LDS (the Wo1 slices reuse the s_wq/s_wo buffers), and occupancy or scheduling may suffer.

```diff
diff --git a/chiaswarm_amd/models/layers.py b/chiaswarm_amd/models/layers.py
--- a/chiaswarm_amd/models/layers.py
+++ b/chiaswarm_amd/models/layers.py
@@ -164,7 +164,7 @@
             return self.attend_q(self.to_q(x), kv, ctx if ctx is not None else x, residual)
         return self.attend_qkv(ops.gemm(x, self.w_qkv, self.b_qkv), residual, causal=causal)
 
-    def attend_qkv(self, qkv, residual=None, causal=False, row_stats=False):
+    def attend_qkv(self, qkv, residual=None, causal=False, row_stats=False, project=True):
         b, s, _ = qkv.shape
         h, d = self.heads, self.dim_head
         qkv = qkv.view(b, s, 3, h, d)
@@ -173,6 +173,8 @@
             q, k = qkv[:, :, 0].float().transpose(1, 2), qkv[:, :, 1].float().transpose(1, 2)
             store.append(torch.softmax(q @ k.transpose(-1, -2) * self.scale, dim=-1))
         o = ops.attention(qkv[:, :, 0], qkv[:, :, 1], qkv[:, :, 2], self.scale, causal=causal)
+        if not project:
+            return o.reshape(b, s, h * d)
         return self.to_out[0](o.reshape(b, s, h * d), residual=residual, row_stats=row_stats)
 
     def attend_q(self, q, kv, ctx, residual=None, row_stats=False):
@@ -266,7 +268,7 @@
             folds[name] = f
         return f[1]
 
-    def forward(self, x, ctx=None, kv=None, row_stats=None, dup=False, qkv=None):
+    def forward(self, x, ctx=None, kv=None, row_stats=None, dup=False, qkv=None, tail=None):
         hip = ops.row_stats_wanted(x)
         if row_stats is None:
             row_stats = hip
@@ -276,6 +278,18 @@
             fus = ops.ln_fusable(x)
             qkv = ops.layer_norm_gemm(x, self.norm1, a1.w_qkv, a1.b_qkv,
                                       self._fold("qkv", a1.w_qkv, a1.b_qkv, self.norm1) if fus else None)
+        if hip and kv is not None and x.dim() == 3 and ops.xattn_pre_fusable(x, kv, x.shape[1], dup):
+            f = self._fold("q", a2.to_q.weight, a2.to_q.bias, self.norm2)
+            hit = self.__dict__.get("_q_perm")
+            if hit is None or hit[0] is not f:
+                hit = (f, ops.permute_xattn_q(f[0]))
+                self.__dict__["_q_perm"] = hit
+            o = a1.attend_qkv(qkv, project=False)
+            x = ops.xattn_block(None, hit[1], f[1], f[2], kv, a2.to_out[0].weight, a2.to_out[0].bias, self.norm2.eps,
+                                a2.scale, x.shape[1], row_stats=hip,
+                                pre=(o, x, a1.to_out[0].weight, a1.to_out[0].bias),
+                                batch=(2 if dup else 1) * x.shape[0])
+            return self._ff_tail(x, row_stats, hip, tail)
         x = a1.attend_qkv(qkv, residual=x, row_stats=hip)
         if hip and not dup and kv is not None and x.dim() == 3 and ops.xattn_fusable(x, kv, x.shape[1]):
             w2, colsum, b2 = self._fold("q", a2.to_q.weight, a2.to_q.bias, self.norm2)
@@ -294,17 +308,28 @@
             if dup:
                 q, x = ops.dup2(q), ops.dup2(x)
             x = a2.attend_q(q, kv, ctx if ctx is not None else x, residual=x, row_stats=hip)
+        return self._ff_tail(x, row_stats, hip, tail)
+
+    def _ff_tail(self, x, row_stats, hip, tail):
+        ff = self.ff
         if hip and not row_stats and ops.ff_fusable(x, ff.inner):
             w1p, b1p, w2p = ff.fused_weights()
+            seg = ops.ff_proj_fusable(x, ff.inner, tail[3]) if tail is not None and w1p is not None else 0
+            if seg:
+                wpp, bp, xin, gn_rows = tail
+                return ops.ff_fused_proj(x, self.norm3.weight, self.norm3.bias, w1p, b1p, w2p, ff.net[2].bias, wpp, bp,
+                                         xin, self.norm3.eps, gn_rows, seg), True
             if w1p is not None:
-                return ops.ff_fused(x, self.norm3.weight, self.norm3.bias, w1p, b1p, w2p, ff.net[2].bias,
-                                    self.norm3.eps)
+                y = ops.ff_fused(x, self.norm3.weight, self.norm3.bias, w1p, b1p, w2p, ff.net[2].bias,
+                                 self.norm3.eps)
+                return y if tail is None else (y, False)
         g = ff.net[0]
         g.ensure()
         fus = ops.ln_fusable(x)
         hdn = ops.layer_norm_gemm(x, self.norm3, g.wp, g.bp, self._fold("ff", g.wp, g.bp, self.norm3) if fus else None,
                                   act="geglu")
-        return ff.net[2](hdn, residual=x, row_stats=row_stats)
+        y = ff.net[2](hdn, residual=x, row_stats=row_stats)
+        return y if tail is None else (y, False)
 
 
 class Transformer2D(nn.Module):
@@ -340,6 +365,21 @@
             hit = (key, ops.pack_xin_qkv(wi.detach().reshape(c, c), None if self.proj_in.bias is None
                                          else self.proj_in.bias.detach(), w2, colsum, b2))
             self.__dict__["_xin"] = hit
+        return hit[1]
+
+    def _proj_tail(self, x):
+        po = self.proj_out
+        c = x.shape[-1]
+        if (not isinstance(po, Linear) or not self.transformer_blocks or c != 320 or tuple(po.weight.shape) != (c, c)
+                or x.dtype != torch.bfloat16 or po.weight.dtype != torch.bfloat16 or not x.is_contiguous()
+                or not ops.row_stats_wanted(x)):
+            return None
+        w = po.weight
+        key = (w.data_ptr(), w._version, w.device, w.dtype)
+        hit = self.__dict__.get("_ffproj")
+        if hit is None or hit[0] != key:
+            hit = (key, ops.pack_ff_proj(w.detach()))
+            self.__dict__["_ffproj"] = hit
         return hit[1]
 
     def _xin_ok(self, x) -> bool:
@@ -369,14 +409,18 @@
             if rows is not None:
                 h._csk_rows = rows
         nb = len(self.transformer_blocks)
+        wpp = self._proj_tail(x)
         for i, blk in enumerate(self.transformer_blocks):
-            if dup and i == 0:
-                h = blk(h, ctx=ctx, kv=None if kvs is None else kvs[i], row_stats=hip and i + 1 < nb, dup=True,
-                        qkv=qkv0)
+            d = dup and i == 0
+            if d:
                 x, b = ops.dup2(x), 2 * b
-                continue
-            h = blk(h, ctx=ctx, kv=None if kvs is None else kvs[i], row_stats=hip and i + 1 < nb,
-                    qkv=qkv0 if i == 0 else None)
+            tail = (wpp, self.proj_out.bias, x, hh * ww) if wpp is not None and i + 1 == nb else None
+            h = blk(h, ctx=ctx, kv=None if kvs is None else kvs[i], row_stats=hip and i + 1 < nb, dup=d,
+                    qkv=qkv0 if i == 0 else None, tail=tail)
+            if tail is not None:
+                h, done = h
+                if done:
+                    return h
         if isinstance(self.proj_out, Linear):
             return ops.gemm(h.view(b, hh, ww, c), self.proj_out.weight, self.proj_out.bias, residual=x,
                             gn_rows=hh * ww)
diff --git a/chiaswarm_amd/ops/__init__.py b/chiaswarm_amd/ops/__init__.py
--- a/chiaswarm_amd/ops/__init__.py
+++ b/chiaswarm_amd/ops/__init__.py
@@ -206,27 +206,38 @@
     b1p = None
     if b1 is not None:
         b1p = torch.stack((b1[:inner].reshape(t, 16), b1[inner:].reshape(t, 16)), 1).reshape(t, 32).float()
+    return w1p.contiguous(), (None if b1p is None else b1p.contiguous()), _pack_ff_w2(w2)
+
+
+def _pack_ff_w2(w2):
+    c, inner = w2.shape
+    _, k4 = _ff_keys(w2.device)
     perm = torch.tensor(_FF_PERM, device=w2.device)
-    w2q = w2.reshape(c, t, 16).index_select(2, perm).reshape(c // 32, 32, inner // 32, 4, 8)
+    w2q = w2.reshape(c, inner // 16, 16).index_select(2, perm).reshape(c // 32, 32, inner // 32, 4, 8)
     w2p = torch.gather(w2q, 3, k4[None, :, None, :, None].expand(c // 32, 32, inner // 32, 4, 8))
-    w2p = w2p.permute(2, 0, 1, 3, 4).reshape(inner // 32, c // 32, 32, 32)
-    return w1p.contiguous(), (None if b1p is None else b1p.contiguous()), w2p.contiguous()
+    return w2p.permute(2, 0, 1, 3, 4).reshape(inner // 32, c // 32, 32, 32).contiguous()
+
+
+def _unpack_ff_w2(w2p):
+    nc, no = w2p.shape[0], w2p.shape[1]
+    c, inner = 32 * no, 32 * nc
+    _, k4 = _ff_keys(w2p.device)
+    inv4 = torch.argsort(k4, 1)
+    y = w2p.reshape(nc, no, 32, 4, 8).permute(1, 2, 0, 3, 4)
+    y = torch.gather(y, 3, inv4[None, :, None, :, None].expand(no, 32, nc, 4, 8)).reshape(c, inner // 16, 16)
+    return y[:, :, torch.argsort(torch.tensor(_FF_PERM, device=w2p.device))].reshape(c, inner)
 
 
 def unpack_ff_fused(w1p, b1p, w2p):
     t, si = w1p.shape[0], w1p.shape[1]
     c, inner = 64 * si, 16 * t
-    k8, k4 = _ff_keys(w1p.device)
-    inv8, inv4 = torch.argsort(k8, 1), torch.argsort(k4, 1)
+    k8, _ = _ff_keys(w1p.device)
+    inv8 = torch.argsort(k8, 1)
     x = w1p.reshape(t, si, 32, 8, 8).permute(0, 2, 1, 3, 4)
     x = torch.gather(x, 3, inv8[None, :, None, :, None].expand(t, 32, si, 8, 8)).reshape(t, 32, c)
     w1 = torch.cat((x[:, :16].reshape(inner, c), x[:, 16:].reshape(inner, c)), 0)
     b1 = None if b1p is None else torch.cat((b1p[:, :16].reshape(inner), b1p[:, 16:].reshape(inner)), 0)
-    nc, no = w2p.shape[0], w2p.shape[1]
-    y = w2p.reshape(nc, no, 32, 4, 8).permute(1, 2, 0, 3, 4)
-    y = torch.gather(y, 3, inv4[None, :, None, :, None].expand(no, 32, nc, 4, 8)).reshape(c, inner // 16, 16)
-    w2 = y[:, :, torch.argsort(torch.tensor(_FF_PERM, device=w2p.device))].reshape(c, inner)
-    return w1, b1, w2
+    return w1, b1, _unpack_ff_w2(w2p)
 
 
 def ff_fusable(x: torch.Tensor, inner: int) -> bool:
@@ -254,6 +265,38 @@
     hid = vg[..., :inner] * torch.nn.functional.gelu(vg[..., inner:])
     y = torch.nn.functional.linear(hid, w2.float(), None if b2 is None else b2.float())
     return (xf + y).to(x.dtype)
+
+
+def pack_ff_proj(wp):
+    c = wp.shape[0]
+    return _pack_ff_w2(wp.reshape(c, c))
+
+
+def unpack_ff_proj(wpp):
+    return _unpack_ff_w2(wpp)
+
+
+def ff_proj_fusable(x: torch.Tensor, inner: int, gn_rows: int) -> int:
+    if not use_hip(x) or x.dim() != 3:
+        return 0
+    from . import hip_ops
+
+    return hip_ops.ff_proj_ok(x, inner, gn_rows)
+
+
+def ff_fused_proj(x, gamma, beta, w1p, b1p, w2p, b2, wpp, bp, xin, eps, gn_rows=0, seg=0):
+    if use_hip(x):
+        from . import hip_ops
+
+        return hip_ops.ff_geglu_proj(x, gamma, beta, w1p, b1p, w2p, b2, wpp, bp, xin, eps, gn_rows, seg)
+    return _ref_ff_fused_proj(x, gamma, beta, w1p, b1p, w2p, b2, wpp, bp, xin, eps)
+
+
+def _ref_ff_fused_proj(x, gamma, beta, w1p, b1p, w2p, b2, wpp, bp, xin, eps):
+    wp = unpack_ff_proj(wpp)
+    y = _ref_ff_fused(x.float(), gamma, beta, w1p, b1p, w2p, b2, eps)
+    z = torch.nn.functional.linear(y, wp.float(), None if bp is None else bp.float())
+    return (xin.float() + z.reshape(xin.shape)).to(x.dtype)
 
 
 def _a_tiles(w):
@@ -334,15 +377,48 @@
     return hip_ops.xattn_ok(x, kv, rows_per_b)
 
 
-def xattn_block(x, wq, colsum, bq, kv, wo, bo, eps, scale, rows_per_b, row_stats=True):
-    if use_hip(x):
-        from . import hip_ops
-
-        return hip_ops.xattn_block(x, wq, colsum, bq, kv, wo, bo, eps, scale, rows_per_b, row_stats=row_stats)
-    return _ref_xattn_block(x, wq, colsum, bq, kv, wo, bo, eps, scale)
-
-
-def _ref_xattn_block(x, wq, colsum, bq, kv, wo, bo, eps, scale):
+_XQ_PERM = tuple((4 * g + j if j < 4 else 16 + 4 * g + j - 4) for g in range(4) for j in range(8))
+
+
+def permute_xattn_q(wq):
+    n, c = wq.shape
+    return wq.reshape(n, c // 32, 32)[:, :, torch.tensor(_XQ_PERM, device=wq.device)].reshape(n, c).contiguous()
+
+
+def unpermute_xattn_q(wqp):
+    n, c = wqp.shape
+    inv = torch.argsort(torch.tensor(_XQ_PERM, device=wqp.device))
+    return wqp.reshape(n, c // 32, 32)[:, :, inv].reshape(n, c).contiguous()
+
+
+def xattn_pre_fusable(o: torch.Tensor, kv, rows_per_b: int, dup=False) -> bool:
+    if not use_hip(o):
+        return False
+    from . import hip_ops
+
+    return hip_ops.xattn_pre_ok(o, kv, rows_per_b, dup)
+
+
+def xattn_block(x, wq, colsum, bq, kv, wo, bo, eps, scale, rows_per_b, row_stats=True, pre=None, batch=None):
+    if use_hip(x if pre is None else pre[0]):
+        from . import hip_ops
+
+        return hip_ops.xattn_block(x, wq, colsum, bq, kv, wo, bo, eps, scale, rows_per_b, row_stats=row_stats,
+                                   pre=pre, batch=batch)
+    return _ref_xattn_block(x, wq, colsum, bq, kv, wo, bo, eps, scale, pre=pre, batch=batch)
+
+
+def _ref_xattn_block(x, wq, colsum, bq, kv, wo, bo, eps, scale, pre=None, batch=None):
+    if pre is not None:
+        o, h0, wo1, bo1 = pre
+        xf = h0.float() + o.float() @ wo1.float().t()
+        if bo1 is not None:
+            xf = xf + bo1.float()
+        if batch is not None and batch != o.shape[0]:
+            xf = xf.repeat(batch // o.shape[0], 1, 1)
+        dt, x, wq = o.dtype, xf, unpermute_xattn_q(wq)
+    else:
+        dt = x.dtype
     xf = x.float()
     mean = xf.mean(-1, keepdim=True)
     rstd = torch.rsqrt(xf.var(-1, unbiased=False, keepdim=True) + eps)
@@ -356,7 +432,7 @@
     y = o @ wo.float().t() + xf
     if bo is not None:
         y = y + bo.float()
-    return y.to(x.dtype)
+    return y.to(dt)
 
 
 def cat_channels(a: torch.Tensor, b: torch.Tensor) -> torch.Tensor:
diff --git a/chiaswarm_amd/ops/hip_ops.py b/chiaswarm_amd/ops/hip_ops.py
--- a/chiaswarm_amd/ops/hip_ops.py
+++ b/chiaswarm_amd/ops/hip_ops.py
@@ -1027,15 +1027,69 @@
 
 def xattn_ok(x, kv, rows_per_b) -> bool:
     C = x.shape[-1]
-    if x.numel() // max(C, 1) // 128 < XATTN_MIN_WG:
+    return _xattn_rows_ok(x.numel() // max(C, 1), C, kv, rows_per_b)
+
+
+def _xattn_rows_ok(M, C, kv, rows_per_b) -> bool:
+    if M // 128 < XATTN_MIN_WG:
         return False
     return (XATTN_FUSED and C in XATTN_CHANNELS and kv is not None and kv.dim() == 5 and kv.shape[2] == 2
             and kv.shape[3] * kv.shape[4] == C and kv.shape[4] == 64 and 1 <= kv.shape[1] <= 80
-            and rows_per_b % 128 == 0 and x.numel() // C % rows_per_b == 0
-            and kv.shape[0] >= x.numel() // C // rows_per_b)
-
-
-def xattn_block(x, wq, colsum, bq, kv, wo, bo, eps, scale, rows_per_b, row_stats=True):
+            and rows_per_b % 128 == 0 and M % rows_per_b == 0
+            and kv.shape[0] >= M // rows_per_b)
+
+
+sig("csk_xattn_block_pre_ok", c_int, c_int, c_int, c_int, c_int, c_int)
+sig("csk_xattn_block_pre", c_void_p, c_void_p, c_void_p, c_void_p, c_void_p, c_void_p, c_void_p, c_void_p, c_void_p,
+    c_void_p, c_void_p, c_void_p, c_int, c_int, c_int, c_int, c_int, c_int, c_float, c_float, c_void_p)
+XATTN_PRE = os.environ.get("CSK_XATTN_PRE", "1") == "1"
+XATTN_DUP = os.environ.get("CSK_XATTN_DUP", "1") == "1"
+XATTN_PRE_STATS = [0]
+XATTN_DUP_STATS = [0]
+
+
+def xattn_pre_ok(o, kv, rows_per_b, dup=False) -> bool:
+    if not XATTN_PRE or (dup and not XATTN_DUP) or o.dim() != 3 or o.dtype != torch.bfloat16:
+        return False
+    b, s, c = o.shape
+    return _xattn_rows_ok((2 * b if dup else b) * s, c, kv, rows_per_b)
+
+
+def _xattn_block_pre(pre, batch, wq, colsum, bq, kv, wo, bo, eps, scale, rows_per_b, row_stats):
+    o, h0, wo1, bo1 = pre
+    for t, n in ((o, "o"), (h0, "h0"), (wo1, "wo1"), (wq, "wq"), (bq, "bq"), (kv, "kv"), (wo, "wo")):
+        _bf16(t, "xattn_block.pre." + n)
+    for t, n in ((bo1, "bo1"), (bo, "bo")):
+        if t is not None:
+            _bf16(t, "xattn_block.pre." + n)
+    b, s, C = o.shape
+    batch = b if batch is None else int(batch)
+    if h0.shape != o.shape or tuple(wo1.shape) != (C, C) or batch % b:
+        raise ValueError(f"xattn_block: prologue operands {tuple(o.shape)} / {tuple(h0.shape)} / {tuple(wo1.shape)} "
+                         f"do not match batch {batch}")
+    src_rows, M = b * s, batch * s
+    kv = kv.contiguous()
+    if colsum.dtype != torch.float32 or colsum.numel() != C:
+        raise ValueError("xattn_block: colsum must be fp32 [C]")
+    if _lib.call_int("csk_xattn_block_pre_ok", M, C, int(rows_per_b), int(kv.shape[0]), int(kv.shape[1]),
+                     src_rows) != 1:
+        raise ValueError(f"xattn_block: unsupported prologue shape M={M} C={C} rows/sample={rows_per_b} "
+                         f"kv={tuple(kv.shape)} source rows={src_rows}")
+    y = torch.empty((batch, s, C), dtype=torch.bfloat16, device=o.device)
+    rp = torch.empty(M * 2, dtype=torch.float32, device=o.device) if row_stats else None
+    (XATTN_DUP_STATS if batch != b else XATTN_PRE_STATS)[0] += 1
+    _lib.call("csk_xattn_block_pre", _p(y), _p(o.contiguous()), _p(h0.contiguous()), _p(wo1.contiguous()),
+              _p(None if bo1 is None else bo1.contiguous()), _p(wq.contiguous()), _p(colsum.contiguous()),
+              _p(bq.contiguous()), _p(kv), _p(wo.contiguous()), _p(None if bo is None else bo.contiguous()), _p(rp),
+              M, C, int(rows_per_b), int(kv.shape[0]), int(kv.shape[1]), src_rows, float(eps), float(scale), _s())
+    if rp is not None:
+        y._csk_rows = (rp, 1, C)
+    return y
+
+
+def xattn_block(x, wq, colsum, bq, kv, wo, bo, eps, scale, rows_per_b, row_stats=True, pre=None, batch=None):
+    if pre is not None:
+        return _xattn_block_pre(pre, batch, wq, colsum, bq, kv, wo, bo, eps, scale, rows_per_b, row_stats)
     for t, n in ((x, "x"), (wq, "wq"), (bq, "bq"), (kv, "kv"), (wo, "wo")):
         _bf16(t, "xattn_block." + n)
     if bo is not None:
@@ -1097,6 +1151,68 @@
               _p(w1p.contiguous()), _p(None if b1p is None else b1p.contiguous()), _p(w2p.contiguous()),
               _p(None if b2 is None else b2.contiguous()), M, C, inner, float(eps), _s())
     return y.view(x.shape)
+
+
+sig("csk_ff_geglu_proj_ok", c_int, c_int, c_int, c_int, c_int)
+sig("csk_ff_geglu_proj", c_void_p, c_void_p, c_void_p, c_void_p, c_void_p, c_void_p, c_void_p, c_void_p, c_void_p,
+    c_void_p, c_void_p, c_void_p, c_int, c_int, c_int, c_int, c_int, c_float, c_void_p)
+FF_PROJ = os.environ.get("CSK_FF_PROJ", "1") == "1"
+FF_PROJ_STATS = [0]
+
+
+def ff_proj_seg(M, C, gn_rows) -> int:
+    hit = tuning._lookup(tuning.table(), f"g:{M}:{C}:{C}:0")
+    tile, split = (int(hit[0]), int(hit[1])) if hit is not None else tuning.heuristic(M, C, C)
+    if split < 0 and tile not in tuning.GLDS:
+        split = 1
+    return _gn_seg(tile, split, gn_rows, M, 0, C)
+
+
+def ff_proj_ok(x, inner: int, gn_rows: int) -> int:
+    C = x.shape[-1]
+    M = x.numel() // C
+    if not (FF_PROJ and ff_fused_ok(x, inner)):
+        return 0
+    seg = ff_proj_seg(M, C, gn_rows)
+    if seg not in (32, 64, 128) or _lib.call_int("csk_ff_geglu_proj_ok", M, C, inner, seg, gn_rows) != 1:
+        return 0
+    return seg
+
+
+def ff_geglu_proj(x, gamma, beta, w1p, b1p, w2p, b2, wpp, bp, xin, eps, gn_rows=0, seg=0):
+    for t, n in ((x, "x"), (gamma, "gamma"), (w1p, "w1p"), (w2p, "w2p"), (wpp, "wpp"), (xin, "xin")):
+        _bf16(t, "ff_geglu_proj." + n)
+    for t, n in ((beta, "beta"), (b2, "b2"), (bp, "bp")):
+        if t is not None:
+            _bf16(t, "ff_geglu_proj." + n)
+    if b1p is not None and b1p.dtype != torch.float32:
+        raise ValueError("ff_geglu_proj: b1p must be fp32")
+    C = x.shape[-1]
+    M = x.numel() // C
+    inner = 32 * w2p.shape[0]
+    if xin.numel() != M * C or tuple(wpp.shape) != (C // 32, C // 32, 32, 32):
+        raise ValueError(f"ff_geglu_proj: residual {tuple(xin.shape)} / packed proj {tuple(wpp.shape)} do not match "
+                         f"{tuple(x.shape)}")
+    if _lib.call_int("csk_ff_geglu_proj_ok", M, C, inner, int(seg), int(gn_rows)) != 1:
+        raise ValueError(f"ff_geglu_proj: unsupported shape M={M} C={C} I={inner} seg={seg} rows/sample={gn_rows}")
+    x2, r2 = x.reshape(M, C), xin.reshape(M, C)
+    if not x2.is_contiguous():
+        x2 = x2.contiguous()
+    if not r2.is_contiguous():
+        r2 = r2.contiguous()
+    z = torch.empty((M, C), dtype=torch.bfloat16, device=x.device)
+    part = _gn_part(M, C, seg, x.device) if seg else None
+    FF_PROJ_STATS[0] += 1
+    _lib.call("csk_ff_geglu_proj", _p(z), _p(x2), _p(gamma.contiguous()),
+              _p(None if beta is None else beta.contiguous()), _p(w1p.contiguous()),
+              _p(None if b1p is None else b1p.contiguous()), _p(w2p.contiguous()),
+              _p(None if b2 is None else b2.contiguous()), _p(wpp.contiguous()),
+              _p(None if bp is None else bp.contiguous()), _p(r2), _p(part), int(seg), int(gn_rows), M, C, inner,
+              float(eps), _s())
+    z = z.view(xin.shape)
+    if part is not None:
+        z._csk_gn = (part, seg)
+    return z
 
 
 sig("csk_set_xattn_probe", c_int)
diff --git a/csrc/kernels/ff.hip b/csrc/kernels/ff.hip
--- a/csrc/kernels/ff.hip
+++ b/csrc/kernels/ff.hip
@@ -14,9 +14,15 @@
   const bf16_t* w2;
   const bf16_t* b2;
   bf16_t* y;
+  const bf16_t* wp;
+  const bf16_t* bp;
+  const bf16_t* xin;
+  float* gn_part;
+  int gn_seg;
   const bf16_t* x_end;
   const bf16_t* w1_end;
   const bf16_t* w2_end;
+  const bf16_t* wp_end;
   int M, I;
   float eps;
 };
@@ -28,6 +34,7 @@
 #define FF_PIECES (FF_SLOT / 512)
 #define FF_PPW (FF_PIECES / FF_WAVES)
 #define FF_IMAX 1280
+#define FF_ZLD 328
 
 template <int N>
 __device__ __forceinline__ void ff_vmcnt() {
@@ -57,7 +64,7 @@
   asm volatile("s_waitcnt lgkmcnt(%4)" : "+v"(b[0]), "+v"(b[1]), "+v"(b[2]), "+v"(b[3]) : "n"(N));
 }
 
-template <int C, int PROBE = 0>
+template <int C, int PROBE = 0, bool PROJ = false>
 __global__ __launch_bounds__(FF_WAVES * 64, 1) void ff_geglu_kernel(const FfArgs a) {
   constexpr int KS = C / 16;
   constexpr int NOT = C / 32;
@@ -75,7 +82,8 @@
   const bool row_ok = row < a.M;
   const int I = a.I;
   const int nchunk = I / 32;
-  const int nslots = 3 * nchunk;
+  const int nff = 3 * nchunk;
+  const int nslots = nff + (PROJ ? NOT : 0);
 
   auto dma_piece = [&](int t, int i) {
     bf16_t* base = ring + (t % FF_NSLOT) * FF_SLOT;
@@ -83,7 +91,9 @@
     const int p = wid + FF_WAVES * i;
     const bf16_t* src = (kind < 2 ? a.w1 + (size_t)(2 * c + kind) * FF_SLOT : a.w2 + (size_t)c * FF_SLOT) +
                         512 * p + 8 * lane;
-    CSK_DCHECK(src + 8 <= (kind < 2 ? a.w1_end : a.w2_end), 91, t, I);
+    const bool tail = PROJ && t >= nff;
+    if (tail) src = a.wp + (size_t)(t - nff) * FF_SLOT + 512 * p + 8 * lane;
+    CSK_DCHECK(src + 8 <= (tail ? a.wp_end : kind < 2 ? a.w1_end : a.w2_end), 91, t, I);
     __builtin_amdgcn_global_load_lds((ff_gptr_t)src, (ff_lptr_t)(base + 512 * p), 16, 0, 0);
   };
   auto dma_slot = [&](int t) {
@@ -219,11 +229,10 @@
     }
   };
 
-  auto w2_slice = [&](int t, const v8s& ha, v16f& acc_b, v4f (&bqb)[4]) {
+  auto slice = [&](int t, v16f (&dst)[NOT], const v8s& ha, v8s& hb, auto&& mid) {
     const unsigned sb = slot_base(t);
     constexpr int NR = 2 * NOT;
     v8s wf[NR];
-    v8s hb;
 #pragma unroll
     for (int i = 0; i < D; ++i) ff_ld(wf[i], sb + w2o[i / NOT] + (unsigned)((i % NOT) * 2048));
 #pragma unroll
@@ -231,14 +240,18 @@
       ff_wait(i + D - 1 < NR ? D - 1 : NR - 1 - i, wf[i]);
       const int o = i % NOT;
       if constexpr ((PROBE & 1) != 0) asm volatile("" ::"v"(wf[i]), "v"(ha), "v"(hb));
-      else out[o] = __builtin_amdgcn_mfma_f32_32x32x16_bf16(wf[i], i < NOT ? ha : hb, out[o], 0, 0, 0);
+      else dst[o] = __builtin_amdgcn_mfma_f32_32x32x16_bf16(wf[i], i < NOT ? ha : hb, dst[o], 0, 0, 0);
       if (i + D < NR) {
         const int i1 = i + D;
         ff_ld(wf[i1], sb + w2o[i1 / NOT] + (unsigned)((i1 % NOT) * 2048));
       }
       dma_hook(t, i);
-      if (i == GAT) hb = geglu(acc_b, bqb);
-    }
+      if (i == GAT) mid();
+    }
+  };
+  auto w2_slice = [&](int t, const v8s& ha, v16f& acc_b, v4f (&bqb)[4]) {
+    v8s hb;
+    slice(t, out, ha, hb, [&] { hb = geglu(acc_b, bqb); });
   };
 
   for (int c = 0; c < nchunk; c += 2) {
@@ -257,6 +270,118 @@
     w2_slice(t + 5, ha, acc_b, bqb);
   }
 
+  auto u2f4 = [](const uint2& u, float (&f)[4]) {
+    f[0] = bf2f((bf16_t)(u.x & 0xffff));
+    f[1] = bf2f((bf16_t)(u.x >> 16));
+    f[2] = bf2f((bf16_t)(u.y & 0xffff));
+    f[3] = bf2f((bf16_t)(u.y >> 16));
+  };
+  if constexpr (PROJ) {
+    uint2 xr[NOT][4], br[NOT][4], xi[NOT][4];
+#pragma unroll
+    for (int o = 0; o < NOT; ++o)
+#pragma unroll
+      for (int q = 0; q < 4; ++q) {
+        const int n = 32 * o + 8 * q + 4 * h;
+        CSK_DCHECK(a.x + (size_t)row * C + n + 4 <= a.x_end, 95, row, a.M);
+        xr[o][q] = *reinterpret_cast<const uint2*>(a.x + (size_t)row * C + n);
+        br[o][q] = a.b2 ? *reinterpret_cast<const uint2*>(a.b2 + n) : make_uint2(0, 0);
+      }
+#pragma unroll
+    for (int o = 0; o < NOT; ++o)
+#pragma unroll
+      for (int q = 0; q < 4; ++q) {
+        const int n = 32 * o + 8 * q + 4 * h;
+        xi[o][q] = *reinterpret_cast<const uint2*>(a.xin + (size_t)row * C + n);
+      }
+    v8s yf[NOT][2];
+#pragma unroll
+    for (int o = 0; o < NOT; ++o) {
+      float v[16];
+#pragma unroll
+      for (int q = 0; q < 4; ++q) {
+        float rv[4], bb[4];
+        u2f4(xr[o][q], rv);
+        u2f4(br[o][q], bb);
+#pragma unroll
+        for (int r = 0; r < 4; ++r) v[4 * q + r] = out[o][4 * q + r] + bb[r] + rv[r];
+      }
+      yf[o][0] = __builtin_bit_cast(v8s, pack8(v));
+      yf[o][1] = __builtin_bit_cast(v8s, pack8(v + 8));
+    }
+    v16f z[NOT];
+#pragma unroll
+    for (int o = 0; o < NOT; ++o)
+#pragma unroll
+      for (int i = 0; i < 16; ++i) z[o][i] = 0.f;
+#pragma unroll
+    for (int j = 0; j < NOT; ++j) {
+      if ((j & 1) == 0) enter_pair(nff + j);
+      slice(nff + j, z, yf[j][0], yf[j][1], [] {});
+    }
+    asm volatile("s_waitcnt vmcnt(0) lgkmcnt(0)" ::: "memory");
+    __syncthreads();
+    bf16_t* zs = ring + wid * 32 * FF_ZLD;
+#pragma unroll
+    for (int o = 0; o < NOT; ++o)
+#pragma unroll
+      for (int q = 0; q < 4; ++q) {
+        float rv[4], bb[4];
+        u2f4(xi[o][q], rv);
+        u2f4(a.bp ? *reinterpret_cast<const uint2*>(a.bp + 32 * o + 8 * q + 4 * h) : make_uint2(0, 0), bb);
+        uint2 w;
+        w.x = pack2(z[o][4 * q] + bb[0] + rv[0], z[o][4 * q + 1] + bb[1] + rv[1]);
+        w.y = pack2(z[o][4 * q + 2] + bb[2] + rv[2], z[o][4 * q + 3] + bb[3] + rv[3]);
+        *reinterpret_cast<uint2*>(zs + r32 * FF_ZLD + 32 * o + 8 * q + 4 * h) = w;
+      }
+    __syncthreads();
+    float* st = reinterpret_cast<float*>(ring + FF_WAVES * 32 * FF_ZLD);
+    if (lane < C / 8) {
+      bf16_t* yrow = a.y + (size_t)(m0 + wid * 32) * C + 8 * lane;
+      float sum[8], m2[8];
+#pragma unroll
+      for (int j = 0; j < 8; ++j) sum[j] = m2[j] = 0.f;
+#pragma unroll 8
+      for (int r = 0; r < 32; ++r) {
+        const uint4 u = *reinterpret_cast<const uint4*>(zs + r * FF_ZLD + 8 * lane);
+        *reinterpret_cast<uint4*>(yrow + (size_t)r * C) = u;
+        float f[8];
+        unpack8(u, f);
+#pragma unroll
+        for (int j = 0; j < 8; ++j) sum[j] += f[j];
+      }
+      if (a.gn_part) {
+#pragma unroll
+        for (int j = 0; j < 8; ++j) sum[j] *= (1.0f / 32);
+#pragma unroll 8
+        for (int r = 0; r < 32; ++r) {
+          float f[8];
+          unpack8(*reinterpret_cast<const uint4*>(zs + r * FF_ZLD + 8 * lane), f);
+#pragma unroll
+          for (int j = 0; j < 8; ++j) {
+            const float d = f[j] - sum[j];
+            m2[j] = __builtin_fmaf(d, d, m2[j]);
+          }
+        }
+#pragma unroll
+        for (int j = 0; j < 8; ++j)
+          *reinterpret_cast<float2*>(st + ((size_t)wid * C + 8 * lane + j) * 2) = make_float2(sum[j], m2[j]);
+      }
+    }
+    if (!a.gn_part) return;
+    __syncthreads();
+    const int seg = a.gn_seg, per = seg / 32;
+    for (int i = tid; i < (FF_ROWS / seg) * C; i += FF_WAVES * 64) {
+      const int n = i % C, sg = i / C;
+      float cnt = 0.f, mean = 0.f, q2 = 0.f;
+      for (int w = 0; w < per; ++w) {
+        const float2 pm = *reinterpret_cast<const float2*>(st + ((size_t)(sg * per + w) * C + n) * 2);
+        chan_combine(cnt, mean, q2, 32.f, pm.x, pm.y);
+      }
+      *reinterpret_cast<float2*>(a.gn_part + ((size_t)(m0 / seg + sg) * C + n) * 2) = make_float2(mean, q2);
+    }
+    return;
+  }
   if (!row_ok) return;
   uint2 xr[NOT][4], br[NOT][4];
 #pragma unroll
@@ -299,7 +424,7 @@
 CSK_API int csk_ff_geglu(void* y, const void* x, const void* gamma, const void* beta, const void* w1, const void* b1,
                          const void* w2, const void* b2, int M, int C, int I, float eps, hipStream_t stream) {
   if (!csk_ff_geglu_ok(M, C, I) || !x || !y || !gamma || !w1 || !w2 || x == y) return (int)hipErrorInvalidValue;
-  FfArgs a;
+  FfArgs a = {};
   a.x = (const bf16_t*)x;
   a.gamma = (const bf16_t*)gamma;
   a.beta = (const bf16_t*)beta;
@@ -323,3 +448,45 @@
   }
   return (int)hipGetLastError();
 }
+
+CSK_API int csk_ff_geglu_proj_ok(int M, int C, int I, int gn_seg, int rows_per_b) {
+  if (!csk_ff_geglu_ok(M, C, I) || M % FF_ROWS) return 0;
+  if (gn_seg == 0) return 1;
+  return ((gn_seg == 32 || gn_seg == 64 || gn_seg == 128) && rows_per_b > 0 && rows_per_b % gn_seg == 0 &&
+          M % rows_per_b == 0)
+             ? 1
+             : 0;
+}
+
+CSK_API int csk_ff_geglu_proj(void* z, const void* x, const void* gamma, const void* beta, const void* w1,
+                              const void* b1, const void* w2, const void* b2, const void* wp, const void* bp,
+                              const void* xin, void* gn_part, int gn_seg, int rows_per_b, int M, int C, int I, float eps,
+                              hipStream_t stream) {
+  if (!gn_part) gn_seg = 0;
+  if (!csk_ff_geglu_proj_ok(M, C, I, gn_seg, rows_per_b) || !x || !z || !gamma || !w1 || !w2 || !wp || !xin ||
+      x == z || xin == z)
+    return (int)hipErrorInvalidValue;
+  FfArgs a = {};
+  a.x = (const bf16_t*)x;
+  a.gamma = (const bf16_t*)gamma;
+  a.beta = (const bf16_t*)beta;
+  a.w1 = (const bf16_t*)w1;
+  a.b1 = (const float*)b1;
+  a.w2 = (const bf16_t*)w2;
+  a.b2 = (const bf16_t*)b2;
+  a.y = (bf16_t*)z;
+  a.wp = (const bf16_t*)wp;
+  a.bp = (const bf16_t*)bp;
+  a.xin = (const bf16_t*)xin;
+  a.gn_part = (float*)gn_part;
+  a.gn_seg = gn_seg;
+  a.x_end = a.x + (size_t)M * C;
+  a.w1_end = a.w1 + (size_t)2 * I * C;
+  a.w2_end = a.w2 + (size_t)C * I;
+  a.wp_end = a.wp + (size_t)C * C;
+  a.M = M;
+  a.I = I;
+  a.eps = eps;
+  ff_geglu_kernel<320, 0, true><<<dim3(M / FF_ROWS), FF_WAVES * 64, 0, stream>>>(a);
+  return (int)hipGetLastError();
+}
diff --git a/csrc/kernels/xattn.hip b/csrc/kernels/xattn.hip
--- a/csrc/kernels/xattn.hip
+++ b/csrc/kernels/xattn.hip
@@ -14,6 +14,11 @@
   bf16_t* y;
   float* row_part;
   const bf16_t* zero;
+  const bf16_t* o;
+  const bf16_t* h0;
+  const bf16_t* wo1;
+  const bf16_t* bo1;
+  int src_rows;
   const bf16_t* x_end;
   const bf16_t* kv_end;
   int M, rows_per_b, Skv;
@@ -38,7 +43,7 @@
 __device__ __forceinline__ int xa_off64(int r, int c) { return at_off64(r, c); }
 __device__ __forceinline__ v8s xa_pack8(const v4f& lo, const v4f& hi, float s) { return at_pack8(lo, hi, s); }
 
-template <int C, int NW, int RT, int PROBE = 0>
+template <int C, int NW, int RT, int PROBE = 0, bool PRE = false>
 __global__ __launch_bounds__(NW * 64, 1) void xattn_block_kernel(const XattnArgs a) {
   constexpr int H = C / 64, NCS = C / 32, NNT = C / 16, CPR = C / 8;
   constexpr int WQ = 64 * C, WO = C * 64, KVI = XA_KVR * 64;
@@ -69,15 +74,16 @@
       xa_dma_off(a.wq, (unsigned)((h * 64 + row) * C + 8 * (slot ^ (row & 7))), s_wq + 512 * p);
     }
   };
-  auto dma_wo = [&](int h) {
+  auto dma_cols = [&](const bf16_t* w, int h, bf16_t* dst) {
 #pragma unroll
     for (int i = 0; i < NWO; ++i) {
       const int p = wid + NW * i;
       const int row = 8 * p + (lane >> 3), slot = lane & 7;
       CSK_DCHECK(row < C, 72, row, C);
-      xa_dma_off(a.wo, (unsigned)(row * C + h * 64 + 8 * (slot ^ at_key(row))), s_wo + 512 * p);
+      xa_dma_off(w, (unsigned)(row * C + h * 64 + 8 * (slot ^ at_key(row))), dst + 512 * p);
     }
   };
+  auto dma_wo = [&](int h) { dma_cols(a.wo, h, s_wo); };
   auto dma_kv = [&](int h, bf16_t* dst) {
 #pragma unroll
     for (int i = 0; i < NKV; ++i) {
@@ -95,10 +101,73 @@
     s_cb[i] = a.colsum[i];
     s_cb[C + i] = bf2f(a.bq[i]);
   }
+  v8s xf[RT][NCS];
+  if constexpr (PRE) {
+    static_assert(WQ == WO && C % 64 == 0, "Wo1 K-slices double-buffer through s_wq / s_wo");
+    constexpr int NKS = C / 64;
+    dma_kv(0, s_kv0);
+    v8s of0[RT][NCS];
+    uint2 hres[RT][NNT];
+#pragma unroll
+    for (int rt = 0; rt < RT; ++rt) {
+      const int ms = (row_w + rt * 16 + fr) % a.src_rows;
+      CSK_DCHECK(a.o + (size_t)ms * C + C <= a.x_end, 75, ms, a.src_rows);
+#pragma unroll
+      for (int cs = 0; cs < NCS; ++cs)
+        of0[rt][cs] = __builtin_bit_cast(v8s, *reinterpret_cast<const uint4*>(a.o + (size_t)ms * C + 32 * cs + 8 * g));
+#pragma unroll
+      for (int nt = 0; nt < NNT; ++nt)
+        hres[rt][nt] = *reinterpret_cast<const uint2*>(a.h0 + (size_t)ms * C + 16 * nt + 4 * g);
+    }
+    dma_cols(a.wo1, 0, s_wq);
+    dma_cols(a.wo1, 1, s_wo);
+    v4f xa[RT][NNT];
+#pragma unroll
+    for (int rt = 0; rt < RT; ++rt)
+#pragma unroll
+      for (int nt = 0; nt < NNT; ++nt) xa[rt][nt] = v4f{0.f, 0.f, 0.f, 0.f};
+#pragma unroll
+    for (int ks = 0; ks < NKS; ++ks) {
+      xa_vmcnt<NWO>();
+      __builtin_amdgcn_s_barrier();
+      const bf16_t* buf = (ks & 1) ? s_wo : s_wq;
+#pragma unroll
+      for (int nt = 0; nt < NNT; ++nt) {
+#pragma unroll
+        for (int ds = 0; ds < 2; ++ds) {
+          const v8s wf = *reinterpret_cast<const v8s*>(buf + at_off64(16 * nt + fr, 4 * ds + g));
+#pragma unroll
+          for (int rt = 0; rt < RT; ++rt)
+            xa[rt][nt] = __builtin_amdgcn_mfma_f32_16x16x32_bf16(wf, of0[rt][2 * ks + ds], xa[rt][nt], 0, 0, 0);
+        }
+      }
+      asm volatile("s_waitcnt lgkmcnt(0)" ::: "memory");
+      __builtin_amdgcn_s_barrier();
+      if (ks + 2 < NKS) dma_cols(a.wo1, ks + 2, (ks & 1) ? s_wo : s_wq);
+      else if (ks & 1) dma_wo(0);
+      else dma_wq(0);
+    }
+#pragma unroll
+    for (int rt = 0; rt < RT; ++rt)
+#pragma unroll
+      for (int nt = 0; nt < NNT; ++nt) {
+        const uint2 u = hres[rt][nt];
+        const uint2 ub = a.bo1 ? *reinterpret_cast<const uint2*>(a.bo1 + 16 * nt + 4 * g) : make_uint2(0, 0);
+        const float rv[4] = {bf2f((bf16_t)(u.x & 0xffff)), bf2f((bf16_t)(u.x >> 16)), bf2f((bf16_t)(u.y & 0xffff)),
+                             bf2f((bf16_t)(u.y >> 16))};
+        const float bv[4] = {bf2f((bf16_t)(ub.x & 0xffff)), bf2f((bf16_t)(ub.x >> 16)), bf2f((bf16_t)(ub.y & 0xffff)),
+                             bf2f((bf16_t)(ub.y >> 16))};
+#pragma unroll
+        for (int r = 0; r < 4; ++r) xa[rt][nt][r] = xa[rt][nt][r] + bv[r] + rv[r];
+      }
+#pragma unroll
+    for (int rt = 0; rt < RT; ++rt)
+#pragma unroll
+      for (int cs = 0; cs < NCS; ++cs) xf[rt][cs] = xa_pack8(xa[rt][2 * cs], xa[rt][2 * cs + 1], 1.0f);
+  } else {
   dma_wq(0);
   dma_wo(0);
   dma_kv(0, s_kv0);
-  v8s xf[RT][NCS];
 #pragma unroll
   for (int rt = 0; rt < RT; ++rt) {
     const int m = row_w + rt * 16 + fr;
@@ -111,6 +180,7 @@
       }
       xf[rt][cs] = __builtin_bit_cast(v8s, u);
     }
+  }
   }
   float mean[RT], rstd[RT];
 #pragma unroll
@@ -261,6 +331,12 @@
   }
 
   uint2 xres[RT][NNT], bres[NNT];
+  if constexpr (PRE) {
+#pragma unroll
+    for (int rt = 0; rt < RT; ++rt)
+#pragma unroll
+      for (int cs = 0; cs < NCS; ++cs) asm volatile("" : "+v"(xf[rt][cs]));
+  }
 #pragma unroll
   for (int nt = 0; nt < NNT; ++nt) {
     bres[nt] = make_uint2(0, 0);
@@ -272,7 +348,12 @@
 #pragma unroll
     for (int nt = 0; nt < NNT; ++nt) {
       xres[rt][nt] = make_uint2(0, 0);
-      if (m < a.M) xres[rt][nt] = *reinterpret_cast<const uint2*>(a.x + (size_t)m * C + 16 * nt + 4 * g);
+      if constexpr (PRE) {
+        const uint4 u = __builtin_bit_cast(uint4, xf[rt][nt >> 1]);
+        xres[rt][nt] = (nt & 1) ? make_uint2(u.z, u.w) : make_uint2(u.x, u.y);
+      } else if (m < a.M) {
+        xres[rt][nt] = *reinterpret_cast<const uint2*>(a.x + (size_t)m * C + 16 * nt + 4 * g);
+      }
     }
   }
 #pragma unroll
@@ -355,7 +436,7 @@
   if (!csk_zero_ptr()) return (int)hipErrorNotInitialized;
   if (Skv < 1 || Skv > 80 || rows_per_b % XA_BM != 0 || M % rows_per_b != 0 || M / rows_per_b > Bc)
     return (int)hipErrorInvalidValue;
-  XattnArgs a;
+  XattnArgs a = {};
   a.x = (const bf16_t*)x;
   a.wq = (const bf16_t*)wq;
   a.colsum = (const float*)colsum;
@@ -383,3 +464,44 @@
   }
   return (int)hipGetLastError();
 }
+
+CSK_API int csk_xattn_block_pre_ok(int M, int C, int rows_per_b, int Bc, int Skv, int src_rows) {
+  return (C == 320 && Skv >= 1 && Skv <= 80 && rows_per_b > 0 && rows_per_b % XA_BM == 0 && M > 0 &&
+          M % rows_per_b == 0 && M / rows_per_b <= Bc && src_rows > 0 && M % src_rows == 0)
+             ? 1
+             : 0;
+}
+
+CSK_API int csk_xattn_block_pre(void* y, const void* o, const void* h0, const void* wo1, const void* bo1,
+                                const void* wq, const void* colsum, const void* bq, const void* kv, const void* wo,
+                                const void* bo, void* row_part, int M, int C, int rows_per_b, int Bc, int Skv,
+                                int src_rows, float eps, float scale, hipStream_t stream) {
+  if (!csk_zero_ptr()) return (int)hipErrorNotInitialized;
+  if (!csk_xattn_block_pre_ok(M, C, rows_per_b, Bc, Skv, src_rows) || !y || !o || !h0 || !wo1 || !wq || !colsum ||
+      !bq || !kv || !wo || y == o || y == h0)
+    return (int)hipErrorInvalidValue;
+  XattnArgs a = {};
+  a.o = (const bf16_t*)o;
+  a.h0 = (const bf16_t*)h0;
+  a.wo1 = (const bf16_t*)wo1;
+  a.bo1 = (const bf16_t*)bo1;
+  a.src_rows = src_rows;
+  a.wq = (const bf16_t*)wq;
+  a.colsum = (const float*)colsum;
+  a.bq = (const bf16_t*)bq;
+  a.kv = (const bf16_t*)kv;
+  a.wo = (const bf16_t*)wo;
+  a.bo = (const bf16_t*)bo;
+  a.y = (bf16_t*)y;
+  a.row_part = (float*)row_part;
+  a.zero = csk_zero_ptr();
+  a.x_end = a.o + (size_t)src_rows * C;
+  a.kv_end = a.kv + (size_t)Bc * Skv * 2 * C;
+  a.M = M;
+  a.rows_per_b = rows_per_b;
+  a.Skv = Skv;
+  a.eps = eps;
+  a.scale_log2 = scale * 1.4426950408889634f;
+  xattn_block_kernel<320, 8, 1, 0, true><<<dim3(M / XA_BM), 8 * 64, 0, stream>>>(a);
+  return (int)hipGetLastError();
+}
```

Measured after the change: 7.688 images/s (median of 6 runs). 1.01x the previous value.
